# GuoYi0/alphaFive

Hardware: AMD Instinct MI355X
Metric: self-play moves/sec (11x11, 500 sims/move) (higher is better)
Workload: dtype f32 (fp16x2 split operands: 3 fp16 MFMA products per MAC, fp32 accumulate)

## Files before the change

### alphafive_amd/csrc/af_conv_f16s.h

```cpp
#ifndef AF_CONV_F16S_H
#define AF_CONV_F16S_H

#include <hip/hip_runtime.h>

#define AF_NET_BLOCKS(X) X("bone/block1", 32, 64) X("bone/block2", 64, 128) X("value/block3", 128, 32) X("policy/block4", 128, 64) X("policy/block5", 64, 32)
struct NetBlock { const char* name; int cin, cout; };
#define AF_BLOCK_ROW(name, cin, cout) {name, cin, cout},
constexpr NetBlock kBlocks[5] = {AF_NET_BLOCKS(AF_BLOCK_ROW)};
enum { kVarStemK, kVarStemB, kVarHeads, kVarVcK = kVarHeads, kVarVcB, kVarV1K, kVarV1B, kVarV2K, kVarV2B, kVarPcK, kVarPcB, kVarPfK, kVarPfB,
       kVarBlocks, kVars = kVarBlocks + 6 * 5, kC1K = 0, kC1B, kC2K, kC2B, kResK, kResB };
constexpr int var(int block, int which) { return kVarBlocks + 6 * block + which; }
struct NetVar { const char* name; int c0, c1, c2; };
#define AF_BLOCK_VARS(name, cin, cout) {name "_conv1/kernel", 9 * cin * cout}, {name "_conv1/bias", cout}, {name "_conv2/kernel", 9 * cout * cout}, \
                                       {name "_conv2/bias", cout}, {name "_res/kernel", cin * cout}, {name "_res/bias", cout},
constexpr NetVar kNetVars[kVars] = {
    {"bone/conv1/kernel", 75 * 32}, {"bone/conv1/bias", 32}, {"value/conv/kernel", 32 * 4}, {"value/conv/bias", 4},
    {"value/fc1/kernel", 0, 4 * 64}, {"value/fc1/bias", 64}, {"value/fc2/kernel", 64}, {"value/fc2/bias", 1},
    {"policy/conv/kernel", 32 * 16}, {"policy/conv/bias", 16}, {"policy/fc/kernel", 0, 0, 16}, {"policy/fc/bias", 0, 1},
    AF_NET_BLOCKS(AF_BLOCK_VARS)};

struct f16s_net;

int f16s_supported(int board_size);
int f16s_create(f16s_net** out, int board_size, int max_batch, int device);
void f16s_destroy(f16s_net* n);
int f16s_reset_roles(f16s_net* n);
enum F16sBits : int {
    kF16sProfilingBits = 1 | 2 | 4 | 8 | 4096,
    kF16sValuStem = 16,
    kF16sOneWgPerCu = 32,
    kF16sTwoHalves15 = 64,
    kF16sWgPerPosition = 128,
    kF16sTwoLaunchBlocks = 256,
    kF16sBranchLaunchesSmall = 512,
    kF16sBranchLaunchesBig = 1024,
    kF16sLaunchSequence = 2048,
};
enum F16sForm {
    kF16sRoles,
    kF16sPaired,
    kF16sBranches,
};
struct F16sPlan {
    int batch, bits;
    bool heads;
    F16sForm form;
    bool valu_stem, two_wg_per_cu, half_classes, tile_split, fused_blocks;
};
F16sPlan f16s_plan(const f16s_net* n, int batch, int bits, bool heads);
int f16s_forward(f16s_net* n, const F16sPlan& p, hipStream_t st, const float* planes_dev, float* value, float* policy);
int f16s_trunk(f16s_net* n, const F16sPlan& p, hipStream_t st, const float* planes_dev);
int f16s_value_branch(f16s_net* n, const F16sPlan& p, hipStream_t st, float* o3_dev, int WP, int PP, float* value);
int f16s_policy_branch(f16s_net* n, const F16sPlan& p, hipStream_t st, float* o5_dev, int WP, int PP, float* policy);
int f16s_small_forward_error(f16s_net* n);
int f16s_read_activation(f16s_net* n, int which, int batch, float* host);

constexpr int kF16sScaleGroups = 20;
int f16s_update_absmax(f16s_net* n, hipStream_t st, const float* const* src, float* max_dev);
int f16s_update_pack(f16s_net* n, hipStream_t st, const float* const* src, const float* max_host);
int f16s_weight_buffer(const f16s_net* n, int index, const void** ptr, size_t* bytes);
int f16s_scales(const f16s_net* n, float* out, int cap);
struct UpdCopy { float* dst; const float* a; const float* b; int n_dst, n_src, sum; };
int upd_launch_copies(hipStream_t st, const UpdCopy* d, int count);

#endif
```

### alphafive_amd/csrc/af_conv_f16s.hip

```cpp
#include <hip/hip_runtime.h>
#include <stdint.h>
#include <stdio.h>
#include <stdlib.h>
#include <string.h>

#include <algorithm>
#include <atomic>
#include <cmath>
#include <vector>

#include "af_conv_f16s.h"

typedef _Float16 h8 __attribute__((ext_vector_type(8)));
typedef float f32x16 __attribute__((ext_vector_type(16)));
typedef float f32x4 __attribute__((ext_vector_type(4)));

#define FS_HIP_OK(x) do { hipError_t e_ = (x); if (e_ != hipSuccess) { fprintf(stderr, "[af_conv_f16s] %s failed: %s\n", #x, hipGetErrorString(e_)); return -2; } } while (0)

namespace {

template <int S_> struct Geo;
template <> struct Geo<11> {
    static constexpr int S = 11, NPIX = 121, HALVES = 1, POFF = 11;
    static constexpr uint32_t ROWU = 144, WINU = 144;
    static constexpr int PR = 2, NPC = 4;
    static constexpr uint32_t PADL = 8, PADR = 8;
    __host__ __device__ static constexpr uint32_t seg_unit(int seg) { return 8u + 64u * (uint32_t)seg; }
    __host__ __device__ static constexpr uint32_t wbase(int) { return 0u; }
};
template <> struct Geo<15> {
    static constexpr int S = 15, NPIX = 225, HALVES = 2, POFF = 16;
    static constexpr uint32_t ROWU = 256, WINU = 160;
    static constexpr int PR = 3, NPC = 6;
    static constexpr uint32_t PADL = 0, PADR = 0;
    __host__ __device__ static constexpr uint32_t seg_unit(int seg) { return seg == 0 ? 0u : (seg == 1 ? 64u : 96u); }
    __host__ __device__ static constexpr uint32_t wbase(int h) { return h ? 96u : 0u; }
};
template <class G> struct Lay {
    static constexpr uint32_t kRowH = G::ROWU * 16u, kHalfH = 4u * kRowH, kSlabH = 2u * kHalfH;
    static constexpr uint32_t kRowL = G::WINU * 16u, kHalfL = 4u * kRowL, kSlotL = 2u * kHalfL;
};
constexpr uint32_t kLds0 = 256u;
#ifndef AF_F16S_DIST
#define AF_F16S_DIST 3
#endif
constexpr int kDist = AF_F16S_DIST;
template <class G, int DIST = kDist> struct Lds {
    static constexpr uint32_t kZoff = kLds0 + (DIST + 2) * Lay<G>::kSlotL;
    static constexpr uint32_t kBiasOff = kZoff + Lay<G>::kSlotL;
    static constexpr uint32_t kScrOff = kBiasOff + 512u;
};
template <class G> struct Hx {
    static constexpr int HXP = 128 * G::HALVES;
    static constexpr uint32_t kValPos = HXP * 16u, kValLo = HXP * 8u;
    static constexpr uint32_t kPolPos = HXP * 64u, kPolLo = HXP * 32u;
    static constexpr int VSTEPS = (G::NPIX + 3) / 4;
    static constexpr int NLT = (G::NPIX + 31) / 32;
};

constexpr int kS = 11, kPIX = 144, kNPIX = kS * kS;
constexpr uint32_t kRowB = kPIX * 16u, kHalfB = 4u * kRowB, kSlabB = 2u * kHalfB;

#ifndef AF_F16S_APIN
#define AF_F16S_APIN 1
#endif
#ifndef AF_F16S_VW
#define AF_F16S_VW 128
#endif
#ifndef AF_F16S_ZPAD
#define AF_F16S_ZPAD 1
#endif

__device__ __forceinline__ void st16(void* gdst, const h8& v) { *reinterpret_cast<h8*>(gdst) = v; }

template <class V16>
__device__ __forceinline__ void st16_sc1(void* gdst, const V16& v) {
    static_assert(sizeof(V16) == 16, "16-byte store");
    asm volatile("global_store_dwordx4 %0, %1, off sc1\n\ts_nop 1" : : "v"(gdst), "v"(v) : "memory");
}
template <class V8>
__device__ __forceinline__ void st8_sc1(void* gdst, const V8& v) {
    static_assert(sizeof(V8) == 8, "8-byte store");
    asm volatile("global_store_dwordx2 %0, %1, off sc1" : : "v"(gdst), "v"(v) : "memory");
}

__device__ __forceinline__ void wait_vmcnt(int n) {
#define AF_VM(k) case k: asm volatile("s_waitcnt vmcnt(" #k ")" ::: "memory"); break;
    switch (n) {
        AF_VM(0) AF_VM(1) AF_VM(2) AF_VM(3) AF_VM(4) AF_VM(5) AF_VM(6) AF_VM(7) AF_VM(8) AF_VM(9) AF_VM(10) AF_VM(11) AF_VM(12) AF_VM(13)
        AF_VM(14) AF_VM(15) AF_VM(16) AF_VM(17) AF_VM(18) AF_VM(19) AF_VM(20) AF_VM(21) AF_VM(22) AF_VM(23) AF_VM(24) AF_VM(25) AF_VM(26)
        AF_VM(27) AF_VM(28) AF_VM(29) AF_VM(30) AF_VM(31) AF_VM(32) AF_VM(33) AF_VM(34) AF_VM(35) AF_VM(36) AF_VM(37) AF_VM(38) AF_VM(39)
        AF_VM(40) AF_VM(41) AF_VM(42) AF_VM(43) AF_VM(44) AF_VM(45) AF_VM(46) AF_VM(47) AF_VM(48) AF_VM(49) AF_VM(50) AF_VM(51) AF_VM(52)
        AF_VM(53) AF_VM(54) AF_VM(55) AF_VM(56) AF_VM(57) AF_VM(58) AF_VM(59) AF_VM(60) AF_VM(61) AF_VM(62) AF_VM(63)
        default: asm volatile("s_waitcnt vmcnt(0)" ::: "memory"); break;
    }
#undef AF_VM
}

__device__ __forceinline__ void glds16(const void* gsrc, uint32_t lds_dst) {
    unsigned keep;
    asm volatile("s_mov_b32 %0, m0\n\ts_mov_b32 m0, %2\n\ts_nop 0\n\tglobal_load_lds_dwordx4 %1, off nt\n\ts_mov_b32 m0, %0"
                 : "=&s"(keep) : "v"(gsrc), "s"(lds_dst) : "memory");
}

__device__ __forceinline__ void glds16_sc1(const void* gsrc, uint32_t lds_dst) {
    unsigned keep;
    asm volatile("s_mov_b32 %0, m0\n\ts_mov_b32 m0, %2\n\ts_nop 0\n\tglobal_load_lds_dwordx4 %1, off sc1\n\ts_mov_b32 m0, %0"
                 : "=&s"(keep) : "v"(gsrc), "s"(lds_dst) : "memory");
}

typedef float f32x2 __attribute__((ext_vector_type(2)));
__device__ __forceinline__ float elu1(float x) {
    const float e = __builtin_amdgcn_exp2f(x * 1.44269504088896341f);
    return fmaxf(x, fminf(fmaxf(e, 0.0f), 1.0f) - 1.0f);
}
__device__ __forceinline__ f32x2 elu2(f32x2 x) {
    const f32x2 t = x * 1.44269504088896341f;
    f32x2 e;
    e.x = fminf(fmaxf(__builtin_amdgcn_exp2f(t.x), 0.0f), 1.0f);
    e.y = fminf(fmaxf(__builtin_amdgcn_exp2f(t.y), 0.0f), 1.0f);
    const f32x2 em1 = e - 1.0f;
    return f32x2{fmaxf(x.x, em1.x), fmaxf(x.y, em1.y)};
}

#ifndef AF_F16S_XCD_SWIZZLE
#define AF_F16S_XCD_SWIZZLE 1
#endif
#ifdef AF_F16S_TIMING
__device__ unsigned long long g_f16s_cycles[10][512][4][9];
__device__ unsigned long long g_f16s_wall[10][512][2];
#define AF_T(var) const unsigned long long var = __builtin_readcyclecounter()
#define AF_TACC(slot, a, b) tacc[slot] += (b) - (a)
#else
#define AF_T(var)
#define AF_TACC(slot, a, b)
#endif

#ifdef AF_DF_TIMING
__device__ unsigned long long g_df_wall[256][5];
#define DF_T(i) if (threadIdx.x == 0 && blockIdx.x < 256) g_df_wall[blockIdx.x][i] = wall_clock64()
#else
#define DF_T(i)
#endif
__device__ __forceinline__ void df_signal(int* ctr) {
    DF_T(2);
    asm volatile("s_waitcnt vmcnt(0)" ::: "memory");
    __syncthreads();
    if (threadIdx.x == 0) __hip_atomic_fetch_add(ctr, 1, __ATOMIC_RELAXED, __HIP_MEMORY_SCOPE_AGENT);
    DF_T(3);
}
__device__ __forceinline__ void df_poll(const int* ctr, int need, int* err) {
    int it = 0;
    while (__hip_atomic_load(ctr, __ATOMIC_RELAXED, __HIP_MEMORY_SCOPE_AGENT) < need) {
        __builtin_amdgcn_s_sleep(2);
        if (++it > (1 << 22)) { __hip_atomic_store(err, 1, __ATOMIC_RELAXED, __HIP_MEMORY_SCOPE_AGENT); break; }
    }
}
__device__ __forceinline__ void df_wait_one(const int* ctr, int need, int* err) {
    if (threadIdx.x == 0) df_poll(ctr, need, err);
    DF_T(1);
    __syncthreads();
}
__device__ __forceinline__ void df_wait_inv(const int* ctr, int need, int* err) {
    if (threadIdx.x == 0) {
        df_poll(ctr, need, err);
        __builtin_amdgcn_fence(__ATOMIC_ACQUIRE, "agent");
    }
    DF_T(1);
    __syncthreads();
}

struct F16sArgs {
    const char* in;
    const char* in2;
    const uint4* w;
    const float* bias;
    char* out;
    float* out32;
    float inv_scale;
    const uint4* pw;
    float* pbuf;
    float inv_scale_p;
    const uint4* hw;
    const float* hbias;
    char* hx;
    float inv_scale_h;
    int batch, WP, PP;
    const uint4* w2;
    const float* bias2;
    float inv_scale2;
    int gx0;
    char* stash;
    const int* df_wait;
    int df_need;
    int* df_done;
    int* df_err;
    int abl;
};

template <class G, int NSM, int NSP, int CT, int KS, int PS, bool OUT32, bool XACC, int PJ, int HD, int DIST, int WPE, int NTW, int HSEL, int FU = 0, int DF = 0>
__device__ __forceinline__ void f16s_body(const F16sArgs& A, char* smem, const int bx, const int gxw, const int tb = 0,
                                          const int by = (int)blockIdx.y, const int gy = (int)gridDim.y) {
    using L = Lay<G>;
    constexpr uint32_t kRowH = L::kRowH, kHalfH = L::kHalfH, kSlabH = L::kSlabH, kRowL = L::kRowL, kHalfL = L::kHalfL, kSlotL = L::kSlotL;
    constexpr uint32_t kZoff = Lds<G, DIST>::kZoff, kBiasOff = Lds<G, DIST>::kBiasOff, kScrOff = Lds<G, DIST>::kScrOff;
    constexpr int kDist = DIST, kRing = DIST + 2;
    constexpr int NPC = G::NPC, HV = G::HALVES;
    static_assert(FU == 0 || (G::HALVES == 1 && PJ == 1 && HD == 0 && !OUT32 && NSP == 0 && CT == 1 && HSEL < 0 &&
                              ((KS == 1 && NTW == 1) || (KS == 2 && NTW == 2))), "fused block: see above");
    constexpr uint32_t kScrBytes = KS == 2 ? (uint32_t)(CT * PS * NTW) * 4096u * (PJ == 1 ? 2u : 1u) : 0u;
    constexpr uint32_t kGOff = Lds<G, DIST>::kScrOff;
    constexpr uint32_t kW2Off = kGOff + (kScrBytes > Lay<G>::kSlotL ? kScrBytes : Lay<G>::kSlotL);
    constexpr int NT = NTW;
    static_assert(HSEL < 0 || (HV == 2 && PJ == 0 && HD == 0 && !OUT32), "half classes: plain 15x15 layers only");
    static_assert(NT % KS == 0 || PJ == 0, "an odd tile count under a k-split has no projection exchange");
    constexpr int C16 = 2 / KS;
    constexpr int ITP = C16, ITM = 9 * C16;
    constexpr int NIT = NSP * ITP + NSM * ITM;
    constexpr int SPP = NSP + NSM;
    constexpr int NFIN = NT / KS;
    static_assert(CT * KS * PS == 4 && NT >= KS, "4 waves");
    static_assert(PJ == 0 || NSP == 0, "a producer / consumer of the separate projection has no projection slabs");
    constexpr int NPW = PJ == 1 ? NSM * C16 : 0;
    static_assert(NPC * (DIST > 1 ? DIST - 1 : 1) < 64, "vmcnt is a 6-bit field");
    static_assert(DIST >= 2 || (NSP == 0 && ITM - 1 >= NPC), "distance 1: a slab's pieces must all be issued before its predecessor's last item");
    const int lane = threadIdx.x & 63, kg = lane >> 5, nn = lane & 31;
    const int wv = __builtin_amdgcn_readfirstlane((int)(threadIdx.x >> 6));
    const int ct = wv % CT, ks = (wv / CT) % KS, ps = wv / (CT * KS);
    const int rot = KS == 2 ? ks * ((NT + 1) / 2) : 0;
#define AF_OWN(jj) (KS == 1 || (jj) < NT / 2 || ((jj) < (NT + 1) / 2 && ks == 0))
    const int ctg = by * CT + ct, nso = gy * CT;
    const uint32_t lds = (uint32_t)(uintptr_t)smem;

    const int nq = HSEL >= 0 ? A.batch : A.batch * HV;
    int qpos = bx;
    if (AF_F16S_XCD_SWIZZLE && (gxw & (8 * (HSEL >= 0 ? 1 : HV) - 1)) == 0) qpos = (bx >> 3) + (gxw >> 3) * (bx & 7);
    if (qpos >= nq) return;
    const int hv = HSEL >= 0 ? HSEL : (HV == 1 ? 0 : qpos % HV);
    const uint32_t wsrc = G::wbase(hv) * 16u;
    AF_T(t_entry);
#ifdef AF_F16S_TIMING
    const unsigned long long wall_entry = wall_clock64();
#endif

    auto slab_src = [&](int qq, int j) -> const char* {
        const int p_ = (HV == 1 || HSEL >= 0) ? qq : qq / HV;
        const int p = (A.abl & 0x1000) ? (p_ & 127) : p_;
        return (j < NSM ? A.in + ((size_t)p * NSM + j) * kSlabH : A.in2 + ((size_t)p * NSP + (j - NSM)) * kSlabH) + wsrc;
    };
    auto dma_piece = [&](const char* src, uint32_t slot_off, int k) {
        const int piece = wv + 4 * k, row = piece / G::PR;
        const uint32_t su = G::seg_unit(piece % G::PR) * 16u;
        const uint32_t offh = (uint32_t)(row >> 2) * kHalfH + (uint32_t)(row & 3) * kRowH + su;
        const uint32_t offl = (uint32_t)(row >> 2) * kHalfL + (uint32_t)(row & 3) * kRowL + su;
        if (DF != 0) glds16_sc1(src + offh + lane * 16, (uint32_t)__builtin_amdgcn_readfirstlane((int)(lds + kLds0 + slot_off + offl)));
        else glds16(src + offh + lane * 16, (uint32_t)__builtin_amdgcn_readfirstlane((int)(lds + kLds0 + slot_off + offl)));
    };
    const int q0 = qpos;
    auto stream_src = [&](uint32_t idx) -> const char* {
        const int p = q0 + (int)(idx / SPP) * gxw, j = (int)(idx % SPP);
        return slab_src(p, j);
    };
    const uint32_t nslabs = (uint32_t)((nq - q0 + gxw - 1) / gxw) * SPP;

    if (DF == 0) {
#pragma unroll
        for (int d = 0; d < kDist; ++d) {
            if ((uint32_t)d < nslabs) {
#pragma unroll
                for (int k = 0; k < NPC; ++k) dma_piece(stream_src(d), (uint32_t)d * kSlotL, k);
            }
        }
    }

    h8 W[2 * NIT];
    {
        const uint4* wp = A.w + ((size_t)(ctg * KS + ks) * (2 * NIT)) * 64 + lane;
#pragma unroll
        for (int f = 0; f < 2 * NIT; ++f) {
            const uint4 v = wp[f * 64];
            __builtin_memcpy(&W[f], &v, 16);
        }
    }
    h8 PW[PJ == 1 ? 2 * NPW : 1];
    if (PJ == 1) {
        const uint4* wp = A.pw + ((size_t)(ctg * KS + ks) * (2 * NPW)) * 64 + lane;
#pragma unroll
        for (int f = 0; f < 2 * NPW; ++f) {
            const uint4 v = wp[f * 64];
            __builtin_memcpy(&PW[f], &v, 16);
        }
    }
    constexpr int HDS = HD > 0 ? HD : FU;
    h8 HA[HDS > 0 ? 4 : 1];
    float hb[HDS > 0 ? 8 : 1];
    if (FU > 0) {
        const uint4* w2 = A.w2;
#pragma unroll
        for (int i = 0; i < 9; ++i) *reinterpret_cast<uint4*>(smem + kW2Off + (uint32_t)(i * 256 + (int)threadIdx.x) * 16u) = w2[i * 256 + threadIdx.x];
        if (threadIdx.x < 32) reinterpret_cast<float*>(smem + kBiasOff + 256u)[threadIdx.x] = A.bias2[threadIdx.x];
        if (KS == 1) {
            for (uint32_t u = threadIdx.x; u < kSlotL / 16; u += 256) *reinterpret_cast<uint4*>(smem + kGOff + u * 16) = uint4{0, 0, 0, 0};
        }
    }
    if (HDS > 0) {
#pragma unroll
        for (int f = 0; f < 4; ++f) {
            const uint4 v = A.hw[f * 64 + lane];
            __builtin_memcpy(&HA[f], &v, 16);
        }
#pragma unroll
        for (int r = 0; r < 8; ++r) hb[r] = A.hbias[8 * kg + r];
    }
    if (threadIdx.x < kLds0 / 16) *reinterpret_cast<uint4*>(smem + threadIdx.x * 16) = uint4{0, 0, 0, 0};
    if (G::PADL + G::PADR > 0) {
        static_assert(G::PADL + G::PADR == 0 || (G::PADL == 8 && G::PADR == 8), "pad zeroing is written for 8 + 8 units");
        for (uint32_t u = threadIdx.x; u < (uint32_t)kRing * 128u; u += 256) {
            const uint32_t off = kLds0 + (u >> 7) * kSlotL + ((u >> 4) & 7u) * kRowL + (((u >> 3) & 1u) ? (G::WINU - 8u) * 16u : 0u) + (u & 7u) * 16u;
            *reinterpret_cast<uint4*>(smem + off) = uint4{0, 0, 0, 0};
        }
    }
    for (uint32_t u = threadIdx.x; u < kSlotL / 16; u += 256) *reinterpret_cast<uint4*>(smem + kZoff + u * 16) = uint4{0, 0, 0, 0};
    if (threadIdx.x < CT * 32) reinterpret_cast<float*>(smem + kBiasOff)[threadIdx.x] = A.bias[by * CT * 32 + threadIdx.x];
    uint32_t lb[NT], zb[NT];
    int pix[NT];
    bool ok[NT], edgeL[NT], edgeR[NT];
#pragma unroll
    for (int jj = 0; jj < NT; ++jj) {
        const int n = 128 * hv + 32 * (tb + ps * NT + ((jj + rot) % NT)) + nn;
        ok[jj] = n < G::NPIX;
        const int nc = ok[jj] ? n : 128 * hv;
        pix[jj] = nc;
        const int x = nc % G::S;
        edgeL[jj] = x == 0; edgeR[jj] = x == G::S - 1;
        lb[jj] = kLds0 + (uint32_t)((KS == 2 ? 2 * ks : 0) + kg) * kRowL + (uint32_t)((nc + G::POFF - G::S - 1 - (int)G::wbase(hv)) * 16);
        zb[jj] = kZoff + (lb[jj] & 255u);
    }
    constexpr int kAccRegs = 16 * NT * (1 + (XACC ? 1 : 0) + (PJ == 1 ? 1 : 0));
    constexpr int kWRegs = 4 * (2 * NIT + (PJ == 1 ? 2 * NPW : 0) + (HDS > 0 ? 4 : 0));
    constexpr int kNAmax = (256 - kAccRegs - 16) / 4, kNAwant = (kWRegs - AF_F16S_VW + 3) / 4;
    constexpr int NA = (AF_F16S_APIN && WPE == 1 && kNAwant > 0) ? (kNAwant < kNAmax ? kNAwant : kNAmax) : 0;
#pragma unroll
    for (int f = 0; f < 2 * NIT; ++f) {
        if (f < 2 * NIT - NA) asm volatile("" : "+v"(W[f]));
        else asm volatile("" : "+a"(W[f]));
    }
    if (PJ == 1) {
#pragma unroll
        for (int f = 0; f < 2 * NPW; ++f) asm volatile("" : "+v"(PW[f]));
    }
    if (HDS > 0) {
#pragma unroll
        for (int f = 0; f < 4; ++f) asm volatile("" : "+v"(HA[f]));
    }
    if (DF != 0) {
        df_wait_one(A.df_wait + qpos, A.df_need, A.df_err);
#pragma unroll
        for (int d = 0; d < kDist; ++d) {
            if ((uint32_t)d < nslabs) {
#pragma unroll
                for (int k = 0; k < NPC; ++k) dma_piece(stream_src(d), (uint32_t)d * kSlotL, k);
            }
        }
    }
    asm volatile("s_waitcnt vmcnt(0) lgkmcnt(0)" ::: "memory");
    __builtin_amdgcn_s_barrier();
    AF_T(t_ready);

    auto rd = [](const char* sm, bool proj, int it, int p, uint32_t c_, uint32_t l_, uint32_t r_) -> h8 {
        const int c = proj ? it : it / 9, tap = proj ? 4 : it % 9, ky = tap / 3, kx = tap % 3;
        const uint32_t base = kx == 0 ? l_ : (kx == 2 ? r_ : c_);
        const uint32_t imm = (uint32_t)p * kHalfL + (KS == 1 ? 2u * c * kRowL : 0u) + (uint32_t)(ky * G::S + kx) * 16u;
        return *reinterpret_cast<const h8*>(sm + base + imm);
    };

    auto head_tile = [&](const float (&v)[16], const int jj, const int pos) {
      if constexpr (HDS > 0) {
        h8 bh[2], bl[2];
#pragma unroll
        for (int st_ = 0; st_ < 2; ++st_)
#pragma unroll
            for (int e = 0; e < 8; ++e) {
                const float f = v[8 * st_ + e];
                const _Float16 h = (_Float16)f;
                bh[st_][e] = h;
                bl[st_][e] = (_Float16)(f - (float)h);
            }
        f32x16 a2;
#pragma unroll
        for (int r = 0; r < 16; ++r) a2[r] = 0.0f;
#pragma unroll
        for (int st_ = 0; st_ < 2; ++st_) {
            a2 = __builtin_amdgcn_mfma_f32_32x32x16_f16(HA[2 * st_], bh[st_], a2, 0, 0, 0);
            a2 = __builtin_amdgcn_mfma_f32_32x32x16_f16(HA[2 * st_], bl[st_], a2, 0, 0, 0);
            a2 = __builtin_amdgcn_mfma_f32_32x32x16_f16(HA[2 * st_ + 1], bh[st_], a2, 0, 0, 0);
        }
        constexpr int NR = HDS == 1 ? 4 : 8;
        _Float16 uh[8], ul[8];
#pragma unroll
        for (int r = 0; r < NR; ++r) {
            const float f = elu1(a2[r] * A.inv_scale_h + hb[r]);
            const _Float16 h = (_Float16)f;
            uh[r] = h;
            ul[r] = (_Float16)(f - (float)h);
        }
        if (ok[jj] && !(A.abl & 2)) {
            if (HDS == 1) {
                if (kg == 0) {
                    typedef _Float16 h4 __attribute__((ext_vector_type(4)));
                    char* o = A.hx + (size_t)pos * Hx<G>::kValPos + (uint32_t)pix[jj] * 8u;
                    if (DF != 0) {
                        st8_sc1(o, h4{uh[0], uh[1], uh[2], uh[3]});
                        st8_sc1(o + Hx<G>::kValLo, h4{ul[0], ul[1], ul[2], ul[3]});
                    } else {
                        *reinterpret_cast<h4*>(o) = h4{uh[0], uh[1], uh[2], uh[3]};
                        *reinterpret_cast<h4*>(o + Hx<G>::kValLo) = h4{ul[0], ul[1], ul[2], ul[3]};
                    }
                }
            } else {
                char* o = A.hx + (size_t)pos * Hx<G>::kPolPos + (uint32_t)pix[jj] * 32u + (uint32_t)kg * 16u;
                if (DF != 0) {
                    st16_sc1(o, h8{uh[0], uh[1], uh[2], uh[3], uh[4], uh[5], uh[6], uh[7]});
                    st16_sc1(o + Hx<G>::kPolLo, h8{ul[0], ul[1], ul[2], ul[3], ul[4], ul[5], ul[6], ul[7]});
                } else {
                    *reinterpret_cast<h8*>(o) = h8{uh[0], uh[1], uh[2], uh[3], uh[4], uh[5], uh[6], uh[7]};
                    *reinterpret_cast<h8*>(o + Hx<G>::kPolLo) = h8{ul[0], ul[1], ul[2], ul[3], ul[4], ul[5], ul[6], ul[7]};
                }
            }
        }
      }
    };
    uint32_t t = 0;
    uint32_t cur = 0u, nxd = (uint32_t)kDist * kSlotL;
    constexpr bool XPOS = !(NT >= 3 && NIT >= 36) && FU == 0;
    h8 fr[2][NT][2];
#define AF_FIRST_ITEM(slot)                                                                                      \
    _Pragma("unroll") for (int jj = 0; jj < NT; ++jj) {                                                          \
        const uint32_t c_ = (AF_F16S_ZPAD && !ok[jj]) ? zb[jj] : lb[jj] + (slot), l_ = edgeL[jj] ? zb[jj] : c_, r_ = edgeR[jj] ? zb[jj] : c_; \
        fr[0][jj][0] = rd(smem, false, 0, 0, c_, l_, r_);                                                        \
        fr[0][jj][1] = rd(smem, false, 0, 1, c_, l_, r_);                                                        \
    }
    if (XPOS) { AF_FIRST_ITEM(0u) }
#ifdef AF_F16S_TIMING
    unsigned long long tacc[8] = {0, 0, 0, 0, 0, 0, 0, 0};
#endif
    for (; qpos < nq; qpos += gxw) {
        const int pos = (HV == 1 || HSEL >= 0) ? qpos : qpos / HV;
        AF_T(tp0);
        if (!XPOS) { AF_FIRST_ITEM(cur) }
#undef AF_FIRST_ITEM
        f32x16 acc[NT], acx[XACC ? NT : 1], pac[PJ == 1 ? NT : 1];
#pragma unroll
        for (int jj = 0; jj < NT; ++jj)
#pragma unroll
            for (int r = 0; r < 16; ++r) { acc[jj][r] = 0.0f; if (XACC) acx[jj][r] = 0.0f; if (PJ == 1) pac[jj][r] = 0.0f; }
        f32x4 padd[PJ == 2 ? NFIN : 1][4];
        if (PJ == 2) {
#pragma unroll
            for (int jf = 0; jf < NFIN; ++jf) {
                const int tile = tb + ps * NT + (KS == 2 ? ks * NFIN : 0) + jf;
                const f32x4* src = reinterpret_cast<const f32x4*>(A.pbuf) + ((((size_t)qpos * nso + ctg) * 4 + tile) * 4) * 64 + lane;
#pragma unroll
                for (int q = 0; q < 4; ++q) padd[jf][q] = src[q * 64];
            }
        }

#pragma clang loop unroll(full)
        for (int j = 0; j < SPP; ++j) {
            const bool proj = j >= NSM;
            const bool nproj = (j + 1) % SPP >= NSM;
            const int ms = j, pslab = j - NSM;
            const int NI = proj ? ITP : ITM;
            const int ibase = proj ? pslab * ITP : NSP * ITP + ms * ITM;
            const int seq = proj ? NSM * ITM + pslab * ITP : ms * ITM;
            const int npos = qpos + ((j + kDist) / SPP) * gxw;
            const bool more = npos < nq && !(A.abl & 1);
            const char* nsrc = slab_src((A.abl & 4) ? q0 : (more ? npos : qpos), (j + kDist) % SPP);
            const uint32_t nx1 = cur + kSlotL == kRing * kSlotL ? 0u : cur + kSlotL;
            uint32_t bC[NT], bL[NT], bR[NT];
#pragma unroll
            for (int jj = 0; jj < NT; ++jj) {
                bC[jj] = (AF_F16S_ZPAD && !ok[jj]) ? zb[jj] : lb[jj] + cur;
                bL[jj] = edgeL[jj] ? zb[jj] : bC[jj];
                bR[jj] = edgeR[jj] ? zb[jj] : bC[jj];
            }
            if (HSEL == 1 && wv == (j & 3) && by == 0 && lane < 32) {
                const uint32_t u = (uint32_t)(lane & 3), un = (u < 2 ? 128u + u : 141u + u);
                const uint4 q = *reinterpret_cast<const uint4*>(smem + kLds0 + cur + (uint32_t)(lane >> 4) * kHalfL + (uint32_t)((lane >> 2) & 3) * kRowL + un * 16u);
                *reinterpret_cast<uint4*>(A.stash + (((size_t)pos * SPP + j) * 32 + lane) * 16) = q;
            }
#pragma clang loop unroll(full)
            for (int it = 0; it < NI; ++it) {
                const int b = (seq + it) & 1;
                if (it + 1 < NI) {
#pragma unroll
                    for (int jj = 0; jj < NT; ++jj) {
                        fr[b ^ 1][jj][0] = rd(smem, proj, it + 1, 0, bC[jj], bL[jj], bR[jj]);
                        fr[b ^ 1][jj][1] = rd(smem, proj, it + 1, 1, bC[jj], bL[jj], bR[jj]);
                    }
                } else {
                    const int issued = NI - 1 < NPC ? NI - 1 : NPC;
                    AF_T(tw0);
                    if (more) {
                        wait_vmcnt(NPC * (kDist - 2) + issued);
                    } else {
                        asm volatile("s_waitcnt vmcnt(0)" ::: "memory");
                    }
                    AF_T(tw1);
                    __builtin_amdgcn_s_barrier();
                    AF_T(tw2);
                    AF_TACC(1, tw0, tw1);
                    AF_TACC(2, tw1, tw2);
                    if ((XPOS || j + 1 < SPP) && t + 1 < nslabs) {
#pragma unroll
                        for (int jj = 0; jj < NT; ++jj) {
                            const uint32_t c_ = (AF_F16S_ZPAD && !ok[jj]) ? zb[jj] : lb[jj] + nx1, l_ = edgeL[jj] ? zb[jj] : c_, r_ = edgeR[jj] ? zb[jj] : c_;
                            fr[b ^ 1][jj][0] = rd(smem, nproj, 0, 0, c_, l_, r_);
                            fr[b ^ 1][jj][1] = rd(smem, nproj, 0, 1, c_, l_, r_);
                        }
                    }
                }
                const h8 wh = W[2 * (ibase + it)], wl = W[2 * (ibase + it) + 1];
#pragma unroll
                for (int jj = 0; jj < NT; ++jj) acc[jj] = __builtin_amdgcn_mfma_f32_32x32x16_f16(wh, fr[b][jj][0], acc[jj], 0, 0, 0);
                if (XACC) {
#pragma unroll
                    for (int jj = 0; jj < NT; ++jj) acx[jj] = __builtin_amdgcn_mfma_f32_32x32x16_f16(wh, fr[b][jj][1], acx[jj], 0, 0, 0);
#pragma unroll
                    for (int jj = 0; jj < NT; ++jj) acx[jj] = __builtin_amdgcn_mfma_f32_32x32x16_f16(wl, fr[b][jj][0], acx[jj], 0, 0, 0);
                } else {
#pragma unroll
                    for (int jj = 0; jj < NT; ++jj) acc[jj] = __builtin_amdgcn_mfma_f32_32x32x16_f16(wh, fr[b][jj][1], acc[jj], 0, 0, 0);
#pragma unroll
                    for (int jj = 0; jj < NT; ++jj) acc[jj] = __builtin_amdgcn_mfma_f32_32x32x16_f16(wl, fr[b][jj][0], acc[jj], 0, 0, 0);
                }
                if (PJ == 1 && !proj && it % 9 == 4) {
                    const int pi = ms * C16 + it / 9;
                    const h8 ph = PW[2 * pi], pl = PW[2 * pi + 1];
#pragma unroll
                    for (int jj = 0; jj < NT; ++jj) pac[jj] = __builtin_amdgcn_mfma_f32_32x32x16_f16(ph, fr[b][jj][0], pac[jj], 0, 0, 0);
#pragma unroll
                    for (int jj = 0; jj < NT; ++jj) pac[jj] = __builtin_amdgcn_mfma_f32_32x32x16_f16(ph, fr[b][jj][1], pac[jj], 0, 0, 0);
#pragma unroll
                    for (int jj = 0; jj < NT; ++jj) pac[jj] = __builtin_amdgcn_mfma_f32_32x32x16_f16(pl, fr[b][jj][0], pac[jj], 0, 0, 0);
                }
#pragma unroll
                for (int q = 0; q < 2 * NT; ++q) {
                    __builtin_amdgcn_sched_group_barrier(0x008, 1, 0);
                    __builtin_amdgcn_sched_group_barrier(0x100, 1, 0);
                }
                __builtin_amdgcn_sched_group_barrier(0x008, NT, 0);
                if (more) {
                    if (it < NI - 1 && it < NPC) dma_piece(nsrc, nxd, it);
                    if (it == NI - 1) {
#pragma unroll
                        for (int k = (NI - 1 < NPC ? NI - 1 : NPC); k < NPC; ++k) dma_piece(nsrc, nxd, k);
                    }
                }
            }
            ++t;
            cur = nx1;
            nxd = nxd + kSlotL == kRing * kSlotL ? 0u : nxd + kSlotL;
        }
        if (XPOS && (NIT & 1)) {
#pragma unroll
            for (int jj = 0; jj < NT; ++jj) { fr[0][jj][0] = fr[1][jj][0]; fr[0][jj][1] = fr[1][jj][1]; }
        }

        AF_T(tp1);
        if (XACC) {
#pragma unroll
            for (int jj = 0; jj < NT; ++jj)
#pragma unroll
                for (int r = 0; r < 16; ++r) acc[jj][r] += acx[jj][r];
        }
#define AF_EXCHANGE(ACC, SCR)                                                                                              \
    {                                                                                                                      \
        _Pragma("unroll") for (int jj = 0; jj < NT; ++jj) {                                                                \
            if (!AF_OWN(jj)) {                                                                                             \
                _Pragma("unroll") for (int q = 0; q < 4; ++q) {                                                            \
                    f32x4 v = {ACC[jj][4 * q], ACC[jj][4 * q + 1], ACC[jj][4 * q + 2], ACC[jj][4 * q + 3]};                \
                    *reinterpret_cast<f32x4*>((SCR) + (uint32_t)(((jj + rot) % NT) * 4 + q) * 1024u + lane * 16u) = v;     \
                }                                                                                                          \
            }                                                                                                              \
        }                                                                                                                  \
    }
#define AF_COMBINE(ACC, SCR)                                                                                               \
    {                                                                                                                      \
        _Pragma("unroll") for (int jj = 0; jj < NT; ++jj) {                                                                \
            if (AF_OWN(jj)) {                                                                                              \
                _Pragma("unroll") for (int q = 0; q < 4; ++q) {                                                            \
                    const f32x4 v = *reinterpret_cast<const f32x4*>((SCR) + (uint32_t)(((jj + rot) % NT) * 4 + q) * 1024u + lane * 16u); \
                    ACC[jj][4 * q] += v[0]; ACC[jj][4 * q + 1] += v[1]; ACC[jj][4 * q + 2] += v[2]; ACC[jj][4 * q + 3] += v[3]; \
                }                                                                                                          \
            }                                                                                                              \
        }                                                                                                                  \
    }
        if (KS == 2) {
            char* scr = smem + kScrOff + (uint32_t)(ct + CT * ps) * (NT * 4096u);
            char* scp = scr + (uint32_t)(CT * PS) * (NT * 4096u);
            AF_EXCHANGE(acc, scr)
            if (PJ == 1) AF_EXCHANGE(pac, scp)
            asm volatile("s_waitcnt lgkmcnt(0)" ::: "memory");
            AF_T(tx0);
            __builtin_amdgcn_s_barrier();
            AF_T(tx1);
            AF_TACC(7, tx0, tx1);
            AF_COMBINE(acc, scr)
            if (PJ == 1) AF_COMBINE(pac, scp)
        }
#undef AF_EXCHANGE
#undef AF_COMBINE
        if (PJ == 1 && FU == 0) {
#pragma unroll
            for (int jj = 0; jj < NT; ++jj) {
                if (!AF_OWN(jj)) continue;
                f32x4* dst = reinterpret_cast<f32x4*>(A.pbuf) + ((((size_t)qpos * nso + ctg) * 4 + tb + ps * NT + ((jj + rot) % NT)) * 4) * 64 + lane;
                if (!(A.abl & 2)) {
#pragma unroll
                    for (int q = 0; q < 4; ++q) {
                        f32x4 v = {pac[jj][4 * q] * A.inv_scale_p, pac[jj][4 * q + 1] * A.inv_scale_p, pac[jj][4 * q + 2] * A.inv_scale_p, pac[jj][4 * q + 3] * A.inv_scale_p};
                        dst[q * 64] = v;
                    }
                }
            }
        }

        if (FU > 0 && KS == 2) {
// ... 186 lines not shown
    const int tile = (int)blockIdx.y * 4 + (int)(threadIdx.x >> 6);
    if (tile >= A.NCT) return;
    const int p = 32 * (int)blockIdx.x + nn;
    const bool valid = p < A.batch;
    const size_t pc = (size_t)(valid ? p : A.batch - 1);
    f32x16 acc[KS], acx[XACC ? KS : 1];
#pragma unroll
    for (int h = 0; h < KS; ++h)
#pragma unroll
        for (int r = 0; r < 16; ++r) { acc[h][r] = 0.0f; if (XACC) acx[h][r] = 0.0f; }
    const uint4* const wbase = A.w + (size_t)tile * KS * NIT * 2 * 64 + lane;
    constexpr int SPP = NSM + NSP;
    const char* const st0 = A.stash + (pc * SPP * 32 + (uint32_t)kg * 4u) * 16;
    struct Ops { uint4 a0, a1, b0, b1; };
    auto half_of = [](int t) constexpr -> int {
        const int k16 = t < NSM * 8 ? (t >> 2) & 1 : (t - NSM * 8) & 1;
        return KS == 2 ? k16 : 0;
    };
    auto fetch = [&](int t) -> Ops {
        int k16, item;
        const char* bsrc;
        if (t < NSM * 8) {
            const int s_ = t >> 3, tq = t & 3, ky = tq >> 1, kx = tq & 1;
            k16 = (t >> 2) & 1;
            item = NSP * C16 + s_ * 9 * C16 + (KS == 2 ? 0 : k16) * 9 + 3 * ky + kx;
            bsrc = st0 + (uint32_t)((s_ * 32 + 2 * k16 * 4 + tq) * 16);
        } else {
            const int u = t - NSM * 8, s_ = u >> 1;
            k16 = u & 1;
            item = s_ * C16 + (KS == 2 ? 0 : k16);
            bsrc = st0 + (uint32_t)(((NSM + s_) * 32 + 2 * k16 * 4 + 3) * 16);
        }
        const uint4* wp = wbase + ((size_t)((KS == 2 ? k16 : 0) * NIT + item) * 2) * 64;
        Ops o;
        o.a0 = wp[0]; o.a1 = wp[64];
        o.b0 = *reinterpret_cast<const uint4*>(bsrc); o.b1 = *reinterpret_cast<const uint4*>(bsrc + 256);
        return o;
    };
    Ops ring[D];
#pragma unroll
    for (int t = 0; t < D; ++t) ring[t] = fetch(t);
    __builtin_amdgcn_sched_barrier(0);
#pragma unroll
    for (int t = 0; t < NST; ++t) {
        const Ops o = ring[t % D];
        if (t + D < NST) ring[t % D] = fetch(t + D);
        const int h = half_of(t);
        h8 wh, wl, bh, bl;
        __builtin_memcpy(&wh, &o.a0, 16); __builtin_memcpy(&wl, &o.a1, 16); __builtin_memcpy(&bh, &o.b0, 16); __builtin_memcpy(&bl, &o.b1, 16);
        acc[h] = __builtin_amdgcn_mfma_f32_32x32x16_f16(wh, bh, acc[h], 0, 0, 0);
        if (XACC) {
            acx[h] = __builtin_amdgcn_mfma_f32_32x32x16_f16(wh, bl, acx[h], 0, 0, 0);
            acx[h] = __builtin_amdgcn_mfma_f32_32x32x16_f16(wl, bh, acx[h], 0, 0, 0);
        } else {
            acc[h] = __builtin_amdgcn_mfma_f32_32x32x16_f16(wh, bl, acc[h], 0, 0, 0);
            acc[h] = __builtin_amdgcn_mfma_f32_32x32x16_f16(wl, bh, acc[h], 0, 0, 0);
        }
        __builtin_amdgcn_sched_group_barrier(0x008, 3, 0);
        __builtin_amdgcn_sched_group_barrier(0x020, 4, 0);
    }
    if (XACC) {
#pragma unroll
        for (int h = 0; h < KS; ++h)
#pragma unroll
            for (int r = 0; r < 16; ++r) acc[h][r] += acx[h][r];
    }
    if (KS == 2) {
#pragma unroll
        for (int r = 0; r < 16; ++r) acc[0][r] = acc[KS - 1][r] + acc[0][r];
    }
    if (!valid) return;
    float v[16];
#pragma unroll
    for (int r = 0; r < 16; r += 2) {
        const f32x2 pre = f32x2{acc[0][r], acc[0][r + 1]} * A.inv_scale + f32x2{A.bias[32 * tile + 16 * kg + r], A.bias[32 * tile + 16 * kg + r + 1]};
        const f32x2 y = elu2(pre);
        v[r] = y.x; v[r + 1] = y.y;
    }
    char* o = A.out + ((size_t)p * A.NCT + tile) * L::kSlabH + (uint32_t)(2 * kg) * L::kRowH + (uint32_t)(CPIX + G::POFF) * 16u;
#pragma unroll
    for (int hf = 0; hf < 2; ++hf) {
        h8 hi, lo;
#pragma unroll
        for (int e = 0; e < 8; ++e) {
            const float f = v[8 * hf + e];
            const _Float16 h = (_Float16)f;
            hi[e] = h;
            lo[e] = (_Float16)(f - (float)h);
        }
        st16(o + hf * L::kRowH, hi);
        st16(o + hf * L::kRowH + L::kHalfH, lo);
    }
}

template <class G>
__global__ __launch_bounds__(256) void af_stem_f16s(const float* __restrict__ planes, const float* __restrict__ w,
                                                    const float* __restrict__ bias, char* __restrict__ out, int batch) {
    constexpr int S = G::S, NPIX = G::NPIX, SP = S + 4;
    constexpr uint32_t kRowH = Lay<G>::kRowH, kHalfH = Lay<G>::kHalfH, kSlabH = Lay<G>::kSlabH;
    __shared__ float sx[3 * SP * SP];
    __shared__ float sw[75 * 32];
    __shared__ float sb[32];
    const int t = threadIdx.x;
    for (int i = t; i < 75 * 32; i += 256) sw[i] = w[i];
    if (t < 32) sb[t] = bias[t];
    for (int i = t; i < 3 * SP * SP; i += 256) sx[i] = 0.0f;
    for (int b = blockIdx.x; b < batch; b += gridDim.x) {
        __syncthreads();
        for (int i = t; i < 3 * NPIX; i += 256) {
            const int c = i / NPIX, p = i - c * NPIX, y = p / S, x = p - y * S;
            sx[c * SP * SP + (y + 2) * SP + x + 2] = planes[(size_t)b * 3 * NPIX + i];
        }
        __syncthreads();
        if (t < NPIX) {
            const int y = t / S, x = t - y * S;
            float acc[32];
#pragma unroll
            for (int co = 0; co < 32; ++co) acc[co] = sb[co];
            for (int ky = 0; ky < 5; ++ky)
                for (int kx = 0; kx < 5; ++kx)
#pragma unroll
                    for (int c = 0; c < 3; ++c) {
                        const float xv = sx[c * SP * SP + (y + ky) * SP + x + kx];
                        const float* wr = sw + ((ky * 5 + kx) * 3 + c) * 32;
#pragma unroll
                        for (int co = 0; co < 32; ++co) acc[co] = fmaf(xv, wr[co], acc[co]);
                    }
            char* o = out + (size_t)b * kSlabH + (uint32_t)(t + G::POFF) * 16u;
#pragma unroll
            for (int u = 0; u < 4; ++u) {
                h8 hi, lo;
#pragma unroll
                for (int e = 0; e < 8; ++e) {
                    const float f = elu1(acc[8 * u + e]);
                    const _Float16 h = (_Float16)f;
                    hi[e] = h;
                    lo[e] = (_Float16)(f - (float)h);
                }
                *reinterpret_cast<h8*>(o + u * kRowH) = hi;
                *reinterpret_cast<h8*>(o + u * kRowH + kHalfH) = lo;
            }
        }
    }
}

template <class G> struct StemLds {
    static constexpr int SR = G::S + 4, IW = G::S + 5;
    static constexpr int kEnt = 3 * SR * G::S + 1, kImg = 3 * SR * IW;
    static constexpr uint32_t kImgOff = (uint32_t)((kEnt * 16 + 255) / 256 * 256), kBytes = kImgOff + (uint32_t)kImg * 2u;
};
template <class G, bool SC1 = false>
__device__ __forceinline__ void f16s_stem_body(const float* __restrict__ planes, const uint4* __restrict__ w ,
                                               const float* __restrict__ bias, float inv_scale, char* __restrict__ out, int batch,
                                               const int bx, const int gx, uint4* ent, _Float16* img) {
    constexpr int S = G::S, NPIX = G::NPIX, SR = S + 4, IW = S + 5;
    constexpr int NPL = 3 * NPIX, NLD = (NPL + 255) / 256;
    constexpr int NTL = (NPIX + 31) / 32, NRND = (NTL + 3) / 4;
    constexpr uint32_t kRowH = Lay<G>::kRowH, kHalfH = Lay<G>::kHalfH, kSlabH = Lay<G>::kSlabH;
    const int lane = threadIdx.x & 63, kg = lane >> 5, nn = lane & 31;
    const int wv = __builtin_amdgcn_readfirstlane((int)(threadIdx.x >> 6));
    h8 W[16];
#pragma unroll
    for (int f = 0; f < 16; ++f) {
        const uint4 v = w[f * 64 + lane];
        __builtin_memcpy(&W[f], &v, 16);
    }
    float bs[16];
#pragma unroll
    for (int r = 0; r < 16; ++r) bs[r] = bias[16 * kg + r];
    for (int i = threadIdx.x; i < 3 * SR * IW; i += 256) img[i] = (_Float16)0.0f;
    auto img_at = [](int i) -> int { const int c = i / NPIX, p = i - c * NPIX, y = p / S, x = p - y * S; return (c * SR + y + 2) * IW + x + 2; };
    int at[NLD];
    float nx[NLD];
#pragma unroll
    for (int q = 0; q < NLD; ++q) {
        const int i = (int)threadIdx.x + 256 * q;
        at[q] = img_at(i < NPL ? i : 0);
        nx[q] = 0.0f;
        if (i < NPL && bx < batch) nx[q] = planes[(size_t)bx * NPL + i];
    }
    for (int pos = bx; pos < batch; pos += gx) {
        __syncthreads();
#pragma unroll
        for (int q = 0; q < NLD; ++q)
            if ((int)threadIdx.x + 256 * q < NPL) img[at[q]] = (_Float16)nx[q];
        if (pos + gx < batch) {
            const float* pl = planes + (size_t)(pos + gx) * NPL;
#pragma unroll
            for (int q = 0; q < NLD; ++q)
                if ((int)threadIdx.x + 256 * q < NPL) nx[q] = pl[threadIdx.x + 256 * q];
        }
        __syncthreads();
        for (int en = threadIdx.x; en < 3 * SR * S; en += 256) {
            const int cin = en / (SR * S), rem = en - cin * SR * S, yy = rem / S, x = rem - yy * S;
            const _Float16* src = img + (cin * SR + yy) * IW + x;
            const h8 v = {src[0], src[1], src[2], src[3], src[4], 0, 0, 0};
            __builtin_memcpy(&ent[en], &v, 16);
        }
        __syncthreads();
#pragma unroll
        for (int rd_ = 0; rd_ < NRND; ++rd_) {
            const int n = 32 * (wv + 4 * rd_) + nn;
            const bool ok = n < NPIX;
            const int nc = ok ? n : 0;
            if (32 * (wv + 4 * rd_) >= NPIX) continue;
            f32x16 acc;
#pragma unroll
            for (int r = 0; r < 16; ++r) acc[r] = 0.0f;
#pragma unroll
            for (int s_ = 0; s_ < 8; ++s_) {
                const int ga = 2 * s_, gb = 2 * s_ + 1 < 15 ? 2 * s_ + 1 : 0;
                const uint32_t offa = (uint32_t)((ga / 5) * SR + ga % 5) * S, offb = (uint32_t)((gb / 5) * SR + gb % 5) * S;
                h8 b;
                __builtin_memcpy(&b, &ent[(uint32_t)nc + (kg ? offb : offa)], 16);
                acc = __builtin_amdgcn_mfma_f32_32x32x16_f16(W[2 * s_], b, acc, 0, 0, 0);
                acc = __builtin_amdgcn_mfma_f32_32x32x16_f16(W[2 * s_ + 1], b, acc, 0, 0, 0);
            }
            char* o = out + (size_t)pos * kSlabH + (uint32_t)(2 * kg) * kRowH + (uint32_t)(nc + G::POFF) * 16u;
#pragma unroll
            for (int hf = 0; hf < 2; ++hf) {
                h8 hi, lo;
#pragma unroll
                for (int e = 0; e < 8; ++e) {
                    const float f = elu1(acc[8 * hf + e] * inv_scale + bs[8 * hf + e]);
                    const _Float16 h = (_Float16)f;
                    hi[e] = h;
                    lo[e] = (_Float16)(f - (float)h);
                }
                if (ok) {
                    if (SC1) { st16_sc1(o + hf * kRowH, hi); st16_sc1(o + hf * kRowH + kHalfH, lo); }
                    else {
                        *reinterpret_cast<h8*>(o + hf * kRowH) = hi;
                        *reinterpret_cast<h8*>(o + hf * kRowH + kHalfH) = lo;
                    }
                }
            }
        }
    }
}

template <class G>
__global__ __launch_bounds__(256) void af_stem_mfma_f16s(const float* __restrict__ planes, const uint4* __restrict__ w, const float* __restrict__ bias,
                                                         float inv_scale, char* __restrict__ out, int batch) {
    __shared__ __attribute__((aligned(16))) uint4 ent[StemLds<G>::kEnt];
    __shared__ _Float16 img[StemLds<G>::kImg];
    f16s_stem_body<G>(planes, w, bias, inv_scale, out, batch, (int)blockIdx.x, (int)gridDim.x, ent, img);
}

template <class G>
__device__ __forceinline__ void f16s_vfc_body(const char* __restrict__ xv, const uint4* __restrict__ a, const float* __restrict__ b1,
                                              const float* __restrict__ w2, const float* __restrict__ b2, float inv_scale,
                                              float* __restrict__ value, int batch, const int bx) {
    __shared__ float red[2][32];
    constexpr int NS = Hx<G>::VSTEPS;
    const bool act = threadIdx.x < 128;
    const int lane = threadIdx.x & 63, mt = (threadIdx.x >> 6) & 1, n = lane & 31, kg = lane >> 5;
    const int pos = bx * 32 + n, posc = pos < batch ? pos : batch - 1;
    const char* xb = xv + (size_t)posc * Hx<G>::kValPos + (uint32_t)kg * 16u;
    const uint4* ap = a + (size_t)mt * 128 + lane;
    f32x16 acc;
#pragma unroll
    for (int r = 0; r < 16; ++r) acc[r] = 0.0f;
#pragma unroll
    for (int half = 0; half < (NS + 15) / 16; ++half) {
        uint4 bh[16], bl[16], ah[16], al[16];
#pragma unroll
        for (int q = 0; q < 16; ++q) {
            const int s_ = 16 * half + q;
            if (s_ < NS) {
                bh[q] = *reinterpret_cast<const uint4*>(xb + s_ * 32);
                bl[q] = *reinterpret_cast<const uint4*>(xb + Hx<G>::kValLo + s_ * 32);
                ah[q] = ap[(size_t)s_ * 256];
                al[q] = ap[(size_t)s_ * 256 + 64];
            }
        }
        typedef uint32_t u32x4 __attribute__((ext_vector_type(4)));
#pragma unroll
        for (int q = 0; q < 16; ++q) {
            if (16 * half + q < NS) {
                u32x4 t0, t1, t2, t3;
                __builtin_memcpy(&t0, &bh[q], 16); __builtin_memcpy(&t1, &bl[q], 16); __builtin_memcpy(&t2, &ah[q], 16); __builtin_memcpy(&t3, &al[q], 16);
                asm volatile("" : "+v"(t0), "+v"(t1), "+v"(t2), "+v"(t3));
                __builtin_memcpy(&bh[q], &t0, 16); __builtin_memcpy(&bl[q], &t1, 16); __builtin_memcpy(&ah[q], &t2, 16); __builtin_memcpy(&al[q], &t3, 16);
            }
        }
#pragma unroll
        for (int q = 0; q < 16; ++q) {
            if (16 * half + q < NS) {
                h8 xh, xl, wh, wl;
                __builtin_memcpy(&xh, &bh[q], 16); __builtin_memcpy(&xl, &bl[q], 16);
                __builtin_memcpy(&wh, &ah[q], 16); __builtin_memcpy(&wl, &al[q], 16);
                acc = __builtin_amdgcn_mfma_f32_32x32x16_f16(wh, xh, acc, 0, 0, 0);
                acc = __builtin_amdgcn_mfma_f32_32x32x16_f16(wh, xl, acc, 0, 0, 0);
                acc = __builtin_amdgcn_mfma_f32_32x32x16_f16(wl, xh, acc, 0, 0, 0);
            }
        }
    }
    float part = 0.0f;
#pragma unroll
    for (int r = 0; r < 16; ++r) {
        const int j = 32 * mt + 16 * kg + r;
        part += elu1(acc[r] * inv_scale + b1[j]) * w2[j];
    }
    part += __shfl_xor(part, 32);
    if (act && kg == 0) red[mt][n] = part;
    __syncthreads();
    if (act && mt == 0 && kg == 0 && pos < batch) value[pos] = tanhf((red[0][n] + red[1][n] + b2[0]) * 0.5f);
}
template <class G>
__global__ __launch_bounds__(128) __attribute__((amdgpu_waves_per_eu(1, 2))) void af_value_fc_f16s(
    const char* __restrict__ xv, const uint4* __restrict__ a , const float* __restrict__ b1, const float* __restrict__ w2,
    const float* __restrict__ b2, float inv_scale, float* __restrict__ value, int batch) {
    f16s_vfc_body<G>(xv, a, b1, w2, b2, inv_scale, value, batch, (int)blockIdx.x);
}
struct VfcArgs { const char* xv; const uint4* a; const float *b1, *w2, *b2; float inv_scale; float* value; };
template <class G>
__global__ __launch_bounds__(256, 1) __attribute__((amdgpu_waves_per_eu(1, 1))) void af_small_l7v_f16s(F16sArgs P, VfcArgs V) {
    extern __shared__ __attribute__((aligned(16))) char smem[];
    const int nb = P.batch, id = (int)blockIdx.x;
    if (id < 2 * nb) f16s_body<G, 2, 4, 2, 2, 1, false, true, 0, 0, kDist, 1, 2, -1>(P, smem, id % nb, nb, (id / nb) * 2);
    else f16s_vfc_body<G>(V.xv, V.a, V.b1, V.w2, V.b2, V.inv_scale, V.value, nb, id - 2 * nb);
}
template <class G>
__global__ __launch_bounds__(256, 1) __attribute__((amdgpu_waves_per_eu(1, 1))) void af_big_l7v_f16s(F16sArgs P, VfcArgs V) {
    extern __shared__ __attribute__((aligned(16))) char smem[];
    const int gp = P.gx0, id = (int)blockIdx.x;
    if (id < gp) f16s_body<G, 2, 4, 2, 2, 1, false, true, 0, 0, kDist, 1, 4, -1>(P, smem, id, gp);
    else f16s_vfc_body<G>(V.xv, V.a, V.b1, V.w2, V.b2, V.inv_scale, V.value, P.batch, id - gp);
}

constexpr int kDfStem = 0, kDfL0 = 8, kDfL1 = 16, kDfL2 = 24, kDfL3 = 32, kDfP = 40, kDfV = 48, kDfQ = 56, kDfB5 = 64, kDfPF = 72, kDfFin = 73, kDfErr = 74, kDfWords = 75;
struct SmallFwdArgs {
    const float* planes; const uint4* stem_w; const float* stem_b; float stem_inv; char* f0;
    F16sArgs L0, L1, L2, L3, P, V, Q, B5;
    VfcArgs F;
    const char* xp; const uint4* pfa; const float* pfb; float pf_inv; float* policy; float* pfx;
    int* df;
    int batch;
};

template <class G>
__device__ __forceinline__ void f16s_pfc_role(const SmallFwdArgs& S, const int kh, char* smem) {
    constexpr int NPIX = G::NPIX, HXP = Hx<G>::HXP, NLT = Hx<G>::NLT, LW = 32 * NLT, LWP = LW + 1, NS = HXP / 2, RD = 32;
    static_assert(NLT == 4 && NS == 64, "the role form of the policy head is written for 11x11 (one logit tile per wave)");
    const int nb = S.batch, lane = threadIdx.x & 63, n = lane & 31, kg = lane >> 5;
    const int mt = __builtin_amdgcn_readfirstlane((int)(threadIdx.x >> 6));
    int* const df = S.df;
    const int step0 = NS * kh, nstep = NPIX - step0 < NS ? NPIX - step0 : NS;
    const uint4* ap = S.pfa + ((size_t)step0 * NLT + mt) * 128 + lane;
    uint4 ring[RD][2];
#pragma unroll
    for (int q = 0; q < RD; ++q) {
        const int st_ = q < nstep ? q : nstep - 1;
        ring[q][0] = ap[(size_t)st_ * NLT * 128];
        ring[q][1] = ap[(size_t)st_ * NLT * 128 + 64];
    }
    float bj[16];
#pragma unroll
    for (int r = 0; r < 16; ++r) { const int j = 32 * mt + 16 * kg + r; bj[r] = S.pfb[j < NPIX ? j : 0]; }
    {
        unsigned sink = 0;
#pragma unroll
        for (int q = RD; q < NS; ++q) {
            const int st_ = q < nstep ? q : nstep - 1;
            sink ^= reinterpret_cast<const unsigned*>(ap + (size_t)st_ * NLT * 128)[0] ^ reinterpret_cast<const unsigned*>(ap + (size_t)st_ * NLT * 128 + 64)[0];
        }
        asm volatile("" : : "v"(sink));
    }
    if (threadIdx.x == 0) {
        for (int p = 0; p < nb; ++p) df_poll(df + kDfB5 + p, 1, df + kDfErr);
    }
    DF_T(1);
    __syncthreads();
    constexpr uint32_t kXS = 2u * NS * 32u + 16u;
    for (int c = mt; c < nb * 4; c += 4) {
        const int pp = c >> 2, hl = (c >> 1) & 1, part = c & 1;
        glds16_sc1(S.xp + (size_t)pp * Hx<G>::kPolPos + (uint32_t)hl * Hx<G>::kPolLo + (uint32_t)step0 * 32u + (uint32_t)part * 1024u + (uint32_t)lane * 16u,
                   (uint32_t)__builtin_amdgcn_readfirstlane((int)((uint32_t)(uintptr_t)smem + (uint32_t)pp * kXS + (uint32_t)hl * (NS * 32u) + (uint32_t)part * 1024u)));
    }
    asm volatile("s_waitcnt vmcnt(0)" ::: "memory");
    __syncthreads();
    const int pq = n < nb ? n : nb - 1;
    const char* xb = smem + (uint32_t)pq * kXS + (uint32_t)kg * 16u;
    f32x16 acc;
#pragma unroll
    for (int r = 0; r < 16; ++r) acc[r] = 0.0f;
    h8 bh = *reinterpret_cast<const h8*>(xb), bl = *reinterpret_cast<const h8*>(xb + NS * 32);
#pragma unroll
    for (int st_ = 0; st_ < NS; ++st_) {
        h8 ah, al, nbh = bh, nbl = bl;
        __builtin_memcpy(&ah, &ring[st_ % RD][0], 16); __builtin_memcpy(&al, &ring[st_ % RD][1], 16);
        if (st_ + 1 < NS) {
            nbh = *reinterpret_cast<const h8*>(xb + (st_ + 1) * 32);
            nbl = *reinterpret_cast<const h8*>(xb + NS * 32 + (st_ + 1) * 32);
        }
        if (st_ + RD < NS) {
            const int pf = st_ + RD < nstep ? st_ + RD : nstep - 1;
            ring[st_ % RD][0] = ap[(size_t)pf * NLT * 128];
            ring[st_ % RD][1] = ap[(size_t)pf * NLT * 128 + 64];
// ... 490 lines not shown
            const int c16 = D.KS == 2 ? ks : c;
            const int co = 32 * tile + row_perm(m), ci = 32 * s + 16 * c16 + 8 * kh + e;
            return (proj ? D.w1[(size_t)ci * D.cout + co] : D.w3[((size_t)tap * D.cin + ci) * D.cout + co]) * D.scale;
        }
        case FK_STEM: {
            const int g = 2 * f + kh;
            if (e >= 5 || g >= 15) return 0.0f;
            const int cin = g / 5, ky = g - 5 * cin;
            return D.w3[(size_t)((ky * 5 + e) * 3 + cin) * 32 + row_perm(m)] * D.scale;
        }
        case FK_HCONV: {
            const int co = m < 16 ? 8 * ((m >> 2) & 1) + 4 * (m >> 3) + (m & 3) : 99, ci = 16 * kh + 8 * f + e;
            return co < D.nc ? D.w3[(size_t)ci * D.nc + co] * D.scale : 0.0f;
        }
        case FK_VFC: {
            const int s_ = f >> 1, mt = f & 1, px = 4 * s_ + 2 * kh + (e >> 2), ch = e & 3, j = 32 * mt + row_perm(m);
            return px < D.npix ? D.w3[(size_t)(ch * D.npix + px) * 64 + j] * D.scale : 0.0f;
        }
        default: {
            const int nlt = (D.npix + 31) / 32, px = f / nlt, mt = f - px * nlt, c16 = 8 * kh + e, j = 32 * mt + row_perm(m);
            return j < D.npix ? D.w3[(size_t)(c16 * D.npix + px) * D.npix + j] * D.scale : 0.0f;
        }
    }
}

constexpr int kFragBlocks = 64;
__global__ __launch_bounds__(256) void af_update_frags(FragTable T) {
#pragma clang fp contract(off)
    const FragDesc& D = T.d[blockIdx.y];
    for (int row = blockIdx.x * 256 + threadIdx.x; row < D.frags * 64; row += kFragBlocks * 256) {
        const int f = row >> 6, lane = row & 63;
        h8 hi, lo;
#pragma unroll
        for (int e = 0; e < 8; ++e) {
            const float v = frag_value(D, f, lane, e);
            const _Float16 h = (_Float16)v;
            hi[e] = h;
            lo[e] = (_Float16)(v - (float)h);
        }
        h8* dst = reinterpret_cast<h8*>(D.dst);
        dst[(size_t)(2 * f) * 64 + lane] = hi;
        dst[(size_t)(2 * f + 1) * 64 + lane] = lo;
    }
}

constexpr int kMaxCopies = 48, kCopyBlocks = 32;
struct CopyTable { UpdCopy d[kMaxCopies]; };
__global__ __launch_bounds__(256) void af_update_copy(CopyTable T) {
    const UpdCopy& D = T.d[blockIdx.y];
    for (int i = blockIdx.x * 256 + threadIdx.x; i < D.n_dst; i += kCopyBlocks * 256) {
        float v = 0.0f;
        if (i < D.n_src) v = D.sum ? D.a[i] + (D.b ? D.b[i] : 0.0f) : D.a[i];
        D.dst[i] = v;
    }
}

}

int upd_launch_copies(hipStream_t st, const UpdCopy* d, int count) {
    if (count < 1 || count > kMaxCopies) return -1;
    CopyTable T = {};
    for (int i = 0; i < count; ++i) T.d[i] = d[i];
    hipLaunchKernelGGL(af_update_copy, dim3(kCopyBlocks, count), dim3(256), 0, st, T);
    FS_HIP_OK(hipGetLastError());
    return 0;
}

int f16s_update_absmax(f16s_net* n, hipStream_t st, const float* const* src, float* max_dev) {
    const int npix = n->S * n->S;
    MaxTable T = {};
    T.g[0] = {src[kVarStemK], nullptr, 75 * 32, 0};
    for (int b = 0; b < 5; ++b) {
        const LayerCfg &L1 = kLayers[2 * b], &L2 = kLayers[2 * b + 1];
        const float* kr = src[var(b, kResK)];
        const int nr = L1.cin * L2.cout;
        T.g[1 + 3 * b] = {src[var(b, kC1K)], nullptr, 9 * L1.cin * L1.cout, 0};
        T.g[2 + 3 * b] = {src[var(b, kC2K)], kr, 9 * L2.cin * L2.cout, L1.pj == 1 ? 0 : nr};
        T.g[3 + 3 * b] = {kr, nullptr, nr, 0};
    }
    T.g[16] = {src[kVarVcK], nullptr, 32 * 4, 0};
    T.g[17] = {src[kVarPcK], nullptr, 32 * 16, 0};
    T.g[18] = {src[kVarV1K], nullptr, 4 * npix * 64, 0};
    T.g[19] = {src[kVarPfK], nullptr, 16 * npix * npix, 0};
    FS_HIP_OK(hipMemsetAsync(max_dev, 0, kF16sScaleGroups * sizeof(float), st));
    hipLaunchKernelGGL(af_update_absmax, dim3(kMaxBlocks, kF16sScaleGroups), dim3(256), 0, st, T, max_dev);
    FS_HIP_OK(hipGetLastError());
    return 0;
}

int f16s_update_pack(f16s_net* n, hipStream_t st, const float* const* src, const float* max_host) {
    const int npix = n->S * n->S;
    float sc[kF16sScaleGroups];
    for (int g = 0; g < kF16sScaleGroups; ++g) sc[g] = pick_scale(max_host[g]);
    FragTable T = {};
    int nb = 0;
    auto frag = [&](uint4* dst, const float* w3, const float* w1, float scale, int kind, int frags, int cin, int cout, int pcin, int KS, int nc) {
        T.d[nb++] = FragDesc{dst, w3, w1, scale, kind, frags, cin, cout, pcin, KS, nc, npix};
    };
    UpdCopy C[kMaxCopies];
    int ncp = 0;
    auto copy = [&](float* dst, const float* a, const float* b, int n_dst, int n_src, int sum) { C[ncp++] = UpdCopy{dst, a, b, n_dst, n_src, sum}; };
    frag(n->stem_wm, src[kVarStemK], nullptr, sc[0], FK_STEM, kStemFrags, 0, 0, 0, 1, 0);
    copy(n->stem_w, src[kVarStemK], nullptr, 75 * 32, 75 * 32, 0);
    copy(n->stem_b, src[kVarStemB], nullptr, 32, 32, 0);
    for (int b = 0; b < 5; ++b) {
        const LayerCfg &L1 = kLayers[2 * b], &L2 = kLayers[2 * b + 1];
        const float *k1 = src[var(b, kC1K)], *k2 = src[var(b, kC2K)], *kr = src[var(b, kResK)];
        frag(n->w[2 * b], k1, nullptr, sc[1 + 3 * b], FK_LAYER, layer_frags(L1), L1.cin, L1.cout, L1.pcin, L1.KS, 0);
        frag(n->w[2 * b + 1], k2, kr, sc[2 + 3 * b], FK_LAYER, layer_frags(L2), L2.cin, L2.cout, L2.pcin, L2.KS, 0);
        if (L1.pj == 1) frag(n->pw[2 * b], nullptr, kr, sc[3 + 3 * b], FK_LAYER, proj_frags(L1, L2.cout), 0, L2.cout, L1.cin, L1.KS, 0);
        copy(n->bias[2 * b], src[var(b, kC1B)], nullptr, L1.cout, L1.cout, 0);
        copy(n->bias[2 * b + 1], src[var(b, kC2B)], src[var(b, kResB)], L2.cout, L2.cout, 1);
    }
    frag(n->hcw[0], src[kVarVcK], nullptr, sc[16], FK_HCONV, kHconvFrags, 0, 0, 0, 1, 4);
    frag(n->hcw[1], src[kVarPcK], nullptr, sc[17], FK_HCONV, kHconvFrags, 0, 0, 0, 1, 16);
    frag(n->hfw[0], src[kVarV1K], nullptr, sc[18], FK_VFC, vfc_frags(npix), 0, 0, 0, 1, 0);
    frag(n->hfw[1], src[kVarPfK], nullptr, sc[19], FK_PFC, pfc_frags(npix), 0, 0, 0, 1, 0);
    copy(n->hcb[0], src[kVarVcB], nullptr, 16, 4, 0);
    copy(n->hcb[1], src[kVarPcB], nullptr, 16, 16, 0);
    copy(n->hfb[0], src[kVarV1B], nullptr, 64, 64, 0);
    copy(n->hfb[1], src[kVarPfB], nullptr, npix, npix, 0);
    copy(n->v2w, src[kVarV2K], nullptr, 64, 64, 0);
    copy(n->v2b, src[kVarV2B], nullptr, 1, 1, 0);
    hipLaunchKernelGGL(af_update_frags, dim3(kFragBlocks, nb), dim3(256), 0, st, T);
    FS_HIP_OK(hipGetLastError());
    if (upd_launch_copies(st, C, ncp)) return -2;
    n->stem_inv_scale = 1.0f / sc[0];
    for (int b = 0; b < 5; ++b) {
        n->inv_scale[2 * b] = 1.0f / sc[1 + 3 * b]; n->inv_scale[2 * b + 1] = 1.0f / sc[2 + 3 * b];
        if (kLayers[2 * b].pj == 1) n->inv_scale_p[2 * b] = 1.0f / sc[3 + 3 * b];
    }
    n->hc_inv[0] = 1.0f / sc[16]; n->hc_inv[1] = 1.0f / sc[17];
    n->hf_inv[0] = 1.0f / sc[18]; n->hf_inv[1] = 1.0f / sc[19];
    return 0;
}

int f16s_weight_buffer(const f16s_net* n, int index, const void** ptr, size_t* bytes) {
    if (!n || index < 0 || index >= (int)n->wreg.size()) return -1;
    *ptr = n->wreg[index].first; *bytes = n->wreg[index].second;
    return 0;
}

int f16s_scales(const f16s_net* n, float* out, int cap) {
    float v[25];
    v[0] = n->stem_inv_scale;
    for (int i = 0; i < 10; ++i) { v[1 + i] = n->inv_scale[i]; v[11 + i] = n->inv_scale_p[i]; }
    v[21] = n->hc_inv[0]; v[22] = n->hc_inv[1]; v[23] = n->hf_inv[0]; v[24] = n->hf_inv[1];
    for (int i = 0; i < 25 && i < cap; ++i) out[i] = v[i];
    return 25;
}

constexpr int kSmallBatch = 8;

F16sPlan f16s_plan(const f16s_net* n, int batch, int bits, bool heads) {
    const bool s11 = n->S == 11, small = batch <= kSmallBatch;
    F16sPlan p = {};
    p.batch = batch; p.bits = bits; p.heads = heads;
    p.valu_stem = bits & kF16sValuStem;
    p.two_wg_per_cu = s11 && !(bits & kF16sOneWgPerCu);
    p.half_classes = !s11 && batch >= 128 && !(bits & kF16sTwoHalves15);
    p.tile_split = small && !(bits & kF16sWgPerPosition);
    p.fused_blocks = s11 && heads && !(bits & kF16sTwoLaunchBlocks);
    if (p.fused_blocks && p.tile_split && p.two_wg_per_cu && !p.valu_stem && !(bits & (kF16sBranchLaunchesSmall | kF16sLaunchSequence)))
        p.form = kF16sRoles;
    else if (p.fused_blocks && (small ? p.tile_split && !(bits & kF16sBranchLaunchesSmall) : !(bits & kF16sBranchLaunchesBig)))
        p.form = kF16sPaired;
    else
        p.form = kF16sBranches;
    return p;
}

static F16sArgs layer_args(const f16s_net* n, const F16sPlan& p, int li, const char* in, const char* in2, char* out) {
    F16sArgs a = {};
    a.in = in; a.in2 = in2; a.out = out;
    a.w = n->w[li]; a.bias = n->bias[li]; a.inv_scale = n->inv_scale[li];
    a.pw = n->pw[li]; a.pbuf = n->pbuf[li / 2]; a.inv_scale_p = n->inv_scale_p[li];
    a.inv_scale2 = a.inv_scale_h = 1.0f;
    a.batch = p.batch; a.stash = n->stash;
    a.abl = (p.bits & 0xf0ff) | (li << 8);
    static const int mask = [] { const char* e = getenv("AF_F16S_ABL_LAYERS"); return e ? (int)strtol(e, nullptr, 0) : 0x3ff; }();
    if (!((mask >> li) & 1)) a.abl &= ~kF16sProfilingBits;
    return a;
}
static void add_conv2(F16sArgs& a, const f16s_net* n, int li) { a.w2 = n->w[li]; a.bias2 = n->bias[li]; a.inv_scale2 = n->inv_scale[li]; }
static void add_head(F16sArgs& a, const f16s_net* n, int h) { a.hw = n->hcw[h]; a.hbias = n->hcb[h]; a.hx = n->hx[h]; a.inv_scale_h = n->hc_inv[h]; }
template <int LI>
static F16sArgs block_args(const f16s_net* n, const F16sPlan& p, const char* in) {
    F16sArgs a = layer_args(n, p, LI, in, nullptr, nullptr);
    add_conv2(a, n, LI + 1);
    add_head(a, n, kHeadOf<LI> - 1);
    return a;
}

template <class F>
static int with_geo(const f16s_net* n, F&& f) { return n->S == 11 ? f(Geo<11>{}) : f(Geo<15>{}); }

template <class G, int LI>
static int launch_one(const f16s_net* n, const F16sPlan& p, hipStream_t st, const F16sArgs& a) {
    constexpr LayerCfg L = kLayers[LI];
    constexpr int NSM = L.cin / 32, NSP = L.pcin / 32, CT = L.CT, KS = L.KS, PS = L.PS, PJ = L.pj, HD = kHeadOf<LI>;
    constexpr bool OUT32 = PJ == 2, XACC = L.xacc;
    const bool head = OUT32 && p.heads;
    if constexpr (G::S == 11 && (LI == 0 || LI == 5 || LI == 9)) {
        if (p.two_wg_per_cu && (head || !OUT32))
            return launch_cfg<G, NSM, NSP, CT, KS, PS, OUT32, XACC && LI != 0, PJ, HD, 1, 2>(st, a, L.gy, n->ncu, p.tile_split);
    }
    if constexpr (G::S == 15 && (LI == 2 || LI == 3 || LI == 6 || LI == 7)) {
        if (p.half_classes) return launch_h15<G, NSM, NSP, CT, KS, XACC>(st, a, L.gy, n->ncu);
    }
    if constexpr (OUT32) {
        if (head) return launch_cfg<G, NSM, NSP, CT, KS, PS, OUT32, XACC, PJ, HD>(st, a, L.gy, n->ncu, p.tile_split);
    }
    return launch_cfg<G, NSM, NSP, CT, KS, PS, OUT32, XACC, PJ>(st, a, L.gy, n->ncu, p.tile_split);
}
template <int LI>
static int launch_layer(const f16s_net* n, const F16sPlan& p, hipStream_t st, const char* in, const char* in2, char* out,
                        float* out32 = nullptr, int WP = 0, int PP = 0) {
    F16sArgs a = layer_args(n, p, LI, in, in2, out);
    a.out32 = out32; a.WP = WP; a.PP = PP;
    if constexpr (kLayers[LI].pj == 2) {
        if (p.heads) add_head(a, n, kHeadOf<LI> - 1);
    }
    return with_geo(n, [&](auto g) { return launch_one<decltype(g), LI>(n, p, st, a); });
}
static int launch_policy_fc(const f16s_net* n, hipStream_t st, int batch, float* policy) {
    return with_geo(n, [&](auto g) {
        hipLaunchKernelGGL(af_policy_fc_f16s<decltype(g)>, dim3((batch + kPfPos - 1) / kPfPos), dim3(512), kPfLds, st, n->hx[1], n->hfw[1], n->hfb[1],
                           n->hf_inv[1], policy, batch);
        FS_HIP_OK(hipGetLastError());
        return 0;
    });
}

int f16s_trunk(f16s_net* n, const F16sPlan& p, hipStream_t st, const float* planes) {
    const int batch = p.batch;
    if (!n || batch < 1 || batch > n->max_batch) return -1;
    int rc = with_geo(n, [&](auto g) {
        using G = decltype(g);
        if (p.valu_stem) hipLaunchKernelGGL(af_stem_f16s<G>, dim3(std::min(batch, 2048)), dim3(256), 0, st, planes, n->stem_w, n->stem_b, n->f0, batch);
        else hipLaunchKernelGGL(af_stem_mfma_f16s<G>, dim3(std::min(batch, 1024)), dim3(256), 0, st, planes, n->stem_wm, n->stem_b, n->stem_inv_scale, n->f0, batch);
        FS_HIP_OK(hipGetLastError());
        return 0;
    });
    if (!rc) rc = launch_layer<0>(n, p, st, n->f0, nullptr, n->g[0]);
    if (!rc) rc = launch_layer<1>(n, p, st, n->g[0], n->f0, n->o[0]);
    if (!rc) rc = launch_layer<2>(n, p, st, n->o[0], nullptr, n->g[1]);
    if (!rc) rc = launch_layer<3>(n, p, st, n->g[1], n->o[0], n->o[1]);
    return rc;
}

int f16s_value_branch(f16s_net* n, const F16sPlan& p, hipStream_t st, float* o3, int WP, int PP, float* value) {
    int rc;
    if (p.fused_blocks) {
        rc = launch_block<Geo<11>, 4>(st, block_args<4>(n, p, n->o[1]), n->ncu);
    } else {
        rc = launch_layer<4>(n, p, st, n->o[1], nullptr, n->g[2]);
        if (!rc) rc = launch_layer<5>(n, p, st, n->g[2], n->o[1], nullptr, o3, WP, PP);
    }
    if (!rc && p.heads)
        rc = with_geo(n, [&](auto g) {
            hipLaunchKernelGGL(af_value_fc_f16s<decltype(g)>, dim3((p.batch + 31) / 32), dim3(128), 0, st, n->hx[0], n->hfw[0], n->hfb[0], n->v2w, n->v2b,
                               n->hf_inv[0], value, p.batch);
            FS_HIP_OK(hipGetLastError());
            return 0;
        });
    return rc;
}

int f16s_policy_branch(f16s_net* n, const F16sPlan& p, hipStream_t st, float* o5, int WP, int PP, float* policy) {
    int rc = launch_layer<6>(n, p, st, n->o[1], nullptr, n->g[3]);
    if (!rc) rc = launch_layer<7>(n, p, st, n->g[3], n->o[1], n->o[3]);
    if (!rc && p.fused_blocks) {
        rc = launch_block<Geo<11>, 8>(st, block_args<8>(n, p, n->o[3]), n->ncu);
    } else {
        if (!rc) rc = launch_layer<8>(n, p, st, n->o[3], nullptr, n->g[4]);
        if (!rc) rc = launch_layer<9>(n, p, st, n->g[4], n->o[3], nullptr, o5, WP, PP);
    }
    if (!rc && p.heads) rc = launch_policy_fc(n, st, p.batch, policy);
    return rc;
}

static int paired_branches(f16s_net* n, const F16sPlan& p, hipStream_t st, float* value, float* policy) {
    using G = Geo<11>;
    const int batch = p.batch;
    F16sArgs P = layer_args(n, p, 6, n->o[1], nullptr, n->g[3]);
    const F16sArgs V = block_args<4>(n, p, n->o[1]);
    constexpr size_t ldsP = Lds<G, kDist>::kScrOff + (size_t)2 * 1 * 4 * 4096;
    constexpr size_t ldsV = Lds<G, 2>::kScrOff + (size_t)2 * 2 * 4096 * 2 + 36864;
    constexpr size_t lds = ldsP > ldsV ? ldsP : ldsV;
    static_assert(lds <= 160 * 1024, "LDS budget");
    uint64_t bit;
    if (device_bit(&bit)) return -2;
    const int gp = std::max(1, std::min(batch, n->ncu));
    if (p.tile_split) {
        if (dyn_lds<af_small_pair_f16s<G>>(bit, 160 * 1024)) return -2;
        hipLaunchKernelGGL(af_small_pair_f16s<G>, dim3(3 * batch), dim3(256), lds, st, P, V);
    } else {
        if (dyn_lds<af_big_pair_f16s<G>>(bit, 160 * 1024)) return -2;
        P.gx0 = gp;
        hipLaunchKernelGGL(af_big_pair_f16s<G>, dim3(2 * gp), dim3(256), lds, st, P, V);
    }
    FS_HIP_OK(hipGetLastError());
    F16sArgs Q = layer_args(n, p, 7, n->g[3], n->o[1], n->o[3]);
    const VfcArgs F = {n->hx[0], n->hfw[0], n->hfb[0], n->v2w, n->v2b, n->hf_inv[0], value};
    constexpr size_t lds7 = Lds<G, kDist>::kScrOff + (size_t)2 * 1 * 4 * 4096;
    if (p.tile_split) {
        if (dyn_lds<af_small_l7v_f16s<G>>(bit, (int)lds7)) return -2;
        hipLaunchKernelGGL(af_small_l7v_f16s<G>, dim3(2 * batch + 1), dim3(256), lds7, st, Q, F);
    } else {
        if (dyn_lds<af_big_l7v_f16s<G>>(bit, (int)lds7)) return -2;
        Q.gx0 = gp;
        hipLaunchKernelGGL(af_big_l7v_f16s<G>, dim3(gp + (batch + 31) / 32), dim3(256), lds7, st, Q, F);
    }
    FS_HIP_OK(hipGetLastError());
    const int rc = launch_block<G, 8>(st, block_args<8>(n, p, n->o[3]), n->ncu);
    return rc ? rc : launch_policy_fc(n, st, batch, policy);
}

static int roles_forward(f16s_net* n, const F16sPlan& p, hipStream_t st, const float* planes, float* value, float* policy) {
    using G = Geo<11>;
    const int batch = p.batch;
    SmallFwdArgs S = {};
    S.planes = planes; S.stem_w = n->stem_wm; S.stem_b = n->stem_b; S.stem_inv = n->stem_inv_scale; S.f0 = n->f0;
    S.df = n->df; S.batch = batch;
    auto role = [&](F16sArgs a, int wait, int need, int done) { a.df_wait = n->df + wait; a.df_need = need; a.df_done = n->df + done; a.df_err = n->df + kDfErr; return a; };
    S.L0 = role(layer_args(n, p, 0, n->f0, nullptr, n->g[0]), kDfStem, 1, kDfL0);
    S.L1 = role(layer_args(n, p, 1, n->g[0], n->f0, n->o[0]), kDfL0, 2, kDfL1);
    S.L2 = role(layer_args(n, p, 2, n->o[0], nullptr, n->g[1]), kDfL1, 2, kDfL2);
    S.L3 = role(layer_args(n, p, 3, n->g[1], n->o[0], n->o[1]), kDfL2, 4, kDfL3);
    S.P = role(layer_args(n, p, 6, n->o[1], nullptr, n->g[3]), kDfL3, 4, kDfP);
    S.V = role(block_args<4>(n, p, n->o[1]), kDfL3, 4, kDfV);
    S.Q = role(layer_args(n, p, 7, n->g[3], n->o[1], n->o[3]), kDfP, 2, kDfQ);
    S.B5 = role(block_args<8>(n, p, n->o[3]), kDfQ, 2, kDfB5);
    S.F = VfcArgs{n->hx[0], n->hfw[0], n->hfb[0], n->v2w, n->v2b, n->hf_inv[0], value};
    constexpr size_t ldsC = Lds<G, kDist>::kScrOff + (size_t)2 * 1 * 4 * 4096;
    constexpr size_t ldsV = Lds<G, 2>::kScrOff + (size_t)2 * 2 * 4096 * 2 + 36864;
    constexpr size_t ldsB = Lds<G, 2>::kScrOff + Lay<G>::kSlotL + 36864;
    constexpr size_t lds = std::max(std::max(ldsC, ldsV), std::max(ldsB, (size_t)StemLds<G>::kBytes));
    static_assert(lds + 256 <= 160 * 1024, "LDS budget (dynamic + the value head's static reduction buffer)");
    uint64_t bit;
    if (device_bit(&bit) || dyn_lds<af_small_forward_f16s<G>>(bit, (int)lds)) return -2;
    S.xp = n->hx[1]; S.pfa = n->hfw[1]; S.pfb = n->hfb[1]; S.pf_inv = n->hf_inv[1]; S.policy = policy; S.pfx = n->pfx;
    hipLaunchKernelGGL(af_small_forward_f16s<G>, dim3(19 * batch + 3), dim3(256), lds, st, S);
    FS_HIP_OK(hipGetLastError());
    return 0;
}

int f16s_forward(f16s_net* n, const F16sPlan& p, hipStream_t st, const float* planes, float* value, float* policy) {
    if (!n || p.form == kF16sBranches || p.batch < 1 || p.batch > n->max_batch || !planes || !value || !policy) return -1;
    if (p.form == kF16sRoles) return roles_forward(n, p, st, planes, value, policy);
    const int rc = f16s_trunk(n, p, st, planes);
    return rc ? rc : paired_branches(n, p, st, value, policy);
}
int f16s_small_forward_error(f16s_net* n) {
    if (!n || !n->df) return -1;
    int e = 0;
    FS_HIP_OK(hipDeviceSynchronize());
    FS_HIP_OK(hipMemcpy(&e, n->df + kDfErr, sizeof(int), hipMemcpyDeviceToHost));
    return e;
}

int f16s_read_activation(f16s_net* n, int which, int batch, float* host) {
    if (!n || batch < 1 || batch > n->max_batch) return -1;
    if (which == 9 || which == 10) {
        const int C = which == 9 ? 4 : 16, hxp = 128 * (n->S == 11 ? 1 : 2), npix = n->S * n->S;
        const size_t pos_h = (size_t)2 * hxp * C, lo_h = (size_t)hxp * C;
        std::vector<_Float16> h((size_t)batch * pos_h);
        FS_HIP_OK(hipDeviceSynchronize());
        FS_HIP_OK(hipMemcpy(h.data(), n->hx[which - 9], h.size() * 2, hipMemcpyDeviceToHost));
        for (int b = 0; b < batch; ++b)
            for (int c = 0; c < C; ++c)
                for (int p = 0; p < npix; ++p) {
                    const size_t idx = (size_t)b * pos_h + (size_t)p * C + c;
                    host[((size_t)b * C + c) * npix + p] = (float)h[idx] + (float)h[idx + lo_h];
                }
        return C;
    }
    const char* bufs[9] = {n->f0, n->g[0], n->o[0], n->g[1], n->o[1], n->g[2], n->g[3], n->o[3], n->g[4]};
    const int chans[9] = {32, 64, 64, 128, 128, 32, 64, 64, 32};
    if (which < 0 || which > 8) return -1;
    const int C = chans[which];
    const bool s11 = n->S == 11;
    const size_t slab_h = (s11 ? Lay<Geo<11>>::kSlabH : Lay<Geo<15>>::kSlabH) / 2, half_h = slab_h / 2;
    const int rowu = s11 ? (int)Geo<11>::ROWU : (int)Geo<15>::ROWU, poff = s11 ? Geo<11>::POFF : Geo<15>::POFF, npix = n->S * n->S;
    std::vector<_Float16> h((size_t)batch * (C / 32) * slab_h);
    FS_HIP_OK(hipDeviceSynchronize());
    FS_HIP_OK(hipMemcpy(h.data(), bufs[which], h.size() * 2, hipMemcpyDeviceToHost));
    for (int b = 0; b < batch; ++b)
        for (int c = 0; c < C; ++c)
            for (int p = 0; p < npix; ++p) {
                const size_t slab = ((size_t)b * (C / 32) + c / 32) * slab_h;
                const size_t idx = slab + ((size_t)((c % 32) / 8) * rowu + p + poff) * 8 + c % 8;
                host[((size_t)b * C + c) * npix + p] = (float)h[idx] + (float)h[idx + half_h];
            }
    return C;
}

#ifdef AF_DF_TIMING
extern "C" int af_df_debug_wall(unsigned long long* host) {
    FS_HIP_OK(hipDeviceSynchronize());
    FS_HIP_OK(hipMemcpyFromSymbol(host, HIP_SYMBOL(g_df_wall), sizeof(unsigned long long) * 256 * 5));
    return 0;
}
#endif
#ifdef AF_F16S_TIMING
extern "C" int af_f16s_debug_cycles(unsigned long long* host) {
    FS_HIP_OK(hipDeviceSynchronize());
    FS_HIP_OK(hipMemcpyFromSymbol(host, HIP_SYMBOL(g_f16s_cycles), sizeof(unsigned long long) * 10 * 512 * 4 * 9));
    return 0;
}
extern "C" int af_f16s_debug_wall(unsigned long long* host) {
    FS_HIP_OK(hipDeviceSynchronize());
    FS_HIP_OK(hipMemcpyFromSymbol(host, HIP_SYMBOL(g_f16s_wall), sizeof(unsigned long long) * 10 * 512 * 2));
    return 0;
}
#endif
```

### alphafive_amd/csrc/af_engine.hip

```cpp

#include <hip/hip_runtime.h>
#include <stdint.h>
#include <stdio.h>
#include <stdlib.h>
#include <string.h>

#include <type_traits>
#include <vector>

#include "af_engine.h"
#include "af_noise.h"

typedef unsigned long long u64;

enum { PH_IDLE = 0, PH_MOVE_START = 1, PH_SEARCH = 2, PH_MOVE_DONE = 3, PH_ERROR = 4, PH_DESCENT = 5  };
enum { CT_SIMS = 0, CT_SELECTS, CT_EXPANDS, CT_TERMINALS, CT_PLIES, CT_EPISODES, CT_LSUM, CT_LEXP,
       CT_GC, CT_GC_SCANNED, CT_YIELDS, CT_STALLS, CT_N };
enum { HIST_WORK = 0, HIST_TIME = 64, HIST_MAXTIME = 96, HIST_N = 97 };

struct EngineParams {
    int G, S, C, goal, sims, upper, training, mode, node_cap, max_ply, budget, budget_hard;
    uint32_t hash_mask;
    double init_temp, tau_decay, tau_decay_r, alpha, c_puct;
    float c_puct32;
// ... 1388 lines not shown
        for (int c = 0; c < C; ++c) dst[i * W + c] = (D)src[i * C + c];
    return dst;
}

extern "C" {

int af_abi_version(void) { return AF_ABI_VERSION; }

const char* af_strerror(int code) {
    switch (code) {
        case AF_OK: return "ok";
        case AF_ERR_ARG: return "bad argument";
        case AF_ERR_HIP: return "HIP runtime error";
        case AF_ERR_NODE_CAP: return "transposition store full (raise node_cap)";
        case AF_ERR_NO_ROOT: return "get_action on a finished position";
        case AF_ERR_EP_OVERRUN: return "finished episodes not popped in time";
        case AF_ERR_STATE: return "engine state error";
        default: return "unknown error";
    }
}

int af_engine_create(const af_config* cfg, int32_t num_games, int32_t device, int32_t mode, int32_t training,
                     uint64_t seed, uint32_t first_game_id, int32_t node_cap, af_engine** out) {
    if (!cfg || !out || num_games < 1) return AF_ERR_ARG;
    const int S = cfg->board_size, C = S * S;
    if (S < 2 || C > 256 || cfg->goal < 2 || cfg->goal > S || cfg->simulation_per_step < 1) return AF_ERR_ARG;
    const int value_f64 = (mode & AF_MODE_VALUE_F64) ? 1 : 0;
    mode &= ~AF_MODE_VALUE_F64;
    if (mode != AF_MODE_SELFPLAY && mode != AF_MODE_EXTERNAL) return AF_ERR_ARG;
    if (!(cfg->dirichlet_alpha > 0.0 && cfg->dirichlet_alpha < 1.0)) return AF_ERR_ARG;
    if (cfg->upper_simulation_per_step < 1 || !(cfg->c_puct >= 0.0)) return AF_ERR_ARG;
    HIP_OK(hipSetDevice(device));
    af_engine* e = new af_engine();
    e->device = device;
    e->KW = C <= 128 ? 2 : 4;
    const int KW = e->KW, CP = 64 * KW;
    EngineParams& P = e->P;
    memset(&P, 0, sizeof(P));
    P.G = num_games; P.S = S; P.C = C; P.goal = cfg->goal;
    P.sims = cfg->simulation_per_step; P.upper = cfg->upper_simulation_per_step;
    P.training = training ? 1 : 0; P.mode = mode; P.max_ply = C; P.w64 = value_f64;
    P.budget = AF_DEFAULT_TICK_BUDGET; P.budget_hard = AF_DEFAULT_TICK_BUDGET_HARD;
    if (const char* b = getenv("AF_TICK_BUDGET")) { const int v = atoi(b); if (v > 0) P.budget = v; }
    if (const char* b = getenv("AF_TICK_BUDGET_HARD")) { const int v = atoi(b); if (v > 0) P.budget_hard = v; }
    if (P.budget_hard < P.budget) P.budget_hard = P.budget;
    if (node_cap <= 0) node_cap = mode == AF_MODE_SELFPLAY ? 4 * P.sims + 64 : 32768;
    if (node_cap < P.sims + 8) node_cap = P.sims + 8;
    P.node_cap = node_cap;
    uint32_t hcap = 64;
    while (hcap < 2u * (uint32_t)node_cap) hcap <<= 1;
    P.hash_mask = hcap - 1;
    P.init_temp = cfg->init_temp; P.tau_decay = cfg->tau_decay_rate; P.tau_decay_r = cfg->tau_decay_rate_r;
    P.alpha = cfg->dirichlet_alpha; P.c_puct = cfg->c_puct; P.c_puct32 = (float)cfg->c_puct;
    P.k0 = af_key0(seed); P.seed_hi = (uint32_t)(seed >> 32); P.first_game_id = first_game_id;
    for (int c = 0; c < C; ++c) {
        P.boardmask[c >> 6] |= 1ull << (c & 63);
        if (c % S <= S - cfg->goal) P.colmask[c >> 6] |= 1ull << (c & 63);
    }
    const size_t G = num_games;
    int rc = AF_OK;
#define A(p, n) if (rc == AF_OK) rc = dalloc(e, &P.p, (n))
    A(phase, G); A(pending, G); A(sims_left, G); A(ply, G); A(root_last, G); A(nodes, G); A(nfree, G); A(depth, G);
    A(leaf_last, G); A(leaf_slot, G); A(status, G); A(random_a, G); A(action, G); A(has_policy, G);
    A(visits, G * CP); A(policy, G * CP); A(root, G * 2 * KW); A(leaf, G * 2 * KW); A(tau, G);
    A(episode, G); A(sel, G); A(plyctr, G); A(path_node, G * CP); A(path_cell, G * CP);
    A(hash, G * hcap); A(node_key, G * node_cap * 2 * KW); A(node_sum, G * node_cap); A(free_idx, G * node_cap);
    A(edge_n, G * node_cap * CP); A(edge_p, G * node_cap * CP); A(edge_c, G * node_cap * CP);
    if (value_f64) { A(edge_w64, G * node_cap * CP); A(edge_w, 64); } else { A(edge_w, G * node_cap * CP); A(edge_w64, 8); }
    A(ep_seq, G); A(ep_popped, G); A(counters, G * CT_N); A(progress, 2); A(hist, HIST_N);
    if (mode == AF_MODE_SELFPLAY) {
        const size_t R = G * 2 * P.max_ply;
        A(ep_len, G * 2); A(ep_final, G * 2); A(rec_key, R * 2 * KW); A(rec_policy, R * C); A(rec_visits, R * C);
        A(rec_last, R); A(rec_action, R);
    }
#undef A
    if (rc == AF_OK) rc = dalloc(e, &e->stamps, (size_t)AF_STAMP_SLOTS);
    if (rc != AF_OK) { af_engine_destroy(e); return rc; }
    std::vector<int32_t> ph(G, mode == AF_MODE_SELFPLAY ? PH_MOVE_START : PH_IDLE), rl(G, -1);
    std::vector<double> tau(G, cfg->init_temp);
    HIP_OK(hipMemcpy(P.phase, ph.data(), G * 4, hipMemcpyHostToDevice));
    HIP_OK(hipMemcpy(P.root_last, rl.data(), G * 4, hipMemcpyHostToDevice));
    HIP_OK(hipMemcpy(P.tau, tau.data(), G * 8, hipMemcpyHostToDevice));
    e->h_i32.resize(G); e->h_i32b.resize(G); e->h_ct.resize(G * CT_N);
    *out = e;
    return AF_OK;
}

void af_engine_destroy(af_engine* e) {
    if (!e) return;
    (void)hipSetDevice(e->device);
    for (void* p : e->allocs) (void)hipFree(p);
    if (e->stage_dev) (void)hipFree(e->stage_dev);
    delete e;
}

int32_t af_engine_num_games(const af_engine* e) { return e->P.G; }
int32_t af_engine_cells(const af_engine* e) { return e->P.C; }
int32_t af_engine_key_words(const af_engine* e) { return 2 * e->KW; }
int32_t af_engine_max_plies(const af_engine* e) { return e->P.max_ply; }

int af_engine_tick(af_engine* e, void* stream, const float* policy_dev, const float* value_dev, float* planes_dev) {
    if (!e || !planes_dev) return AF_ERR_ARG;
    hipStream_t st = (hipStream_t)stream;
    WITH_FLAG(e->memo, MEMO_, WITH_KW(e->KW, WITH_FLAG(e->P.w64, W64_,
        hipLaunchKernelGGL((af_tick_kernel<KW_, W64_, MEMO_>), dim3(e->P.G), dim3(64), 0, st, e->P, policy_dev, value_dev, planes_dev))));
    HIP_OK(hipGetLastError());
    return AF_OK;
}

int af_engine_memo_enable(af_engine* e, int32_t log2_buckets, int32_t max_stones) {
    if (!e || e->memo || log2_buckets < 4 || log2_buckets > 28 || max_stones < 0) return AF_ERR_ARG;
    HIP_OK(hipSetDevice(e->device));
    EngineParams& P = e->P;
    const size_t NE = (size_t)4 << log2_buckets, CP = 64 * (size_t)e->KW, MK = 4 * (size_t)e->KW;
    int rc = AF_OK;
    if (rc == AF_OK) rc = dalloc(e, &P.memo_key, NE * MK);
    if (rc == AF_OK) rc = dalloc(e, &P.memo_pv, NE * CP);
    if (rc == AF_OK) rc = dalloc(e, &P.memo_val, NE);
    if (rc == AF_OK) rc = dalloc(e, &P.memo_lock, NE);
    if (rc == AF_OK) rc = dalloc(e, &P.memo_stats, (size_t)MEMO_N);
    if (rc != AF_OK) return rc;
    P.memo_bucket_mask = (uint32_t)((1ull << log2_buckets) - 1ull);
    P.memo_max_stones = max_stones;
    P.memo_epoch = 1;
    P.memo_budget = P.budget < 6 ? P.budget : 6;
    if (const char* b = getenv("AF_MEMO_BUDGET")) { const int v = atoi(b); if (v > 0) { P.memo_budget = v; e->memo_budget_fixed = true; } }
    e->memo_entries = NE;
    e->memo = true;
    return AF_OK;
}

int af_engine_memo_insert(af_engine* e, void* stream, const float* policy_dev, const float* value_dev) {
    if (!e || !e->memo || !policy_dev || !value_dev) return AF_ERR_ARG;
    hipStream_t st = (hipStream_t)stream;
    WITH_KW(e->KW, hipLaunchKernelGGL((af_memo_insert_kernel<KW_>), dim3(e->P.G), dim3(64), 0, st, e->P, policy_dev, value_dev));
    HIP_OK(hipGetLastError());
    return AF_OK;
}

int af_engine_memo_clear(af_engine* e, void* stream) {
    if (!e || !e->memo) return AF_ERR_ARG;
    hipStream_t st = (hipStream_t)stream;
    if (e->P.memo_epoch == 0xffffffffu) {
        HIP_OK(hipMemsetAsync(e->P.memo_key, 0, e->memo_entries * 4 * (size_t)e->KW * 8, st));
        e->P.memo_epoch = 1;
    } else {
        ++e->P.memo_epoch;
    }
    return AF_OK;
}

int64_t af_engine_memo_epoch(af_engine* e) { return (e && e->memo) ? (int64_t)e->P.memo_epoch : 0; }

int af_engine_memo_stats(af_engine* e, void* stream, uint64_t* out) {
    if (!e || !e->memo || !out) return AF_ERR_ARG;
    hipStream_t st = (hipStream_t)stream;
    HIP_OK(hipMemcpyAsync(out, e->P.memo_stats, (size_t)MEMO_N * 8, hipMemcpyDeviceToHost, st));
    HIP_OK(hipStreamSynchronize(st));
    out[MEMO_N] = (uint64_t)e->memo_entries;
    return AF_OK;
}

int af_engine_status(af_engine* e, void* stream, int32_t* status_host) {
    if (!e || !status_host) return AF_ERR_ARG;
    hipStream_t st = (hipStream_t)stream;
    HIP_OK(hipMemcpyAsync(status_host, e->P.status, (size_t)e->P.G * 4, hipMemcpyDeviceToHost, st));
    HIP_OK(hipStreamSynchronize(st));
    for (int g = 0; g < e->P.G; ++g) if (status_host[g] < 0) return status_host[g];
    return AF_OK;
}

int af_engine_set_training(af_engine* e, int32_t training) {
    if (!e) return AF_ERR_ARG;
    e->P.training = training ? 1 : 0;
    return AF_OK;
}

int af_engine_set_simulations(af_engine* e, int32_t sims, int32_t upper) {
    if (!e || sims < 1 || upper < 1 || sims + 8 > e->P.node_cap) return AF_ERR_ARG;
    e->P.sims = sims;
    e->P.upper = upper;
    return AF_OK;
}

int af_engine_set_root(af_engine* e, int32_t game, const uint64_t* key, int32_t last_cell, int32_t random_a,
                       int32_t reset_tree) {
    if (!e || !key || game < 0 || game >= e->P.G || e->P.mode != AF_MODE_EXTERNAL) return AF_ERR_ARG;
    if (last_cell < -1 || last_cell >= e->P.C) return AF_ERR_ARG;
    HIP_OK(hipDeviceSynchronize());
    return af_engine_set_roots(e, nullptr, 1, &game, key, &last_cell, &random_a, &reset_tree);
}

int af_engine_set_roots(af_engine* e, void* stream, int32_t n, const int32_t* games, const uint64_t* keys, const int32_t* last_cells,
                        const int32_t* random_a, const int32_t* reset_tree) {
    if (!e || e->P.mode != AF_MODE_EXTERNAL || n < 0 || (n > 0 && (!games || !keys || !last_cells))) return AF_ERR_ARG;
    if (n == 0) return AF_OK;
    EngineParams& P = e->P;
    const int KW = e->KW, KW2 = 2 * KW;
    std::vector<int32_t> req((size_t)4 * n);
    for (int i = 0; i < n; ++i) {
        if (games[i] < 0 || games[i] >= P.G || last_cells[i] < -1 || last_cells[i] >= P.C) return AF_ERR_ARG;
        if (!valid_position(P, KW, keys + (size_t)i * KW2)) return AF_ERR_ARG;
        req[4 * i] = games[i]; req[4 * i + 1] = last_cells[i]; req[4 * i + 2] = random_a ? random_a[i] : 0; req[4 * i + 3] = reset_tree ? reset_tree[i] : 0;
    }
    hipStream_t st = (hipStream_t)stream;
    const size_t rb = (size_t)4 * n * 4, kb = (size_t)n * KW2 * 8;
    if (int rc = stage_reserve(e, rb + kb)) return rc;
    HIP_OK(hipMemcpyAsync(e->stage_dev, req.data(), rb, hipMemcpyHostToDevice, st));
    HIP_OK(hipMemcpyAsync(e->stage_dev + rb, keys, kb, hipMemcpyHostToDevice, st));
    hipLaunchKernelGGL(af_set_roots_kernel, dim3(n), dim3(64), 0, st, P, n, (const int32_t*)e->stage_dev, (const u64*)(e->stage_dev + rb), KW2);
    HIP_OK(hipGetLastError());
    HIP_OK(hipStreamSynchronize(st));
    return AF_OK;
}

int af_engine_move_results(af_engine* e, void* stream, int32_t n, const int32_t* games, int32_t* action_cells, int32_t* has_policy,
                           float* policies, int32_t* visits, double* taus) {
    if (!e || n < 0 || (n > 0 && (!games || !action_cells))) return AF_ERR_ARG;
    if (n == 0) return AF_OK;
    EngineParams& P = e->P;
    for (int i = 0; i < n; ++i) if (games[i] < 0 || games[i] >= P.G) return AF_ERR_ARG;
    hipStream_t st = (hipStream_t)stream;
    const int C = P.C, R = 8 + 2 * C, CP = 64 * e->KW;
    const size_t gb = (size_t)n * 4, ob = (size_t)n * R * 4;
    if (int rc = stage_reserve(e, gb + ob)) return rc;
    HIP_OK(hipMemcpyAsync(e->stage_dev, games, gb, hipMemcpyHostToDevice, st));
    hipLaunchKernelGGL(af_move_results_kernel, dim3(n), dim3(64), 0, st, P, n, (const int32_t*)e->stage_dev, (int32_t*)(e->stage_dev + gb), CP);
    HIP_OK(hipGetLastError());
    std::vector<int32_t> out((size_t)n * R);
    HIP_OK(hipMemcpyAsync(out.data(), e->stage_dev + gb, ob, hipMemcpyDeviceToHost, st));
    HIP_OK(hipStreamSynchronize(st));
    for (int i = 0; i < n; ++i) {
        const int32_t* o = out.data() + (size_t)i * R;
        if (o[2] != 0) return o[2];
        action_cells[i] = o[0];
        if (has_policy) has_policy[i] = o[1];
        if (policies) memcpy(policies + (size_t)i * C, o + 8, (size_t)C * 4);
        if (visits) memcpy(visits + (size_t)i * C, o + 8 + C, (size_t)C * 4);
        if (taus) { const uint64_t tb = (uint64_t)(uint32_t)o[3] | ((uint64_t)(uint32_t)o[4] << 32); memcpy(taus + i, &tb, 8); }
    }
    return AF_OK;
}

int af_engine_move_result(af_engine* e, int32_t game, int32_t* action_cell, int32_t* has_policy, float* policy,
                          int32_t* visits, double* tau) {
    if (!e || game < 0 || game >= e->P.G) return AF_ERR_ARG;
    HIP_OK(hipDeviceSynchronize());
    int32_t cell;
    const int rc = af_engine_move_results(e, nullptr, 1, &game, &cell, has_policy, policy, visits, tau);
    if (rc == AF_OK && action_cell) *action_cell = cell;
    return rc;
}

int64_t af_engine_pack_ints(const af_engine* e, int32_t max_episodes, int32_t max_plies) {
    if (!e || max_episodes < 0 || max_plies < 0) return AF_ERR_ARG;
    const int64_t R = 4 * e->KW + 2 * e->P.C + 2;
    return 4 + (int64_t)max_episodes * 5 + (int64_t)max_plies * R;
}

int af_engine_pack_episodes(af_engine* e, void* stream, int32_t max_episodes, int32_t max_plies, int32_t* out_dev) {
    if (!e || e->P.mode != AF_MODE_SELFPLAY || max_episodes < 1 || max_plies < 1 || !out_dev) return AF_ERR_ARG;
    hipStream_t st = (hipStream_t)stream;
    hipLaunchKernelGGL(af_pack_scan, dim3(1), dim3(1024), 0, st, e->P, max_episodes, max_plies, out_dev);
    hipLaunchKernelGGL(af_pack_copy, dim3(max_episodes), dim3(256), 0, st, e->P, max_episodes, out_dev);
    HIP_OK(hipGetLastError());
    return AF_OK;
}

int af_engine_pop_episodes(af_engine* e, void* stream, int32_t cap, int32_t* meta, float* final_value,
                           uint64_t* keys, float* policies, int32_t* visits, int32_t* lasts, int32_t* actions) {
    if (!e || e->P.mode != AF_MODE_SELFPLAY || cap < 0) return AF_ERR_ARG;
    if (cap == 0) return 0;
    EngineParams& P = e->P;
    hipStream_t st = (hipStream_t)stream;
    const int C = P.C, KW2 = 2 * e->KW, MP = P.max_ply, R = 2 * KW2 + 2 * C + 2;
    const int max_plies = cap * MP > (1 << 18) ? (1 << 18) : cap * MP;
    int rc = stage_reserve(e, (size_t)af_engine_pack_ints(e, cap, max_plies) * 4);
    if (rc) return rc;
    int32_t* pack_dev = (int32_t*)e->stage_dev;
    rc = af_engine_pack_episodes(e, stream, cap, max_plies, pack_dev);
    if (rc) return rc;
    const size_t head = 4 + (size_t)cap * 5;
    e->pack_host.resize(head);
    HIP_OK(hipMemcpyAsync(e->pack_host.data(), pack_dev, head * 4, hipMemcpyDeviceToHost, st));
    HIP_OK(hipStreamSynchronize(st));
    const int n = e->pack_host[0], np = e->pack_host[1];
    if (n <= 0) return 0;
    e->pack_host.resize(head + (size_t)np * R);
    HIP_OK(hipMemcpyAsync(e->pack_host.data() + head, pack_dev + head, (size_t)np * R * 4, hipMemcpyDeviceToHost, st));
    HIP_OK(hipStreamSynchronize(st));
    const int32_t* H = e->pack_host.data();
    for (int i = 0; i < n; ++i) {
        const int32_t* m = H + 4 + (size_t)i * 4;
        const int T = m[2], poff = m[3];
        meta[4 * i] = m[0]; meta[4 * i + 1] = m[1]; meta[4 * i + 2] = T; meta[4 * i + 3] = 0;
        memcpy(final_value + i, H + 4 + (size_t)cap * 4 + i, 4);
        for (int t = 0; t < T; ++t) {
            const int32_t* r = H + head + (size_t)(poff + t) * R;
            memcpy(keys + ((size_t)i * MP + t) * KW2, r, (size_t)KW2 * 8);
            memcpy(policies + ((size_t)i * MP + t) * C, r + 2 * KW2, (size_t)C * 4);
            memcpy(visits + ((size_t)i * MP + t) * C, r + 2 * KW2 + C, (size_t)C * 4);
            lasts[(size_t)i * MP + t] = r[2 * KW2 + 2 * C];
            actions[(size_t)i * MP + t] = r[2 * KW2 + 2 * C + 1];
        }
    }
    return n;
// ... 307 lines not shown
```

### alphafive_amd/csrc/af_net.hip

```cpp

#include <hip/hip_runtime.h>
#include <stdint.h>
#include <stdio.h>
#include <string.h>

#include <vector>

#include "af_net.h"
#include "af_conv_f16s.h"

typedef float f32x16 __attribute__((ext_vector_type(16)));
typedef float f4u __attribute__((ext_vector_type(4), aligned(4)));
typedef float f2u __attribute__((ext_vector_type(2), aligned(4)));
typedef float f2a __attribute__((ext_vector_type(2)));

__device__ __forceinline__ float elu1(float x) { return x > 0.0f ? x : __expf(x) - 1.0f; }

struct WinoArgs {
    const float* in;
    const float* u;
    const float* in2;
    const float* u2;
    const float* bias;
    float* out;
// ... 653 lines not shown
    for (float* a : n->act) (void)hipFree(a);
    if (n->upd_max_host) (void)hipHostFree(n->upd_max_host);
    if (n->branch_stream) (void)hipStreamDestroy(n->branch_stream);
    if (n->ev_trunk) (void)hipEventDestroy(n->ev_trunk);
    if (n->ev_value) (void)hipEventDestroy(n->ev_value);
    delete n;
}

int af_net_set_variable(af_net* n, const char* name, const float* data, int64_t count) {
    if (!n || !name || !data) return AF_NET_ERR_ARG;
    const int v = var_index(name);
    if (v < 0 || (int64_t)var_count(v, n->HW) != count) return AF_NET_ERR_NAME;
    memcpy(n->image.data() + var_offset(v, n->HW), data, (size_t)count * sizeof(float));
    n->set[v] = true;
    n->ready = false;
    return AF_NET_OK;
}

int af_net_finalize(af_net* n) {
    if (!n) return AF_NET_ERR_ARG;
    for (bool s : n->set) if (!s) return AF_NET_ERR_STATE;
    NET_HIP_OK(hipSetDevice(n->device));
    NET_HIP_OK(hipDeviceSynchronize());
    if (n->f16s && f16s_reset_roles(n->f16s)) return AF_NET_ERR_HIP;
    NET_HIP_OK(hipMemcpy(n->stage, n->image.data(), n->image.size() * sizeof(float), hipMemcpyHostToDevice));
    const float* src[kVars];
    for (int i = 0; i < kVars; ++i) src[i] = n->stage + var_offset(i, n->HW);
    const int rc = pack_from_device(n, nullptr, src);
    if (rc) return rc;
    NET_HIP_OK(hipStreamSynchronize(nullptr));
    return AF_NET_OK;
}

int af_net_update_device(af_net* n, void* stream, const char* const* tf_names, const float* const* dev_ptrs, const int64_t* counts,
                         int32_t nvars) {
    if (!n || !tf_names || !dev_ptrs || !counts) return AF_NET_ERR_ARG;
    if (!n->packed) return AF_NET_ERR_STATE;
    if (nvars != kVars) return AF_NET_ERR_ARG;
    const float* src[kVars] = {};
    for (int i = 0; i < nvars; ++i) {
        if (!tf_names[i] || !dev_ptrs[i]) return AF_NET_ERR_ARG;
        const int v = var_index(tf_names[i]);
        if (v < 0 || (int64_t)var_count(v, n->HW) != counts[i]) return AF_NET_ERR_NAME;
        if (src[v]) return AF_NET_ERR_ARG;
        src[v] = dev_ptrs[i];
    }
    hipStream_t st = (hipStream_t)stream;
    hipStreamCaptureStatus cap = hipStreamCaptureStatusNone;
    NET_HIP_OK(hipStreamIsCapturing(st, &cap));
    if (cap != hipStreamCaptureStatusNone) return AF_NET_ERR_STATE;
    NET_HIP_OK(hipSetDevice(n->device));
    const int rc = pack_from_device(n, st, src);
    if (rc) return rc;
    for (bool& s : n->set) s = false;
    return AF_NET_OK;
}

int64_t af_net_debug_weights(af_net* n, int32_t index, void* host_out, int64_t cap_bytes) {
    if (!n || index < 0 || !n->packed) return AF_NET_ERR_ARG;
    const void* p = nullptr;
    size_t bytes = 0;
    if (index < kWeightBufs) { p = n->w[index]; bytes = weight_count(index, n->HW) * sizeof(float); }
    else if (!n->f16s || f16s_weight_buffer(n->f16s, index - kWeightBufs, &p, &bytes)) return AF_NET_ERR_ARG;
    if (!host_out) return (int64_t)bytes;
    if (cap_bytes < (int64_t)bytes) return AF_NET_ERR_ARG;
    NET_HIP_OK(hipSetDevice(n->device));
    NET_HIP_OK(hipDeviceSynchronize());
    NET_HIP_OK(hipMemcpy(host_out, p, bytes, hipMemcpyDeviceToHost));
    return (int64_t)bytes;
}

int32_t af_net_debug_scales(af_net* n, float* host_out, int32_t cap) {
    if (!n || !host_out || cap < 0) return AF_NET_ERR_ARG;
    return n->f16s ? f16s_scales(n->f16s, host_out, cap) : 0;
}

}

static struct {
    int conv = 5;
    int branch = 1;
    int phead = 1;
    int f16s_bits = 0;
    int fhead = 1;
} g_tune;

extern "C" int af_net_tune(int32_t key, int32_t value) {
    if (key == 0) { if (value != 1 && value != 5) return AF_NET_ERR_ARG; g_tune.conv = value; return AF_NET_OK; }
    if (key == 4) { g_tune.branch = value; return AF_NET_OK; }
    if (key == 5) { g_tune.phead = value; return AF_NET_OK; }
    if (key == 7) { g_tune.f16s_bits = value; return AF_NET_OK; }
    if (key == 9) { g_tune.fhead = value ? 1 : 0; return AF_NET_OK; }
    return AF_NET_ERR_ARG;
}

static void launch_wino(hipStream_t st, const af_net* n, int batch, const float* in, const float* u, int cin,
                        const float* in2, const float* u2, int cin2, const float* bias, float* out, int cout) {
    WinoArgs a;
    a.in = in; a.u = u; a.in2 = in2; a.u2 = u2; a.bias = bias; a.out = out;
    a.cin = cin; a.cin2 = cin2; a.cout = cout; a.T = n->T; a.S = n->S; a.WP = n->WP; a.PP = n->PP;
    a.ntiles = batch * n->T * n->T;
    const int ntb = (a.ntiles + 31) / 32;
    const int ngrp8 = (((ntb + 3) / 4) + 7) / 8 * 8;
    hipLaunchKernelGGL(af_conv_wino, dim3(ngrp8 * (cout / 32)), dim3(256), 0, st, a);
}
static void launch_wino_block(hipStream_t st, const af_net* n, int batch, int i, const float* in) {
    const NetBlock& b = kBlocks[i];
    float *g = n->act[kG + 2 * i], *o = n->act[kO + 2 * i];
    launch_wino(st, n, batch, in, n->w[kWino1 + i], b.cin, nullptr, nullptr, 0, n->w[kConv1B + i], g, b.cout);
    launch_wino(st, n, batch, g, n->w[kWino2 + i], b.cout, in, n->w[kWinoR + i], b.cin, n->w[kSumB + i], o, b.cout);
}

static void launch_value_head(hipStream_t st, const af_net* n, int batch, const float* o3, float* value) {
    hipLaunchKernelGGL(af_value_head, dim3((batch + VPB - 1) / VPB), dim3(256), 0, st, o3, n->w[kVcW], n->w[kVcB], n->w[kV1W], n->w[kV1B],
                       n->w[kV2W], n->w[kV2B], value, batch, n->S, n->WP, n->PP);
}
static void launch_policy_head(hipStream_t st, const af_net* n, int batch, const float* o5, float* policy) {
    const int HW = n->HW, K = 16 * HW, KS = K + ((2 - K % 32) + 32) % 32;
    const bool mfma = HW <= 128 && g_tune.phead;
    const int ppb = mfma ? 16 : HW <= 128 ? 8 : 4;
    const size_t lds = mfma ? (size_t)16 * KS * 4 : ((size_t)16 * HW * ppb + 512 + 4 * ppb) * 4;
    const auto head = mfma ? af_policy_head_mfma : HW <= 128 ? af_policy_head<8> : af_policy_head<4>;
    hipLaunchKernelGGL(head, dim3((batch + ppb - 1) / ppb), dim3(256), lds, st, o5, n->w[kPcW], n->w[kPcB], n->w[kPfW], n->w[kPfB], policy,
                       batch, n->S, n->WP, n->PP);
}

static int fork_value(af_net* n, hipStream_t st, hipStream_t vs) {
    if (vs != st) { NET_HIP_OK(hipEventRecord(n->ev_trunk, st)); NET_HIP_OK(hipStreamWaitEvent(vs, n->ev_trunk, 0)); }
    return AF_NET_OK;
}
static int value_done(af_net* n, hipStream_t st, hipStream_t vs) { if (vs != st) NET_HIP_OK(hipEventRecord(n->ev_value, vs)); return AF_NET_OK; }
static int join_value(af_net* n, hipStream_t st, hipStream_t vs) {
    if (vs != st) NET_HIP_OK(hipStreamWaitEvent(st, n->ev_value, 0));
    NET_HIP_OK(hipGetLastError());
    return AF_NET_OK;
}

static int forward_wino(af_net* n, hipStream_t st, const float* planes, int batch, float* policy, float* value) {
    float *f0 = n->act[kF0], *o1 = n->act[kO], *o2 = n->act[kO + 2], *o3 = n->act[kO + 4], *o4 = n->act[kO + 6], *o5 = n->act[kO + 8];
    hipLaunchKernelGGL(af_stem_conv, dim3(batch), dim3(256), 0, st, planes, n->w[kStemW], n->w[kStemB], f0, n->S, n->WP, n->PP);
    launch_wino_block(st, n, batch, 0, f0);
    launch_wino_block(st, n, batch, 1, o1);
    const hipStream_t vs = g_tune.branch ? n->branch_stream : st;
    if (const int rc = fork_value(n, st, vs)) return rc;
    launch_wino_block(vs, n, batch, 2, o2);
    launch_value_head(vs, n, batch, o3, value);
    if (const int rc = value_done(n, st, vs)) return rc;
    launch_wino_block(st, n, batch, 3, o2);
    launch_wino_block(st, n, batch, 4, o4);
    launch_policy_head(st, n, batch, o5, policy);
    return join_value(n, st, vs);
}

static int forward_f16s(af_net* n, hipStream_t st, const float* planes, int batch, float* policy, float* value) {
    const bool fhead = g_tune.fhead;
    const F16sPlan plan = f16s_plan(n->f16s, batch, g_tune.f16s_bits, fhead);
    if (plan.form != kF16sBranches) return f16s_forward(n->f16s, plan, st, planes, value, policy) ? AF_NET_ERR_HIP : AF_NET_OK;
    float *o3 = n->act[kO + 4], *o5 = n->act[kO + 8];
    if (f16s_trunk(n->f16s, plan, st, planes)) return AF_NET_ERR_HIP;
    const hipStream_t vs = g_tune.branch == 2 ? n->branch_stream : st;
    if (const int rc = fork_value(n, st, vs)) return rc;
    if (f16s_value_branch(n->f16s, plan, vs, o3, n->WP, n->PP, value)) return AF_NET_ERR_HIP;
    if (!fhead) launch_value_head(vs, n, batch, o3, value);
    if (const int rc = value_done(n, st, vs)) return rc;
    if (f16s_policy_branch(n->f16s, plan, st, o5, n->WP, n->PP, policy)) return AF_NET_ERR_HIP;
    if (!fhead) launch_policy_head(st, n, batch, o5, policy);
    return join_value(n, st, vs);
}

extern "C" {

int af_net_forward(af_net* n, void* stream, const float* planes, int32_t batch, float* policy, float* value) {
    if (!n || !planes || !policy || !value || batch < 1 || batch > n->max_batch) return AF_NET_ERR_ARG;
    if (!n->ready) return AF_NET_ERR_STATE;
    if (g_tune.conv == 5 && n->f16s) return forward_f16s(n, (hipStream_t)stream, planes, batch, policy, value);
    return forward_wino(n, (hipStream_t)stream, planes, batch, policy, value);
}

int af_net_debug_activation(af_net* n, int32_t which, int32_t batch, float* host_out) {
    if (!n || !host_out) return AF_NET_ERR_ARG;
    if (which >= 16) {
        const bool stored = which >= 32;
        const int i = which - (stored ? 32 : 16);
        if (i >= kActs || batch < 1 || batch > n->max_batch) return AF_NET_ERR_ARG;
        const int C = act_channels(i), S = n->S, WP = n->WP, PP = n->PP;
        const size_t count = (size_t)batch * C * PP;
        NET_HIP_OK(hipSetDevice(n->device));
        NET_HIP_OK(hipDeviceSynchronize());
        if (stored) { NET_HIP_OK(hipMemcpy(host_out, n->act[i], count * sizeof(float), hipMemcpyDeviceToHost)); return C; }
        std::vector<float> h(count);
        NET_HIP_OK(hipMemcpy(h.data(), n->act[i], count * sizeof(float), hipMemcpyDeviceToHost));
        for (size_t bc = 0; bc < (size_t)batch * C; ++bc)
            for (int y = 0; y < S; ++y) memcpy(host_out + (bc * S + y) * S, h.data() + bc * PP + (y + 1) * WP + 1, S * sizeof(float));
        return C;
    }
    if (!n->f16s) return AF_NET_ERR_ARG;
    const int c = f16s_read_activation(n->f16s, which, batch, host_out);
    return c < 0 ? AF_NET_ERR_ARG : c;
}

int af_net_small_forward_error(af_net* n) {
    if (!n || !n->f16s) return AF_NET_ERR_ARG;
    return f16s_small_forward_error(n->f16s);
}

int64_t af_net_flops_per_position(const af_net* n) {
    const int64_t HW = n->HW;
    int64_t mac = 75 * 32 * HW;
    for (const NetBlock& b : kBlocks) mac += ((int64_t)9 * b.cin * b.cout + (int64_t)9 * b.cout * b.cout + (int64_t)b.cin * b.cout) * HW;
    mac += 32 * 4 * HW + 4 * HW * 64 + 64 + 32 * 16 * HW + 16 * HW * HW;
    return 2 * mac;
}

}
```

### alphafive_amd/engine.py

```python
import ctypes as C
import os

import numpy as np

_PKG = os.path.dirname(os.path.abspath(__file__))
_LIBPATH = os.environ.get("AF_HIP_LIB") or os.path.join(_PKG, "_lib", "libaf_hip.so")

MODE_SELFPLAY, MODE_EXTERNAL = 0, 1
MODE_VALUE_F64 = 0x100
STATUS_IDLE, STATUS_NEED_EVAL, STATUS_MOVE_DONE, STATUS_YIELD = 0, 1, 2, 3
STAMP_SLOTS = 64
BLACK_WIN, WHITE_WIN, DRAW = 1, -1, 0

CFG_ATTRS = ("board_size", "goal", "simulation_per_step", "upper_simulation_per_step", "init_temp", "gamma",
             "tau_decay_rate", "tau_decay_rate_r", "dirichlet_alpha", "c_puct")


class AfConfig(C.Structure):
    _fields_ = [("board_size", C.c_int32), ("goal", C.c_int32), ("simulation_per_step", C.c_int32),
                ("upper_simulation_per_step", C.c_int32), ("init_temp", C.c_double), ("gamma", C.c_double),
                ("tau_decay_rate", C.c_double), ("tau_decay_rate_r", C.c_double), ("dirichlet_alpha", C.c_double),
                ("c_puct", C.c_double)]

    @classmethod
    def from_cfg(cls, cfg):
        return cls(*[getattr(cfg, a) for a in CFG_ATTRS])


class EngineError(RuntimeError):
    pass


_lib = None


def lib():
    global _lib
    if _lib is None:
        if not os.path.exists(_LIBPATH):
            raise EngineError(f"{_LIBPATH} not found: build the HIP engine first "
                              f"(python -m alphafive_amd.build). There is no CPU fallback.")
        import torch
        L = C.CDLL(_LIBPATH)
        vp = C.c_void_p
        i32p, f32p, u64p, u8p = (C.POINTER(C.c_int32), C.POINTER(C.c_float), C.POINTER(C.c_uint64),
                                 C.POINTER(C.c_uint8))
        L.af_abi_version.restype = C.c_int
        L.af_strerror.restype = C.c_char_p
        L.af_strerror.argtypes = [C.c_int]
        L.af_engine_create.argtypes = [C.POINTER(AfConfig), C.c_int32, C.c_int32, C.c_int32, C.c_int32, C.c_uint64,
                                       C.c_uint32, C.c_int32, C.POINTER(vp)]
        L.af_engine_destroy.argtypes = [vp]
        L.af_engine_destroy.restype = None
        for fn in ("af_engine_num_games", "af_engine_cells", "af_engine_key_words", "af_engine_max_plies"):
            getattr(L, fn).argtypes = [vp]
            getattr(L, fn).restype = C.c_int32
        L.af_engine_tick.argtypes = [vp, vp, vp, vp, vp]
        L.af_engine_status.argtypes = [vp, vp, i32p]
        L.af_engine_set_root.argtypes = [vp, C.c_int32, u64p, C.c_int32, C.c_int32, C.c_int32]
        L.af_engine_move_result.argtypes = [vp, C.c_int32, i32p, i32p, f32p, i32p, C.POINTER(C.c_double)]
        L.af_engine_set_training.argtypes = [vp, C.c_int32]
        L.af_engine_set_simulations.argtypes = [vp, C.c_int32, C.c_int32]
        L.af_engine_set_roots.argtypes = [vp, vp, C.c_int32, i32p, u64p, i32p, i32p, i32p]
        L.af_engine_move_results.argtypes = [vp, vp, C.c_int32, i32p, i32p, i32p, f32p, i32p, C.POINTER(C.c_double)]
        L.af_engine_pop_episodes.argtypes = [vp, vp, C.c_int32, i32p, f32p, u64p, f32p, i32p, i32p, i32p]
        L.af_engine_pack_ints.argtypes = [vp, C.c_int32, C.c_int32]
        L.af_engine_pack_ints.restype = C.c_int64
        L.af_engine_pack_episodes.argtypes = [vp, vp, C.c_int32, C.c_int32, vp]
        L.af_engine_counters.argtypes = [vp, vp, u64p]
        L.af_engine_tree_w64.argtypes = [vp, C.c_int32, C.c_int32, C.POINTER(C.c_double)]
        L.af_engine_set_tree_w64.argtypes = [vp, C.c_int32, C.c_int32, C.POINTER(C.c_double)]
        L.af_engine_progress.argtypes = [vp, vp, u64p]
        L.af_engine_progress_async.argtypes = [vp, vp, vp]
        L.af_engine_stamp.argtypes = [vp, vp, C.c_int32]
        L.af_engine_stamps_async.argtypes = [vp, vp, vp]
        L.af_engine_tick_histogram.argtypes = [vp, vp, u64p, C.c_int32]
        L.af_engine_set_tick_budget.argtypes = [vp, C.c_int32]
        L.af_engine_memo_enable.argtypes = [vp, C.c_int32, C.c_int32]
        L.af_engine_memo_insert.argtypes = [vp, vp, vp, vp]
        L.af_engine_memo_clear.argtypes = [vp, vp]
        L.af_engine_memo_stats.argtypes = [vp, vp, u64p]
        L.af_engine_memo_epoch.argtypes = [vp]
        L.af_engine_memo_epoch.restype = C.c_int64
        L.af_match_create.argtypes = [vp, vp, C.POINTER(vp)]
        L.af_match_destroy.argtypes = [vp]
        L.af_match_destroy.restype = None
        L.af_match_start.argtypes = [vp, vp, C.c_int32, C.c_int32]
        L.af_match_step.argtypes = [vp, vp]
        L.af_match_progress_async.argtypes = [vp, vp, vp]
        L.af_match_results.argtypes = [vp, vp, i32p, i32p, i32p]
        L.af_engine_tree_dump.argtypes = [vp, C.c_int32, C.c_int32, u64p, i32p, i32p, f32p, f32p, u8p]
        L.af_engine_load_tree.argtypes = [vp, C.c_int32, C.c_int32, u64p, i32p, i32p, f32p, f32p, u8p]
        L.af_state_to_key.argtypes = [C.c_char_p, C.c_int32, u64p]
        L.af_key_to_state.argtypes = [u64p, C.c_int32, C.c_char_p, C.c_int32]
        _lib = L
    return _lib


def _check(rc, what):
    if rc < 0:
        raise EngineError(f"{what}: {lib().af_strerror(rc).decode()} (code {rc})")
    return rc


def _p(a, ct):
    return a.ctypes.data_as(C.POINTER(ct))


def key_words(S):
    return 4 if S * S <= 128 else 8


def state_to_key(state, S):
    key = np.zeros(key_words(S), np.uint64)
    _check(lib().af_state_to_key(state.encode(), S, _p(key, C.c_uint64)), "af_state_to_key")
    return key


def key_to_state(key, S):
    key = np.ascontiguousarray(key, np.uint64)
    out = C.create_string_buffer(288)
    _check(lib().af_key_to_state(_p(key, C.c_uint64), S, out, 288), "af_key_to_state")
    return out.value.decode()


COUNTER_NAMES = ("sims", "selects", "expands", "terminals", "plies", "episodes", "legal_sum", "legal_sum_expand",
                 "nodes", "collector_runs", "collector_scanned", "yields", "stalls")


class Engine:

    def __init__(self, cfg, num_games, device=0, mode=MODE_SELFPLAY, training=True, seed=0, first_game_id=0,
                 node_cap=0, value_f64=False):
        self._h = C.c_void_p()
        self.cfg = AfConfig.from_cfg(cfg) if not isinstance(cfg, AfConfig) else cfg
        self.value_f64 = bool(value_f64) or bool(mode & MODE_VALUE_F64)
        mode = (mode & ~MODE_VALUE_F64) | (MODE_VALUE_F64 if self.value_f64 else 0)
        _check(lib().af_engine_create(C.byref(self.cfg), num_games, device, mode, int(training), seed, first_game_id,
                                      node_cap, C.byref(self._h)), "af_engine_create")
        self.G = num_games
        self.S = self.cfg.board_size
        self.C = self.S * self.S
        self.KW2 = lib().af_engine_key_words(self._h)
        self.max_plies = lib().af_engine_max_plies(self._h)
        self.mode = mode & ~MODE_VALUE_F64
        self.device = device
        self._status = np.zeros(num_games, np.int32)
        self._params = {"training": int(bool(training)), "sims": int(self.cfg.simulation_per_step),
                        "upper": int(self.cfg.upper_simulation_per_step), "tick_budget": None}

    def close(self):
        if getattr(self, "_h", None):
            lib().af_engine_destroy(self._h)
            self._h = None

    __del__ = close

    def tick(self, policy_ptr, value_ptr, planes_ptr, stream=None):
        _check(lib().af_engine_tick(self._h, stream, policy_ptr, value_ptr, planes_ptr), "af_engine_tick")

    def status(self, stream=None):
        rc = lib().af_engine_status(self._h, stream, _p(self._status, C.c_int32))
        _check(rc, "engine status")
        return self._status

    def params_key(self):
        p = self._params
        return (p["training"], p["sims"], p["upper"], p["tick_budget"], p.get("memo_epoch"), p.get("memo"))

    def set_training(self, training):
        _check(lib().af_engine_set_training(self._h, int(training)), "af_engine_set_training")
        self._params["training"] = int(bool(training))

    def set_simulations(self, sims, upper):
        _check(lib().af_engine_set_simulations(self._h, int(sims), int(upper)), "af_engine_set_simulations")
        self._params["sims"], self._params["upper"] = int(sims), int(upper)

    def set_root(self, game, key, last_cell=-1, random_a=False, reset_tree=False):
        key = np.ascontiguousarray(key, np.uint64)
        _check(lib().af_engine_set_root(self._h, game, _p(key, C.c_uint64), last_cell, int(random_a), int(reset_tree)),
               "af_engine_set_root")

    def move_result(self, game):
        a, hp, tau = C.c_int32(-1), C.c_int32(0), C.c_double(0)
        pol = np.zeros(self.C, np.float32)
        vis = np.zeros(self.C, np.int32)
        _check(lib().af_engine_move_result(self._h, game, C.byref(a), C.byref(hp), _p(pol, C.c_float),
                                           _p(vis, C.c_int32), C.byref(tau)), "af_engine_move_result")
        return a.value, (pol if hp.value else None), vis, tau.value

    def set_roots(self, games, keys, last_cells, random_a=False, reset_tree=False, stream=None):
        n = len(games)
        g = np.ascontiguousarray(games, np.int32)
        k = np.ascontiguousarray(keys, np.uint64).reshape(n, self.KW2)
        lc = np.ascontiguousarray(last_cells, np.int32)
        ra = np.ascontiguousarray(np.broadcast_to(np.asarray(random_a, np.int32), (n,)))
        rt = np.ascontiguousarray(np.broadcast_to(np.asarray(reset_tree, np.int32), (n,)))
        _check(lib().af_engine_set_roots(self._h, stream, n, _p(g, C.c_int32), _p(k, C.c_uint64), _p(lc, C.c_int32),
                                         _p(ra, C.c_int32), _p(rt, C.c_int32)), "af_engine_set_roots")

    def move_results(self, games, stream=None):
        n = len(games)
        g = np.ascontiguousarray(games, np.int32)
        act, hp = np.zeros(n, np.int32), np.zeros(n, np.int32)
        pol, vis, tau = np.zeros((n, self.C), np.float32), np.zeros((n, self.C), np.int32), np.zeros(n, np.float64)
        _check(lib().af_engine_move_results(self._h, stream, n, _p(g, C.c_int32), _p(act, C.c_int32), _p(hp, C.c_int32),
                                            _p(pol, C.c_float), _p(vis, C.c_int32), _p(tau, C.c_double)), "af_engine_move_results")
        return act, hp, pol, vis, tau

    def counters(self, stream=None):
        out = np.zeros(len(COUNTER_NAMES), np.uint64)
        _check(lib().af_engine_counters(self._h, stream, _p(out, C.c_uint64)), "af_engine_counters")
        return {k: int(v) for k, v in zip(COUNTER_NAMES, out)}

    def tick_histogram(self, stream=None, reset=False):
        out = np.zeros(97, np.uint64)
        _check(lib().af_engine_tick_histogram(self._h, stream, _p(out, C.c_uint64), int(reset)), "tick_histogram")
        return dict(selects=out[:64].astype(np.int64), wave_us=out[64:96].astype(np.int64),
                    max_wave_us=float(out[96]) * 0.01)

    def memo_enable(self, log2_buckets=18, max_stones=5):
        _check(lib().af_engine_memo_enable(self._h, int(log2_buckets), int(max_stones)), "af_engine_memo_enable")
        kw = self.KW2 // 2
        self.memo_bytes = (4 << int(log2_buckets)) * (32 * kw + 256 * kw + 12)
        self._params["memo"] = (int(log2_buckets), int(max_stones))
        self._params["memo_epoch"] = int(lib().af_engine_memo_epoch(self._h))

    @property
    def memo(self):
        return self._params.get("memo")

    def memo_insert(self, policy_ptr, value_ptr, stream=None):
        _check(lib().af_engine_memo_insert(self._h, stream, policy_ptr, value_ptr), "af_engine_memo_insert")

    def memo_clear(self, stream=None):
        _check(lib().af_engine_memo_clear(self._h, stream), "af_engine_memo_clear")
        self._params["memo_epoch"] = int(lib().af_engine_memo_epoch(self._h))

    def memo_stats(self, stream=None):
        out = np.zeros(6, np.uint64)
        _check(lib().af_engine_memo_stats(self._h, stream, _p(out, C.c_uint64)), "af_engine_memo_stats")
        return {k: int(v) for k, v in zip(("launches", "probes", "hits", "inserts", "replaced", "entries"), out)}

    def set_tick_budget(self, selects_per_launch):
        _check(lib().af_engine_set_tick_budget(self._h, int(selects_per_launch)), "af_engine_set_tick_budget")
        self._params["tick_budget"] = int(selects_per_launch)

    def progress(self, stream=None):
        out = np.zeros(2, np.uint64)
        _check(lib().af_engine_progress(self._h, stream, _p(out, C.c_uint64)), "af_engine_progress")
        return int(out[0]), int(out[1])

    def progress_async(self, out_ptr, stream=None):
        _check(lib().af_engine_progress_async(self._h, stream, out_ptr), "af_engine_progress_async")

    def stamp(self, slot, stream=None):
        _check(lib().af_engine_stamp(self._h, stream, int(slot)), "af_engine_stamp")

    def stamps_async(self, out_ptr, stream=None):
        _check(lib().af_engine_stamps_async(self._h, stream, out_ptr), "af_engine_stamps_async")

    def tree_dump(self, game):
        cnt = _check(lib().af_engine_tree_dump(self._h, game, 0, None, None, None, None, None, None), "tree_dump")
        keys = np.zeros((cnt, self.KW2), np.uint64)
        sum_n = np.zeros(cnt, np.int32)
        n = np.zeros((cnt, self.C), np.int32)
        w = np.zeros((cnt, self.C), np.float32)
        p = np.zeros((cnt, self.C), np.float32)
        f = np.zeros((cnt, self.C), np.uint8)
        if cnt:
            _check(lib().af_engine_tree_dump(self._h, game, cnt, _p(keys, C.c_uint64), _p(sum_n, C.c_int32),
                                             _p(n, C.c_int32), _p(w, C.c_float), _p(p, C.c_float), _p(f, C.c_uint8)),
                   "tree_dump")
            if self.value_f64:
                w = np.zeros((cnt, self.C), np.float64)
                _check(lib().af_engine_tree_w64(self._h, game, cnt, _p(w, C.c_double)), "af_engine_tree_w64")
        return dict(keys=keys, sum_n=sum_n, n=n, w=w, p=p, f32=f)

    def load_tree(self, game, dump):
        cnt = len(dump["sum_n"])
        arr = {k: np.ascontiguousarray(dump[k], t) for k, t in (("keys", np.uint64), ("sum_n", np.int32), ("n", np.int32),
                                                                 ("w", np.float32), ("p", np.float32), ("f32", np.uint8))}
        _check(lib().af_engine_load_tree(self._h, game, cnt, _p(arr["keys"], C.c_uint64), _p(arr["sum_n"], C.c_int32),
                                         _p(arr["n"], C.c_int32), _p(arr["w"], C.c_float), _p(arr["p"], C.c_float),
                                         _p(arr["f32"], C.c_uint8)), "af_engine_load_tree")
        if self.value_f64:
            w64 = np.ascontiguousarray(dump["w"], np.float64)
            _check(lib().af_engine_set_tree_w64(self._h, game, cnt, _p(w64, C.c_double)), "af_engine_set_tree_w64")

    def pack_ints(self, max_eps, max_plies):
        return int(_check(lib().af_engine_pack_ints(self._h, max_eps, max_plies), "af_engine_pack_ints"))

    def pack_episodes(self, out_ptr, max_eps, max_plies, stream=None):
        _check(lib().af_engine_pack_episodes(self._h, stream, max_eps, max_plies, out_ptr), "af_engine_pack_episodes")


def unpack_episodes(buf, max_eps):
    buf = np.ascontiguousarray(buf, np.int32)
    n, _, K, Cc = (int(x) for x in buf[:4])
    R = 2 * K + 2 * Cc + 2
    head = 4 + 5 * max_eps
    out = []
    for i in range(n):
        g, seq, T, p0 = (int(x) for x in buf[4 + 4 * i:8 + 4 * i])
        rec = buf[head + p0 * R:head + (p0 + T) * R].reshape(T, R)
        out.append(dict(game=g, seq=seq, T=T, final_value=float(buf[4 + 4 * max_eps + i:5 + 4 * max_eps + i].view(np.float32)[0]),
                        keys=np.ascontiguousarray(rec[:, :2 * K]).view(np.uint64).reshape(T, K).copy(),
                        policies=np.ascontiguousarray(rec[:, 2 * K:2 * K + Cc]).view(np.float32).copy(),
                        visits=rec[:, 2 * K + Cc:2 * K + 2 * Cc].copy(),
                        lasts=rec[:, 2 * K + 2 * Cc].copy(), actions=rec[:, 2 * K + 2 * Cc + 1].copy()))
    return out


def packed_used_ints(hdr, max_eps):
    n_plies, K, Cc = int(hdr[1]), int(hdr[2]), int(hdr[3])
    return 4 + 5 * max_eps + n_plies * (2 * K + 2 * Cc + 2)


def assemble_episode(raw, S, gamma):
    from . import utils
    T = raw["T"]
    value = float(raw["final_value"])
    if T % 2 == 1:
        value = -value
    weights = utils.construct_weights(T, gamma=gamma)
    rec = []
    for t in range(T):
        la = None if raw["lasts"][t] < 0 else (int(raw["lasts"][t]) // S, int(raw["lasts"][t]) % S)
        rec.append((key_to_state(raw["keys"][t], S), raw["policies"][t].reshape(S, S).copy(), la, value, weights[t]))
        value = -value
    last_value = rec[-1][-2]
    if last_value == 0.0:
        result = DRAW
    elif T % 2 == 1:
        result = BLACK_WIN
    else:
        result = WHITE_WIN
    return rec, result


def resolve_weights_version(pv, explicit=None):
    if explicit is not None:
        return (explicit if callable(explicit) else (lambda: explicit)), False
    ver = getattr(pv, "weights_version", None)
    if callable(ver):
        return ver, False
    owner = getattr(pv, "__self__", None)
    if owner is not None and hasattr(owner, "version"):
        return (lambda: owner.version), False
    return None, hasattr(pv, "bind_outputs")


class SelfPlayEngine:

    def __init__(self, cfg, num_games, pv_device, device=0, seed=0, first_game_id=0, training=True, node_cap=0,
                 value_f64=False, weights_version=None, eval_memo=None):
        import torch
        if not torch.cuda.is_available():
            raise EngineError("SelfPlayEngine needs a HIP device (torch.cuda.is_available() is False)")
        self.torch = torch
        self.cfg = cfg
        self.dev = torch.device("cuda", device)
        torch.cuda.set_device(self.dev)
        self.engine = Engine(cfg, num_games, device=device, mode=MODE_SELFPLAY, training=training, seed=seed,
                             first_game_id=first_game_id, node_cap=node_cap, value_f64=value_f64)
        S = cfg.board_size
        self.G, self.S, self.C = num_games, S, S * S
        self.planes = torch.zeros((num_games, 3, S, S), dtype=torch.float32, device=self.dev)
        self.policy = torch.zeros((num_games, S * S), dtype=torch.float32, device=self.dev)
        self.value = torch.zeros((num_games,), dtype=torch.float32, device=self.dev)
        self.pv_device = pv_device
        self._weights_version = self._resolve_weights_version(weights_version)
        if hasattr(pv_device, "bind_outputs"):
            pv_device.bind_outputs(self.policy, self.value)
        self._memo_version = None
        if eval_memo:
            if self._weights_version is None:
                raise EngineError("eval_memo: the evaluator exposes no weights_version (the memo could not tell when to forget); "
                                  "pass SelfPlayEngine(..., weights_version=lambda: net.version)")
            self.engine.memo_enable(**({} if eval_memo is True else dict(eval_memo)))
            self._memo_version = self._weights_version()
        self.ticks = 0
        self._boxes = {}
        self._graph = None
        self._prog_host, self._prog_events, self._prog_turn, self._prog_replays = None, None, 0, 0
        self.replay_events = []
        self._graph_stamped, self._stamp_host, self._stamp_event, self._stamp_pending, self.stamp_samples = None, None, None, False, []

    def tick(self, stamp_base=None):
        torch = self.torch
        stream = torch.cuda.current_stream(self.dev).cuda_stream
        if stamp_base is not None:
            self.engine.stamp(stamp_base, stream)
        memo = self.engine.memo is not None
        if memo:
            ver = self._weights_version()
            if ver != self._memo_version:
                self.engine.memo_clear(stream)
                self._memo_version = ver
        self.engine.tick(self.policy.data_ptr(), self.value.data_ptr(), self.planes.data_ptr(), stream)
        if stamp_base is not None:
            self.engine.stamp(stamp_base + 1, stream)
        p, v = self.pv_device(self.planes)
        if p.data_ptr() != self.policy.data_ptr():
            self.policy.copy_(p.reshape(self.G, self.C))
        if v.data_ptr() != self.value.data_ptr():
            self.value.copy_(v.reshape(self.G))
        if memo:
            self.engine.memo_insert(self.policy.data_ptr(), self.value.data_ptr(), stream)
        if stamp_base is not None:
            self.engine.stamp(stamp_base + 2, stream)
        self.ticks += 1

    def run_ticks(self, n, check_every=0):
        for i in range(n):
            self.tick()
            if check_every and (i + 1) % check_every == 0:
                self.check()

    def _resolve_weights_version(self, explicit):
        ver, missing = resolve_weights_version(self.pv_device, explicit)
        if missing:
            self._weights_version_missing = True
        return ver

    def _graph_key(self, n):
        ver = self._weights_version
        return (int(n), self.engine.params_key(), ver() if ver is not None else None)

    def run_ticks_graph(self, n=16, timed=False, stamped=False):
        torch = self.torch
        if getattr(self, "_weights_version_missing", False):
            raise EngineError("run_ticks_graph: pv_device takes bind_outputs but exposes no weights_version (a replayed graph "
                              "would keep evaluating with stale weights); pass SelfPlayEngine(..., weights_version=lambda: net.version)")
        key = self._graph_key(n)
        if stamped:
            if 3 * n > STAMP_SLOTS:
                raise EngineError("run_ticks_graph(stamped=True): at most %d ticks per replay" % (STAMP_SLOTS // 3))
            if self._graph_stamped is None or self._graph_stamped[0] != key:
                self._graph_stamped = None
                if self._graph is None or self._graph[0] != key:
                    self.run_ticks_graph(n)
                if self._stamp_host is None:
                    self._stamp_host = torch.zeros(STAMP_SLOTS, dtype=torch.int64, pin_memory=True)
                    self._stamp_event = torch.cuda.Event()
                torch.cuda.synchronize(self.dev)
                g = torch.cuda.CUDAGraph()
                with torch.cuda.graph(g, capture_error_mode="thread_local"):
                    for i in range(n):
                        self.tick(stamp_base=3 * i)
                    st = torch.cuda.current_stream(self.dev).cuda_stream
                    self.engine.stamps_async(self._stamp_host.data_ptr(), st)
                    self.engine.progress_async(self._prog_host.data_ptr(), st)
                self.ticks -= n
                self._graph_stamped = (self._graph_key(n), g, n)
            if self._stamp_pending:
                self._collect_stamps()
            self._graph_stamped[1].replay()
            self._stamp_event.record(torch.cuda.current_stream(self.dev))
            self._stamp_pending = True
            self.ticks += n
            self._prog_turn ^= 1
            self._prog_events[self._prog_turn].record(torch.cuda.current_stream(self.dev))
            self._prog_replays += 1
            return
        if self._graph is None or self._graph[0] != key:
            self._graph = None
            if self._prog_host is None:
                self._prog_host = torch.zeros(2, dtype=torch.int64, pin_memory=True)
                self._prog_events = [torch.cuda.Event(), torch.cuda.Event()]
            self.tick()
            torch.cuda.synchronize(self.dev)
            g = torch.cuda.CUDAGraph()
            with torch.cuda.graph(g, capture_error_mode="thread_local"):
                for _ in range(n):
                    self.tick()
                st = torch.cuda.current_stream(self.dev).cuda_stream
                self.engine.progress_async(self._prog_host.data_ptr(), st)
            self.ticks -= n
            self._graph = (self._graph_key(n), g)
        if timed:
            e0, e1 = torch.cuda.Event(enable_timing=True), torch.cuda.Event(enable_timing=True)
            e0.record(torch.cuda.current_stream(self.dev))
        self._graph[1].replay()
        if timed:
            e1.record(torch.cuda.current_stream(self.dev))
            self.replay_events.append((n, e0, e1))
        self.ticks += n
        self._prog_turn ^= 1
        self._prog_events[self._prog_turn].record(torch.cuda.current_stream(self.dev))
        self._prog_replays += 1

    def _collect_stamps(self):
        self._stamp_event.synchronize()
        t = self._stamp_host.numpy().astype(np.int64)[:3 * self._graph_stamped[2]].reshape(-1, 3)
        self.stamp_samples.append(np.stack([(t[:, 1] - t[:, 0]) * 1e-5, (t[:, 2] - t[:, 1]) * 1e-5], axis=1))
        self._stamp_pending = False

    def read_stamps(self):
        if self._stamp_pending:
            self._collect_stamps()
        return np.concatenate(self.stamp_samples) if self.stamp_samples else np.zeros((0, 2))

    def progress_lagged(self):
        if self._prog_replays < 2:
            return 0, 0
        self._prog_events[self._prog_turn ^ 1].synchronize()
        return int(self._prog_host[0]), int(self._prog_host[1])

    def check(self):
        stream = self.torch.cuda.current_stream(self.dev).cuda_stream
        return self.engine.status(stream)

    def counters(self):
        return self.engine.counters(self.torch.cuda.current_stream(self.dev).cuda_stream)

    def progress(self):
        return self.engine.progress(self.torch.cuda.current_stream(self.dev).cuda_stream)

    def _pack_plies(self, cap):
        return max(cap * 40, int(self.engine.max_plies))

    def _outbox(self, cap):
        box = self._boxes.get(cap)
        if box is None:
            torch = self.torch
            max_plies = self._pack_plies(cap)
            ints = self.engine.pack_ints(cap, max_plies)
            box = dict(cap=cap, max_plies=max_plies, buf=torch.zeros(ints, dtype=torch.int32, pin_memory=True),
                       event=torch.cuda.Event(), posted=False)
            self._boxes[cap] = box
        return box

    def post_episodes(self, cap=256):
        box = self._outbox(cap)
        if box["posted"]:
            raise EngineError("post_episodes: the previous post has not been collected")
        stream = self.torch.cuda.current_stream(self.dev)
        self.engine.pack_episodes(box["buf"].data_ptr(), cap, box["max_plies"], stream.cuda_stream)
        box["event"].record(stream)
        box["posted"] = True
        return box

    def collect_episodes(self, cap=256, unpack=True):
        box = self._outbox(cap)
        if not box["posted"]:
            return [] if unpack else None
        box["event"].synchronize()
        box["posted"] = False
        return unpack_episodes(box["buf"].numpy(), cap) if unpack else box["buf"].numpy()

    def pop_raw(self, cap=256):
        self.post_episodes(cap)
        return self.collect_episodes(cap)

    def post_episodes_device(self, cap=256):
        key = ("dev", cap)
        buf = self._boxes.get(key)
        if buf is None:
            buf = self.torch.zeros(self.engine.pack_ints(cap, self._pack_plies(cap)), dtype=self.torch.int32, device=self.dev)
            self._boxes[key] = buf
        self.engine.pack_episodes(buf.data_ptr(), cap, self._pack_plies(cap), self.torch.cuda.current_stream(self.dev).cuda_stream)
        return buf

    def pop_episodes(self, cap=256):
        return [assemble_episode(r, self.S, self.cfg.gamma) for r in self.pop_raw(cap)]

    def close(self):
        self.engine.close()
```

### alphafive_amd/net_hip.py

```python
import ctypes as C
import os

import numpy as np
import torch

_PKG = os.path.dirname(os.path.abspath(__file__))
_LIBPATH = os.environ.get("AF_NET_LIB") or os.path.join(_PKG, "_lib", "libaf_net.so")
_lib = None


class NetError(RuntimeError):
    pass


def lib():
    global _lib
    if _lib is None:
        if not os.path.exists(_LIBPATH):
            raise ImportError(f"{_LIBPATH} not built (python -m alphafive_amd.build)")
        import torch
        L = C.CDLL(_LIBPATH)
        vp = C.c_void_p
        L.af_net_create.argtypes = [C.c_int32, C.c_int32, C.c_int32, C.POINTER(vp)]
        L.af_net_destroy.argtypes = [vp]
        L.af_net_destroy.restype = None
        L.af_net_set_variable.argtypes = [vp, C.c_char_p, C.POINTER(C.c_float), C.c_int64]
        L.af_net_finalize.argtypes = [vp]
        L.af_net_forward.argtypes = [vp, vp, vp, C.c_int32, vp, vp]
        L.af_net_update_device.argtypes = [vp, vp, C.POINTER(C.c_char_p), C.POINTER(vp), C.POINTER(C.c_int64), C.c_int32]
        L.af_net_debug_weights.argtypes = [vp, C.c_int32, vp, C.c_int64]
        L.af_net_debug_weights.restype = C.c_int64
        L.af_net_debug_scales.argtypes = [vp, C.POINTER(C.c_float), C.c_int32]
        L.af_net_debug_scales.restype = C.c_int32
        L.af_net_flops_per_position.argtypes = [vp]
        L.af_net_flops_per_position.restype = C.c_int64
        L.af_net_debug_activation.argtypes = [vp, C.c_int32, C.c_int32, C.POINTER(C.c_float)]
        L.af_net_small_forward_error.argtypes = [vp]
        L.af_net_strerror.argtypes = [C.c_int]
        L.af_net_strerror.restype = C.c_char_p
        _lib = L
    return _lib


def _check(rc, what):
    if rc < 0:
        raise NetError(f"{what}: {lib().af_net_strerror(rc).decode()} (code {rc})")


class HipNet(object):

    def __init__(self, variables, board_size, max_batch, device):
        self.S, self.max_batch, self.device = board_size, max_batch, torch.device(device)
        self._h = C.c_void_p()
        self._version = 0
        idx = self.device.index if self.device.index is not None else torch.cuda.current_device()
        _check(lib().af_net_create(board_size, max_batch, idx, C.byref(self._h)), "af_net_create")
        self.load(variables)
        self.flops_per_position = int(lib().af_net_flops_per_position(self._h))
        self.policy = torch.empty((max_batch, board_size * board_size), dtype=torch.float32, device=self.device)
        self.value = torch.empty((max_batch,), dtype=torch.float32, device=self.device)

    def load(self, variables):
        for name, arr in variables.items():
            a = np.ascontiguousarray(arr, np.float32)
            _check(lib().af_net_set_variable(self._h, name.encode(), a.ctypes.data_as(C.POINTER(C.c_float)), a.size),
                   f"af_net_set_variable({name})")
        _check(lib().af_net_finalize(self._h), "af_net_finalize")
        self._version += 1

    def load_device(self, tensors):
        names, ptrs, counts = [], [], []
        for name, t in tensors.items():
            if not (torch.is_tensor(t) and t.is_cuda and t.dtype == torch.float32 and t.is_contiguous()):
                raise NetError(f"load_device({name}): a contiguous float32 tensor on {self.device} is required")
            if t.device.index != (self.device.index if self.device.index is not None else torch.cuda.current_device()):
                raise NetError(f"load_device({name}): tensor on {t.device}, handle on {self.device}")
            names.append(name.encode())
            ptrs.append(t.data_ptr())
            counts.append(t.numel())
        n = len(names)
        stream = torch.cuda.current_stream(self.device).cuda_stream
        _check(lib().af_net_update_device(self._h, stream, (C.c_char_p * n)(*names), (C.c_void_p * n)(*ptrs), (C.c_int64 * n)(*counts), n),
               "af_net_update_device")
        self._version += 1

    def debug_weights(self):
        out = []
        while True:
            size = lib().af_net_debug_weights(self._h, len(out), None, 0)
            if size < 0:
                return out
            buf = np.empty(size, np.uint8)
            _check(lib().af_net_debug_weights(self._h, len(out), buf.ctypes.data_as(C.c_void_p), size), "af_net_debug_weights")
            out.append(buf)

    def debug_scales(self):
        buf = np.zeros(64, np.float32)
        n = lib().af_net_debug_scales(self._h, buf.ctypes.data_as(C.POINTER(C.c_float)), buf.size)
        _check(n, "af_net_debug_scales")
        return buf[:n].copy()

    ACTIVATIONS = {"f0": (0, 32), "g1": (1, 64), "o1": (2, 64), "g2": (3, 128), "o2": (4, 128), "g3": (5, 32), "g4": (6, 64),
                   "o4": (7, 64), "g5": (8, 32), "vconv": (9, 4), "pconv": (10, 16)}

    def debug_activation(self, which, batch):
        idx, chans = self.ACTIVATIONS[which] if isinstance(which, str) else next(v for v in self.ACTIVATIONS.values() if v[0] == which)
        out = np.empty((batch, chans, self.S * self.S), np.float32)
        c = lib().af_net_debug_activation(self._h, idx, batch, out.ctypes.data_as(C.POINTER(C.c_float)))
        _check(c, "af_net_debug_activation")
        if c != chans:
            raise NetError(f"af_net_debug_activation({idx}) returned {c} channels, expected {chans}")
        return out

    ACTIVATIONS_FP32 = {"f0": (0, 32), "g1": (1, 64), "o1": (2, 64), "g2": (3, 128), "o2": (4, 128), "g3": (5, 32), "o3": (6, 32),
                        "g4": (7, 64), "o4": (8, 64), "g5": (9, 32), "o5": (10, 32)}

    def debug_activation_fp32(self, name, batch, padded=False):
        idx, chans = self.ACTIVATIONS_FP32[name]
        WP = 2 * ((self.S + 1) // 2) + 2
        out = np.empty((batch, chans, (WP * WP + 15) // 16 * 16 if padded else self.S * self.S), np.float32)
        c = lib().af_net_debug_activation(self._h, (32 if padded else 16) + idx, batch, out.ctypes.data_as(C.POINTER(C.c_float)))
        _check(c, "af_net_debug_activation")
        if c != chans:
            raise NetError(f"af_net_debug_activation({(32 if padded else 16) + idx}) returned {c} channels, expected {chans}")
        return out

    def weights_version(self):
        return self._version

    def bind_outputs(self, policy, value):
        assert policy.is_contiguous() and value.is_contiguous() and policy.dtype == torch.float32
        assert policy.shape[0] >= self.max_batch or policy.shape[0] == value.shape[0]
        self.policy, self.value = policy, value

    def __call__(self, planes):
        B = planes.shape[0]
        assert B <= self.max_batch and planes.is_contiguous() and planes.dtype == torch.float32
        stream = torch.cuda.current_stream(self.device).cuda_stream
        _check(lib().af_net_forward(self._h, stream, planes.data_ptr(), B, self.policy.data_ptr(), self.value.data_ptr()),
               "af_net_forward")
        return self.policy[:B], self.value[:B]

    def small_forward_error(self):
        return int(lib().af_net_small_forward_error(self._h))

    def close(self):
        if getattr(self, "_h", None):
            try:
                lib().af_net_destroy(self._h)
            except Exception:
                pass
            self._h = None

    __del__ = close


def make_eval(resnet):
    if resnet.device.type != "cuda" or not (3 <= resnet.board_size <= 15):
        return None
    lib()
    state = {"net": None, "out": None, "version": None}

    def pv(planes):
        B = planes.shape[0]
        if state["net"] is None or state["net"].max_batch < B:
            if state["net"] is not None:
                state["net"].close()
            state["net"] = HipNet(resnet.variables, resnet.board_size, B, resnet.device)
            state["version"] = getattr(resnet, "version", None)
            if state["out"] is not None and state["out"][0].shape[0] >= B:
                state["net"].bind_outputs(*state["out"])
        elif state["version"] != getattr(resnet, "version", None):
            version = getattr(resnet, "version", None)
            snap = resnet.device_snapshot() if hasattr(resnet, "device_snapshot") else None
            if snap is not None:
                tensors, event = snap
                stream = torch.cuda.current_stream(resnet.device)
                stream.wait_event(event)
                state["net"].load_device(tensors)
                for t in tensors.values():
                    t.record_stream(stream)
            else:
                state["net"].load(resnet.variables)
            state["version"] = version
        return state["net"](planes)

    def bind_outputs(policy, value):
        state["out"] = (policy, value)
        if state["net"] is not None and policy.shape[0] >= state["net"].max_batch:
            state["net"].bind_outputs(policy, value)

    def close():
        if state["net"] is not None:
            state["net"].close()
            state["net"] = None

    pv.bind_outputs = bind_outputs
    pv.close = close
    pv.weights_version = lambda: getattr(resnet, "version", None)
    return pv


_SPLIT_MAC_PER_PIXEL = sum(9 * ci * co + 9 * co * co + ci * co for ci, co in ((32, 64), (64, 128), (128, 32), (128, 64), (64, 32)))
_SPLIT_BYTES_PER_POSITION = (28 * 16384 + 17 * 15488 + 2 * (4 + 16) * 121 * 2 * 2 + 3 * 121 * 4 + 122 * 4)


_conv_mode = 5


def roofline_info(board_size=11):
    if board_size == 15 and _conv_mode == 5:
        return {"backend": "hip (af_conv_f16s.hip on 15x15: two half-board pseudo-positions per board, fp16 split operands, fp32 "
                           "accumulation; MFMA stem and fused heads as on 11x11)",
                "kernel": "af_net_forward = af_stem_mfma_f16s<Geo<15>> + 10x af_conv_f16s<Geo<15>> (the last conv of each branch also "
                          "applies the head's 1x1 convolution) + af_value_fc_f16s<Geo<15>> + af_policy_fc_f16s<Geo<15>> (whole "
                          "forward timed)",
                "peak_tflops": 2500.0, "issued_flop_per_position": 2 * 3 * _SPLIT_MAC_PER_PIXEL * 256,
                "algorithmic_bytes_per_position": (30 * 2 * 20480 + 19 * 30720 + 2 * 2 * 2 * 16384 + 2 * (4 + 16) * 225 * 2 * 2 + 3 * 225 * 4 + 226 * 4)}
    if board_size == 11 and _conv_mode == 5:
        return {"backend": "hip (af_conv_f16s.hip: stem, convs and heads on v_mfma_f32_32x32x16_f16 with fp16 split operands and "
                           "fp32 accumulation; convs weight-stationary with an LDS-DMA slab ring)",
                "kernel": "af_net_forward = af_stem_mfma_f16s + 6x af_conv_f16s + 2x af_block_f16s (blocks 3 and 5: both convolutions "
                          "and the head's 1x1 convolution in one kernel, the intermediate in LDS) + af_value_fc_f16s + af_policy_fc_f16s "
                          "(whole forward timed; the convolution kernels carry 99 % of the algorithmic FLOPs, each MAC issued as 3 fp16 MFMA MACs)",
                "peak_tflops": 2500.0, "issued_flop_per_position": 2 * 3 * _SPLIT_MAC_PER_PIXEL * 121,
                "algorithmic_bytes_per_position": _SPLIT_BYTES_PER_POSITION}
    return {"backend": "hip (af_net.hip: fp32 MFMA Winograd F(2x2,3x3) convs, fused transforms/bias/ELU/residual)",
            "kernel": "af_net_forward = af_stem_conv + 10x af_conv_wino + af_value_head + af_policy_head "
                      "(whole forward timed; af_conv_wino carries 97 % of the algorithmic FLOPs; achieved = "
                      "direct-convolution FLOPs / time, the MFMAs issued are 2.25x fewer on the 3x3 layers)",
            "peak_tflops": 157.3}


def tune(key, value):
    global _conv_mode
    lib().af_net_tune.argtypes = [C.c_int32, C.c_int32]
    _check(lib().af_net_tune(key, value), "af_net_tune")
    if key == 0:
        _conv_mode = int(value)
```

### include/af_engine.h

```cpp
#ifndef AF_ENGINE_H
#define AF_ENGINE_H

#include <stdint.h>

#ifdef __cplusplus
extern "C" {
#endif

#define AF_ABI_VERSION 6

#define AF_MODE_SELFPLAY 0
#define AF_MODE_EXTERNAL 1
#define AF_MODE_VALUE_F64 0x100

#define AF_STATUS_IDLE      0
#define AF_STATUS_NEED_EVAL 1
#define AF_STATUS_MOVE_DONE 2
#define AF_STATUS_YIELD     3

#define AF_DEFAULT_TICK_BUDGET 8
#define AF_DEFAULT_TICK_BUDGET_HARD 12

#define AF_OK 0
#define AF_ERR_ARG        (-1)
#define AF_ERR_HIP        (-2)
#define AF_ERR_NODE_CAP   (-3)
#define AF_ERR_NO_ROOT    (-4)
#define AF_ERR_EP_OVERRUN (-5)
#define AF_ERR_STATE      (-6)

typedef struct {
    int32_t board_size;
    int32_t goal;
    int32_t simulation_per_step;
    int32_t upper_simulation_per_step;
    double init_temp;
    double gamma;
    double tau_decay_rate;
    double tau_decay_rate_r;
    double dirichlet_alpha;
    double c_puct;
} af_config;

typedef struct af_engine af_engine;

int af_engine_create(const af_config* cfg, int32_t num_games, int32_t device, int32_t mode, int32_t training,
                     uint64_t seed, uint32_t first_game_id, int32_t node_cap, af_engine** out);
void af_engine_destroy(af_engine* e);

int32_t af_engine_num_games(const af_engine* e);
int32_t af_engine_cells(const af_engine* e);
int32_t af_engine_key_words(const af_engine* e);
int32_t af_engine_max_plies(const af_engine* e);

int af_engine_tick(af_engine* e, void* stream, const float* policy_dev, const float* value_dev, float* planes_dev);

int af_engine_status(af_engine* e, void* stream, int32_t* status_host);

int af_engine_set_root(af_engine* e, int32_t game, const uint64_t* key, int32_t last_cell, int32_t random_a,
                       int32_t reset_tree);
int af_engine_move_result(af_engine* e, int32_t game, int32_t* action_cell, int32_t* has_policy, float* policy,
                          int32_t* visits, double* tau);
int af_engine_set_training(af_engine* e, int32_t training);
int af_engine_set_simulations(af_engine* e, int32_t simulation_per_step, int32_t upper_simulation_per_step);

int af_engine_set_roots(af_engine* e, void* stream, int32_t n, const int32_t* games, const uint64_t* keys, const int32_t* last_cells,
                        const int32_t* random_a, const int32_t* reset_tree);
int af_engine_move_results(af_engine* e, void* stream, int32_t n, const int32_t* games, int32_t* action_cells, int32_t* has_policy,
                           float* policies, int32_t* visits, double* taus);

int64_t af_engine_pack_ints(const af_engine* e, int32_t max_episodes, int32_t max_plies);
int af_engine_pack_episodes(af_engine* e, void* stream, int32_t max_episodes, int32_t max_plies, int32_t* out);

int af_engine_pop_episodes(af_engine* e, void* stream, int32_t cap, int32_t* meta, float* final_value,
                           uint64_t* keys, float* policies, int32_t* visits, int32_t* lasts, int32_t* actions);

#define AF_NUM_COUNTERS 13
int af_engine_counters(af_engine* e, void* stream, uint64_t* out);

#define AF_MEMO_STATS 6
int af_engine_memo_enable(af_engine* e, int32_t log2_buckets, int32_t max_stones);
int af_engine_memo_insert(af_engine* e, void* stream, const float* policy_dev, const float* value_dev);
int af_engine_memo_clear(af_engine* e, void* stream);
int af_engine_memo_stats(af_engine* e, void* stream, uint64_t* out);
int64_t af_engine_memo_epoch(af_engine* e);

#define AF_HIST_WORDS 97
int af_engine_tick_histogram(af_engine* e, void* stream, uint64_t* out, int32_t reset);

int af_engine_set_tick_budget(af_engine* e, int32_t selects_per_launch);

int af_engine_progress(af_engine* e, void* stream, uint64_t* out);
int af_engine_progress_async(af_engine* e, void* stream, uint64_t* out_pinned);

#define AF_STAMP_SLOTS 64
int af_engine_stamp(af_engine* e, void* stream, int32_t slot);
int af_engine_stamps_async(af_engine* e, void* stream, uint64_t* out_pinned);

#define AF_MATCH_UNFINISHED (-1)
#define AF_MATCH_WIN0 0
#define AF_MATCH_WIN1 1
#define AF_MATCH_DRAW 2
typedef struct af_match af_match;
int af_match_create(af_engine* e0, af_engine* e1, af_match** out);
void af_match_destroy(af_match* m);
int af_match_start(af_match* m, void* stream, int32_t n_games, int32_t max_plies);
int af_match_step(af_match* m, void* stream);
int af_match_progress_async(af_match* m, void* stream, uint64_t* out_pinned);
int af_match_results(af_match* m, void* stream, int32_t* result, int32_t* lengths, int32_t* moves);

int af_engine_tree_dump(af_engine* e, int32_t game, int32_t cap, uint64_t* keys, int32_t* sum_n, int32_t* n,
                        float* w, float* p, uint8_t* f32);

int af_engine_load_tree(af_engine* e, int32_t game, int32_t count, const uint64_t* keys, const int32_t* sum_n,
                        const int32_t* n, const float* w, const float* p, const uint8_t* f32);

int af_engine_tree_w64(af_engine* e, int32_t game, int32_t cap, double* w);
int af_engine_set_tree_w64(af_engine* e, int32_t game, int32_t count, const double* w);

int af_state_to_key(const char* state, int32_t board_size, uint64_t* key);
int af_key_to_state(const uint64_t* key, int32_t board_size, char* out, int32_t cap);

const char* af_strerror(int code);
int af_abi_version(void);

#ifdef __cplusplus
}
#endif
#endif
```

### include/af_net.h

```cpp
#ifndef AF_NET_H
#define AF_NET_H

#include <stdint.h>

#ifdef __cplusplus
extern "C" {
#endif

typedef struct af_net af_net;

#define AF_NET_OK 0
#define AF_NET_ERR_ARG   (-1)
#define AF_NET_ERR_HIP   (-2)
#define AF_NET_ERR_NAME  (-3)
#define AF_NET_ERR_STATE (-4)

int af_net_create(int32_t board_size, int32_t max_batch, int32_t device, af_net** out);
void af_net_destroy(af_net* n);

int af_net_set_variable(af_net* n, const char* tf_name, const float* host_data, int64_t count);
int af_net_finalize(af_net* n);

int af_net_update_device(af_net* n, void* stream, const char* const* tf_names, const float* const* dev_ptrs, const int64_t* counts,
                         int32_t nvars);

int af_net_forward(af_net* n, void* stream, const float* planes_dev, int32_t batch, float* policy_dev, float* value_dev);

int af_net_tune(int32_t key, int32_t value);

int af_net_debug_activation(af_net* n, int32_t which, int32_t batch, float* host_out);

int64_t af_net_debug_weights(af_net* n, int32_t index, void* host_out, int64_t cap_bytes);
int32_t af_net_debug_scales(af_net* n, float* host_out, int32_t cap);

int af_net_small_forward_error(af_net* n);

int64_t af_net_flops_per_position(const af_net* n);
const char* af_net_strerror(int code);

#ifdef __cplusplus
}
#endif
#endif
```

Baseline: 6101.

## Skip network evaluation of non-pending rows via live-row mask in f16s kernels

Passes the engine's per-game pending flags into the f16s conv kernels, so each workgroup builds a wave ballot over the positions it owns and walks only the live ones through the stem and the layer pipelines. Rows with no pending leaf are no longer run through the net, which cuts conv work when many games are idle in a tick. In exchange it adds a mask load and ballot per workgroup, rebuilds the prefetch position queue, and needs graph-capture bookkeeping so stale graphs or weights fall back to evaluating all rows.

```diff
diff --git a/alphafive_amd/csrc/af_conv_f16s.h b/alphafive_amd/csrc/af_conv_f16s.h
--- a/alphafive_amd/csrc/af_conv_f16s.h
+++ b/alphafive_amd/csrc/af_conv_f16s.h
@@ -46,14 +46,16 @@
     bool heads;
     F16sForm form;
     bool valu_stem, two_wg_per_cu, half_classes, tile_split, fused_blocks;
+    const int32_t* live;
 };
-F16sPlan f16s_plan(const f16s_net* n, int batch, int bits, bool heads);
+F16sPlan f16s_plan(const f16s_net* n, int batch, int bits, bool heads, const int32_t* live = nullptr);
 int f16s_forward(f16s_net* n, const F16sPlan& p, hipStream_t st, const float* planes_dev, float* value, float* policy);
 int f16s_trunk(f16s_net* n, const F16sPlan& p, hipStream_t st, const float* planes_dev);
 int f16s_value_branch(f16s_net* n, const F16sPlan& p, hipStream_t st, float* o3_dev, int WP, int PP, float* value);
 int f16s_policy_branch(f16s_net* n, const F16sPlan& p, hipStream_t st, float* o5_dev, int WP, int PP, float* policy);
 int f16s_small_forward_error(f16s_net* n);
 int f16s_read_activation(f16s_net* n, int which, int batch, float* host);
+int f16s_live_walk(int bx, int gxw, int nq, int swizzle, const int32_t* live_host, int32_t* out, int cap);
 
 constexpr int kF16sScaleGroups = 20;
 int f16s_update_absmax(f16s_net* n, hipStream_t st, const float* const* src, float* max_dev);
diff --git a/alphafive_amd/csrc/af_conv_f16s.hip b/alphafive_amd/csrc/af_conv_f16s.hip
--- a/alphafive_amd/csrc/af_conv_f16s.hip
+++ b/alphafive_amd/csrc/af_conv_f16s.hip
@@ -170,6 +170,37 @@
     __syncthreads();
 }
 
+constexpr int kLiveMaxOwned = 64;
+__host__ __device__ inline int f16s_first_pos(int bx, int gxw, int halves, bool swizzle) {
+    if (swizzle && (gxw & (8 * halves - 1)) == 0) return (bx >> 3) + (gxw >> 3) * (bx & 7);
+    return bx;
+}
+__host__ __device__ inline bool f16s_live_walkable(int q0, int gxw, int nq) { return q0 < nq && (nq - q0 + gxw - 1) / gxw <= kLiveMaxOwned; }
+struct LiveWalk {
+    uint64_t rem;
+    int q0, gxw, nq;
+    bool masked;
+    __host__ __device__ inline int next(int q) {
+        if (!masked) return q < nq ? q + gxw : q;
+        if (rem == 0) return nq;
+        const int i = __builtin_ctzll(rem);
+        rem &= rem - 1;
+        return q0 + i * gxw;
+    }
+    __host__ __device__ inline int begin(int* count) {
+        if (!masked) { *count = q0 < nq ? (nq - q0 + gxw - 1) / gxw : 0; return q0; }
+        *count = __builtin_popcountll(rem);
+        return next(q0);
+    }
+};
+__device__ __forceinline__ uint64_t f16s_live_mask(const int32_t* __restrict__ live, int q0, int gxw, int nq) {
+    const int lane = threadIdx.x & 63;
+    const long long q = (long long)q0 + (long long)lane * gxw;
+    int f = 0;
+    if (q < nq) f = live[q];
+    return __ballot(f != 0);
+}
+
 struct F16sArgs {
     const char* in;
     const char* in2;
@@ -195,6 +226,7 @@
     int df_need;
     int* df_done;
     int* df_err;
+    const int32_t* live;
     int abl;
 };
 
@@ -233,9 +265,15 @@
     const uint32_t lds = (uint32_t)(uintptr_t)smem;
 
     const int nq = HSEL >= 0 ? A.batch : A.batch * HV;
-    int qpos = bx;
-    if (AF_F16S_XCD_SWIZZLE && (gxw & (8 * (HSEL >= 0 ? 1 : HV) - 1)) == 0) qpos = (bx >> 3) + (gxw >> 3) * (bx & 7);
-    if (qpos >= nq) return;
+    const int q0 = f16s_first_pos(bx, gxw, HSEL >= 0 ? 1 : HV, AF_F16S_XCD_SWIZZLE != 0);
+    if (q0 >= nq) return;
+    LiveWalk walk;
+    walk.rem = 0; walk.q0 = q0; walk.gxw = gxw; walk.nq = nq;
+    walk.masked = HV == 1 && HSEL < 0 && DF == 0 && A.live != nullptr && f16s_live_walkable(q0, gxw, nq);
+    if (walk.masked) walk.rem = f16s_live_mask(A.live, q0, gxw, nq);
+    int npos_;
+    int qpos = walk.begin(&npos_);
+    if (npos_ == 0) return;
     const int hv = HSEL >= 0 ? HSEL : (HV == 1 ? 0 : qpos % HV);
     const uint32_t wsrc = G::wbase(hv) * 16u;
     AF_T(t_entry);
@@ -256,12 +294,13 @@
         if (DF != 0) glds16_sc1(src + offh + lane * 16, (uint32_t)__builtin_amdgcn_readfirstlane((int)(lds + kLds0 + slot_off + offl)));
         else glds16(src + offh + lane * 16, (uint32_t)__builtin_amdgcn_readfirstlane((int)(lds + kLds0 + slot_off + offl)));
     };
-    const int q0 = qpos;
-    auto stream_src = [&](uint32_t idx) -> const char* {
-        const int p = q0 + (int)(idx / SPP) * gxw, j = (int)(idx % SPP);
-        return slab_src(p, j);
-    };
-    const uint32_t nslabs = (uint32_t)((nq - q0 + gxw - 1) / gxw) * SPP;
+    constexpr int LA = (SPP - 1 + kDist) / SPP;
+    int qn[LA + 1];
+    qn[0] = qpos;
+#pragma unroll
+    for (int k = 1; k <= LA; ++k) qn[k] = walk.next(qn[k - 1]);
+    auto stream_src = [&](int idx) -> const char* { return slab_src(qn[idx / SPP], idx % SPP); };
+    const uint32_t nslabs = (uint32_t)npos_ * SPP;
 
     if (DF == 0) {
 #pragma unroll
@@ -354,7 +393,7 @@
         for (int f = 0; f < 4; ++f) asm volatile("" : "+v"(HA[f]));
     }
     if (DF != 0) {
-        df_wait_one(A.df_wait + qpos, A.df_need, A.df_err);
+        df_wait_one(A.df_wait + q0, A.df_need, A.df_err);
 #pragma unroll
         for (int d = 0; d < kDist; ++d) {
             if ((uint32_t)d < nslabs) {
@@ -444,7 +483,13 @@
 #ifdef AF_F16S_TIMING
     unsigned long long tacc[8] = {0, 0, 0, 0, 0, 0, 0, 0};
 #endif
-    for (; qpos < nq; qpos += gxw) {
+    auto advance = [&]() {
+#pragma unroll
+        for (int k = 0; k < LA; ++k) qn[k] = qn[k + 1];
+        qn[LA] = walk.next(qn[LA]);
+        qpos = qn[0];
+    };
+    for (; qpos < nq; advance()) {
         const int pos = (HV == 1 || HSEL >= 0) ? qpos : qpos / HV;
         AF_T(tp0);
         if (!XPOS) { AF_FIRST_ITEM(cur) }
@@ -473,7 +518,7 @@
             const int NI = proj ? ITP : ITM;
             const int ibase = proj ? pslab * ITP : NSP * ITP + ms * ITM;
             const int seq = proj ? NSM * ITM + pslab * ITP : ms * ITM;
-            const int npos = qpos + ((j + kDist) / SPP) * gxw;
+            const int npos = qn[(j + kDist) / SPP];
             const bool more = npos < nq && !(A.abl & 1);
             const char* nsrc = slab_src((A.abl & 4) ? q0 : (more ? npos : qpos), (j + kDist) % SPP);
             const uint32_t nx1 = cur + kSlotL == kRing * kSlotL ? 0u : cur + kSlotL;
@@ -966,7 +1011,16 @@
 template <class G, bool SC1 = false>
 __device__ __forceinline__ void f16s_stem_body(const float* __restrict__ planes, const uint4* __restrict__ w ,
                                                const float* __restrict__ bias, float inv_scale, char* __restrict__ out, int batch,
-                                               const int bx, const int gx, uint4* ent, _Float16* img) {
+                                               const int bx, const int gx, uint4* ent, _Float16* img, const int32_t* __restrict__ live = nullptr) {
+    if (bx >= batch) return;
+    LiveWalk walk;
+    walk.rem = 0; walk.q0 = bx; walk.gxw = gx; walk.nq = batch;
+    walk.masked = !SC1 && live != nullptr && f16s_live_walkable(bx, gx, batch);
+    if (walk.masked) walk.rem = f16s_live_mask(live, bx, gx, batch);
+    int npos_;
+    int pos = walk.begin(&npos_);
+    if (npos_ == 0) return;
+    int nxp = walk.next(pos);
     constexpr int S = G::S, NPIX = G::NPIX, SR = S + 4, IW = S + 5;
     constexpr int NPL = 3 * NPIX, NLD = (NPL + 255) / 256;
     constexpr int NTL = (NPIX + 31) / 32, NRND = (NTL + 3) / 4;
@@ -991,15 +1045,15 @@
         const int i = (int)threadIdx.x + 256 * q;
         at[q] = img_at(i < NPL ? i : 0);
         nx[q] = 0.0f;
-        if (i < NPL && bx < batch) nx[q] = planes[(size_t)bx * NPL + i];
-    }
-    for (int pos = bx; pos < batch; pos += gx) {
+        if (i < NPL) nx[q] = planes[(size_t)pos * NPL + i];
+    }
+    for (; pos < batch; pos = nxp, nxp = walk.next(nxp)) {
         __syncthreads();
 #pragma unroll
         for (int q = 0; q < NLD; ++q)
             if ((int)threadIdx.x + 256 * q < NPL) img[at[q]] = (_Float16)nx[q];
-        if (pos + gx < batch) {
-            const float* pl = planes + (size_t)(pos + gx) * NPL;
+        if (nxp < batch) {
+            const float* pl = planes + (size_t)nxp * NPL;
 #pragma unroll
             for (int q = 0; q < NLD; ++q)
                 if ((int)threadIdx.x + 256 * q < NPL) nx[q] = pl[threadIdx.x + 256 * q];
@@ -1055,10 +1109,10 @@
 
 template <class G>
 __global__ __launch_bounds__(256) void af_stem_mfma_f16s(const float* __restrict__ planes, const uint4* __restrict__ w, const float* __restrict__ bias,
-                                                         float inv_scale, char* __restrict__ out, int batch) {
+                                                         float inv_scale, char* __restrict__ out, int batch, const int32_t* __restrict__ live) {
     __shared__ __attribute__((aligned(16))) uint4 ent[StemLds<G>::kEnt];
     __shared__ _Float16 img[StemLds<G>::kImg];
-    f16s_stem_body<G>(planes, w, bias, inv_scale, out, batch, (int)blockIdx.x, (int)gridDim.x, ent, img);
+    f16s_stem_body<G>(planes, w, bias, inv_scale, out, batch, (int)blockIdx.x, (int)gridDim.x, ent, img, live);
 }
 
 template <class G>
@@ -1855,7 +1909,7 @@
 
 constexpr int kSmallBatch = 8;
 
-F16sPlan f16s_plan(const f16s_net* n, int batch, int bits, bool heads) {
+F16sPlan f16s_plan(const f16s_net* n, int batch, int bits, bool heads, const int32_t* live) {
     const bool s11 = n->S == 11, small = batch <= kSmallBatch;
     F16sPlan p = {};
     p.batch = batch; p.bits = bits; p.heads = heads;
@@ -1870,6 +1924,7 @@
         p.form = kF16sPaired;
     else
         p.form = kF16sBranches;
+    p.live = s11 && p.form != kF16sRoles ? live : nullptr;
     return p;
 }
 
@@ -1879,7 +1934,7 @@
     a.w = n->w[li]; a.bias = n->bias[li]; a.inv_scale = n->inv_scale[li];
     a.pw = n->pw[li]; a.pbuf = n->pbuf[li / 2]; a.inv_scale_p = n->inv_scale_p[li];
     a.inv_scale2 = a.inv_scale_h = 1.0f;
-    a.batch = p.batch; a.stash = n->stash;
+    a.batch = p.batch; a.stash = n->stash; a.live = p.live;
     a.abl = (p.bits & 0xf0ff) | (li << 8);
     static const int mask = [] { const char* e = getenv("AF_F16S_ABL_LAYERS"); return e ? (int)strtol(e, nullptr, 0) : 0x3ff; }();
     if (!((mask >> li) & 1)) a.abl &= ~kF16sProfilingBits;
@@ -1941,7 +1996,7 @@
     int rc = with_geo(n, [&](auto g) {
         using G = decltype(g);
         if (p.valu_stem) hipLaunchKernelGGL(af_stem_f16s<G>, dim3(std::min(batch, 2048)), dim3(256), 0, st, planes, n->stem_w, n->stem_b, n->f0, batch);
-        else hipLaunchKernelGGL(af_stem_mfma_f16s<G>, dim3(std::min(batch, 1024)), dim3(256), 0, st, planes, n->stem_wm, n->stem_b, n->stem_inv_scale, n->f0, batch);
+        else hipLaunchKernelGGL(af_stem_mfma_f16s<G>, dim3(std::min(batch, 1024)), dim3(256), 0, st, planes, n->stem_wm, n->stem_b, n->stem_inv_scale, n->f0, batch, p.live);
         FS_HIP_OK(hipGetLastError());
         return 0;
     });
@@ -2099,6 +2154,24 @@
     return C;
 }
 
+int f16s_live_walk(int bx, int gxw, int nq, int swizzle, const int32_t* live_host, int32_t* out, int cap) {
+    if (bx < 0 || gxw < 1 || bx >= gxw || nq < 0 || (cap > 0 && !out)) return -1;
+    const int q0 = f16s_first_pos(bx, gxw, 1, swizzle != 0);
+    if (q0 >= nq) return 0;
+    LiveWalk walk;
+    walk.rem = 0; walk.q0 = q0; walk.gxw = gxw; walk.nq = nq;
+    walk.masked = live_host != nullptr && f16s_live_walkable(q0, gxw, nq);
+    if (walk.masked)
+        for (int lane = 0; lane < 64; ++lane) {
+            const long long q = (long long)q0 + (long long)lane * gxw;
+            if (q < nq && live_host[q] != 0) walk.rem |= 1ull << lane;
+        }
+    int count = 0, k = 0;
+    for (int q = walk.begin(&count); q < nq; q = walk.next(q), ++k)
+        if (k < cap) out[k] = q;
+    return k == count ? count : -1;
+}
+
 #ifdef AF_DF_TIMING
 extern "C" int af_df_debug_wall(unsigned long long* host) {
     FS_HIP_OK(hipDeviceSynchronize());
diff --git a/alphafive_amd/csrc/af_engine.hip b/alphafive_amd/csrc/af_engine.hip
--- a/alphafive_amd/csrc/af_engine.hip
+++ b/alphafive_amd/csrc/af_engine.hip
@@ -1564,6 +1564,8 @@
 
 int64_t af_engine_memo_epoch(af_engine* e) { return (e && e->memo) ? (int64_t)e->P.memo_epoch : 0; }
 
+const int32_t* af_engine_live_rows(af_engine* e) { return e ? e->P.pending : nullptr; }
+
 int af_engine_memo_stats(af_engine* e, void* stream, uint64_t* out) {
     if (!e || !e->memo || !out) return AF_ERR_ARG;
     hipStream_t st = (hipStream_t)stream;
diff --git a/alphafive_amd/csrc/af_net.hip b/alphafive_amd/csrc/af_net.hip
--- a/alphafive_amd/csrc/af_net.hip
+++ b/alphafive_amd/csrc/af_net.hip
@@ -829,9 +829,9 @@
     return join_value(n, st, vs);
 }
 
-static int forward_f16s(af_net* n, hipStream_t st, const float* planes, int batch, float* policy, float* value) {
+static int forward_f16s(af_net* n, hipStream_t st, const float* planes, int batch, float* policy, float* value, const int32_t* live) {
     const bool fhead = g_tune.fhead;
-    const F16sPlan plan = f16s_plan(n->f16s, batch, g_tune.f16s_bits, fhead);
+    const F16sPlan plan = f16s_plan(n->f16s, batch, g_tune.f16s_bits, fhead, live);
     if (plan.form != kF16sBranches) return f16s_forward(n->f16s, plan, st, planes, value, policy) ? AF_NET_ERR_HIP : AF_NET_OK;
     float *o3 = n->act[kO + 4], *o5 = n->act[kO + 8];
     if (f16s_trunk(n->f16s, plan, st, planes)) return AF_NET_ERR_HIP;
@@ -848,9 +848,18 @@
 extern "C" {
 
 int af_net_forward(af_net* n, void* stream, const float* planes, int32_t batch, float* policy, float* value) {
+    return af_net_forward_live(n, stream, planes, batch, policy, value, nullptr);
+}
+
+int af_net_debug_live_walk(int32_t bx, int32_t gxw, int32_t nq, int32_t swizzle, const int32_t* live_host, int32_t* out, int32_t cap) {
+    const int c = f16s_live_walk(bx, gxw, nq, swizzle, live_host, out, cap);
+    return c < 0 ? AF_NET_ERR_ARG : c;
+}
+
+int af_net_forward_live(af_net* n, void* stream, const float* planes, int32_t batch, float* policy, float* value, const int32_t* live_dev) {
     if (!n || !planes || !policy || !value || batch < 1 || batch > n->max_batch) return AF_NET_ERR_ARG;
     if (!n->ready) return AF_NET_ERR_STATE;
-    if (g_tune.conv == 5 && n->f16s) return forward_f16s(n, (hipStream_t)stream, planes, batch, policy, value);
+    if (g_tune.conv == 5 && n->f16s) return forward_f16s(n, (hipStream_t)stream, planes, batch, policy, value, live_dev);
     return forward_wino(n, (hipStream_t)stream, planes, batch, policy, value);
 }
 
diff --git a/alphafive_amd/engine.py b/alphafive_amd/engine.py
--- a/alphafive_amd/engine.py
+++ b/alphafive_amd/engine.py
@@ -82,6 +82,8 @@
         L.af_engine_memo_stats.argtypes = [vp, vp, u64p]
         L.af_engine_memo_epoch.argtypes = [vp]
         L.af_engine_memo_epoch.restype = C.c_int64
+        L.af_engine_live_rows.argtypes = [vp]
+        L.af_engine_live_rows.restype = vp
         L.af_match_create.argtypes = [vp, vp, C.POINTER(vp)]
         L.af_match_destroy.argtypes = [vp]
         L.af_match_destroy.restype = None
@@ -148,6 +150,7 @@
         self._status = np.zeros(num_games, np.int32)
         self._params = {"training": int(bool(training)), "sims": int(self.cfg.simulation_per_step),
                         "upper": int(self.cfg.upper_simulation_per_step), "tick_budget": None}
+        self.outside_writes = 0
 
     def close(self):
         if getattr(self, "_h", None):
@@ -159,6 +162,12 @@
     def tick(self, policy_ptr, value_ptr, planes_ptr, stream=None):
         _check(lib().af_engine_tick(self._h, stream, policy_ptr, value_ptr, planes_ptr), "af_engine_tick")
 
+    def live_rows(self):
+        ptr = lib().af_engine_live_rows(self._h)
+        if not ptr:
+            raise EngineError("af_engine_live_rows returned NULL")
+        return int(ptr)
+
     def status(self, stream=None):
         rc = lib().af_engine_status(self._h, stream, _p(self._status, C.c_int32))
         _check(rc, "engine status")
@@ -178,6 +187,7 @@
 
     def set_root(self, game, key, last_cell=-1, random_a=False, reset_tree=False):
         key = np.ascontiguousarray(key, np.uint64)
+        self.outside_writes += 1
         _check(lib().af_engine_set_root(self._h, game, _p(key, C.c_uint64), last_cell, int(random_a), int(reset_tree)),
                "af_engine_set_root")
 
@@ -191,6 +201,7 @@
 
     def set_roots(self, games, keys, last_cells, random_a=False, reset_tree=False, stream=None):
         n = len(games)
+        self.outside_writes += 1
         g = np.ascontiguousarray(games, np.int32)
         k = np.ascontiguousarray(keys, np.uint64).reshape(n, self.KW2)
         lc = np.ascontiguousarray(last_cells, np.int32)
@@ -279,6 +290,7 @@
 
     def load_tree(self, game, dump):
         cnt = len(dump["sum_n"])
+        self.outside_writes += 1
         arr = {k: np.ascontiguousarray(dump[k], t) for k, t in (("keys", np.uint64), ("sum_n", np.int32), ("n", np.int32),
                                                                  ("w", np.float32), ("p", np.float32), ("f32", np.uint8))}
         _check(lib().af_engine_load_tree(self._h, game, cnt, _p(arr["keys"], C.c_uint64), _p(arr["sum_n"], C.c_int32),
@@ -354,7 +366,7 @@
 class SelfPlayEngine:
 
     def __init__(self, cfg, num_games, pv_device, device=0, seed=0, first_game_id=0, training=True, node_cap=0,
-                 value_f64=False, weights_version=None, eval_memo=None):
+                 value_f64=False, weights_version=None, eval_memo=None, live_rows=True):
         import torch
         if not torch.cuda.is_available():
             raise EngineError("SelfPlayEngine needs a HIP device (torch.cuda.is_available() is False)")
@@ -380,6 +392,12 @@
                                   "pass SelfPlayEngine(..., weights_version=lambda: net.version)")
             self.engine.memo_enable(**({} if eval_memo is True else dict(eval_memo)))
             self._memo_version = self._weights_version()
+        self._live_ptr = None
+        if live_rows and getattr(pv_device, "accepts_live", False) and self._weights_version is not None:
+            self._live_ptr = self.engine.live_rows()
+        self._live_seen = None
+        self.all_rows_ticks, self.live_ticks = 0, 0
+        self._graph_live = self._graph_stamped_live = False
         self.ticks = 0
         self._boxes = {}
         self._graph = None
@@ -398,10 +416,22 @@
             if ver != self._memo_version:
                 self.engine.memo_clear(stream)
                 self._memo_version = ver
+        live = None
+        if self._live_ptr is not None:
+            seen = (self._weights_version(), self.engine.outside_writes)
+            mine = (self.planes.data_ptr(), self.G, self.policy.data_ptr(), self.value.data_ptr())
+            if seen == self._live_seen and self.pv_device.last_forward() == mine:
+                live = self._live_ptr
+            self._live_seen = seen
         self.engine.tick(self.policy.data_ptr(), self.value.data_ptr(), self.planes.data_ptr(), stream)
         if stamp_base is not None:
             self.engine.stamp(stamp_base + 1, stream)
-        p, v = self.pv_device(self.planes)
+        if live is not None:
+            p, v = self.pv_device(self.planes, live=live)
+            self.live_ticks += 1
+        else:
+            p, v = self.pv_device(self.planes)
+            self.all_rows_ticks += 1
         if p.data_ptr() != self.policy.data_ptr():
             self.policy.copy_(p.reshape(self.G, self.C))
         if v.data_ptr() != self.value.data_ptr():
@@ -426,7 +456,7 @@
 
     def _graph_key(self, n):
         ver = self._weights_version
-        return (int(n), self.engine.params_key(), ver() if ver is not None else None)
+        return (int(n), self.engine.params_key(), ver() if ver is not None else None, self.engine.outside_writes)
 
     def run_ticks_graph(self, n=16, timed=False, stamped=False):
         torch = self.torch
@@ -434,6 +464,10 @@
             raise EngineError("run_ticks_graph: pv_device takes bind_outputs but exposes no weights_version (a replayed graph "
                               "would keep evaluating with stale weights); pass SelfPlayEngine(..., weights_version=lambda: net.version)")
         key = self._graph_key(n)
+        if self._live_ptr is not None and self._graph is not None:
+            mine = (self.planes.data_ptr(), self.G, self.policy.data_ptr(), self.value.data_ptr())
+            if self.pv_device.last_forward() != mine:
+                self._graph = self._graph_stamped = None
         if stamped:
             if 3 * n > STAMP_SLOTS:
                 raise EngineError("run_ticks_graph(stamped=True): at most %d ticks per replay" % (STAMP_SLOTS // 3))
@@ -446,6 +480,7 @@
                     self._stamp_event = torch.cuda.Event()
                 torch.cuda.synchronize(self.dev)
                 g = torch.cuda.CUDAGraph()
+                counts = (self.live_ticks, self.all_rows_ticks)
                 with torch.cuda.graph(g, capture_error_mode="thread_local"):
                     for i in range(n):
                         self.tick(stamp_base=3 * i)
@@ -453,10 +488,13 @@
                     self.engine.stamps_async(self._stamp_host.data_ptr(), st)
                     self.engine.progress_async(self._prog_host.data_ptr(), st)
                 self.ticks -= n
+                self._graph_stamped_live = self.live_ticks - counts[0] == n
+                self.live_ticks, self.all_rows_ticks = counts
                 self._graph_stamped = (self._graph_key(n), g, n)
             if self._stamp_pending:
                 self._collect_stamps()
             self._graph_stamped[1].replay()
+            self._count_replayed(n, self._graph_stamped_live)
             self._stamp_event.record(torch.cuda.current_stream(self.dev))
             self._stamp_pending = True
             self.ticks += n
@@ -472,17 +510,21 @@
             self.tick()
             torch.cuda.synchronize(self.dev)
             g = torch.cuda.CUDAGraph()
+            counts = (self.live_ticks, self.all_rows_ticks)
             with torch.cuda.graph(g, capture_error_mode="thread_local"):
                 for _ in range(n):
                     self.tick()
                 st = torch.cuda.current_stream(self.dev).cuda_stream
                 self.engine.progress_async(self._prog_host.data_ptr(), st)
             self.ticks -= n
+            self._graph_live = self.live_ticks - counts[0] == n
+            self.live_ticks, self.all_rows_ticks = counts
             self._graph = (self._graph_key(n), g)
         if timed:
             e0, e1 = torch.cuda.Event(enable_timing=True), torch.cuda.Event(enable_timing=True)
             e0.record(torch.cuda.current_stream(self.dev))
         self._graph[1].replay()
+        self._count_replayed(n, self._graph_live)
         if timed:
             e1.record(torch.cuda.current_stream(self.dev))
             self.replay_events.append((n, e0, e1))
@@ -490,6 +532,12 @@
         self._prog_turn ^= 1
         self._prog_events[self._prog_turn].record(torch.cuda.current_stream(self.dev))
         self._prog_replays += 1
+
+    def _count_replayed(self, n, live):
+        if live:
+            self.live_ticks += n
+        else:
+            self.all_rows_ticks += n
 
     def _collect_stamps(self):
         self._stamp_event.synchronize()
diff --git a/alphafive_amd/net_hip.py b/alphafive_amd/net_hip.py
--- a/alphafive_amd/net_hip.py
+++ b/alphafive_amd/net_hip.py
@@ -27,6 +27,8 @@
         L.af_net_set_variable.argtypes = [vp, C.c_char_p, C.POINTER(C.c_float), C.c_int64]
         L.af_net_finalize.argtypes = [vp]
         L.af_net_forward.argtypes = [vp, vp, vp, C.c_int32, vp, vp]
+        L.af_net_forward_live.argtypes = [vp, vp, vp, C.c_int32, vp, vp, vp]
+        L.af_net_debug_live_walk.argtypes = [C.c_int32, C.c_int32, C.c_int32, C.c_int32, C.POINTER(C.c_int32), C.POINTER(C.c_int32), C.c_int32]
         L.af_net_update_device.argtypes = [vp, vp, C.POINTER(C.c_char_p), C.POINTER(vp), C.POINTER(C.c_int64), C.c_int32]
         L.af_net_debug_weights.argtypes = [vp, C.c_int32, vp, C.c_int64]
         L.af_net_debug_weights.restype = C.c_int64
@@ -133,12 +135,12 @@
         assert policy.shape[0] >= self.max_batch or policy.shape[0] == value.shape[0]
         self.policy, self.value = policy, value
 
-    def __call__(self, planes):
+    def __call__(self, planes, live=None):
         B = planes.shape[0]
         assert B <= self.max_batch and planes.is_contiguous() and planes.dtype == torch.float32
         stream = torch.cuda.current_stream(self.device).cuda_stream
-        _check(lib().af_net_forward(self._h, stream, planes.data_ptr(), B, self.policy.data_ptr(), self.value.data_ptr()),
-               "af_net_forward")
+        _check(lib().af_net_forward_live(self._h, stream, planes.data_ptr(), B, self.policy.data_ptr(), self.value.data_ptr(), live),
+               "af_net_forward_live")
         return self.policy[:B], self.value[:B]
 
     def small_forward_error(self):
@@ -159,10 +161,11 @@
     if resnet.device.type != "cuda" or not (3 <= resnet.board_size <= 15):
         return None
     lib()
-    state = {"net": None, "out": None, "version": None}
-
-    def pv(planes):
+    state = {"net": None, "out": None, "version": None, "last": None}
+
+    def pv(planes, live=None):
         B = planes.shape[0]
+        reloaded = state["net"] is None or state["net"].max_batch < B or state["version"] != getattr(resnet, "version", None)
         if state["net"] is None or state["net"].max_batch < B:
             if state["net"] is not None:
                 state["net"].close()
@@ -183,7 +186,12 @@
             else:
                 state["net"].load(resnet.variables)
             state["version"] = version
-        return state["net"](planes)
+        net = state["net"]
+        if reloaded:
+            live = None
+        out = net(planes, live)
+        state["last"] = (planes.data_ptr(), B, net.policy.data_ptr(), net.value.data_ptr())
+        return out
 
     def bind_outputs(policy, value):
         state["out"] = (policy, value)
@@ -194,8 +202,11 @@
         if state["net"] is not None:
             state["net"].close()
             state["net"] = None
+            state["last"] = None
 
     pv.bind_outputs = bind_outputs
+    pv.accepts_live = True
+    pv.last_forward = lambda: state["last"]
     pv.close = close
     pv.weights_version = lambda: getattr(resnet, "version", None)
     return pv
diff --git a/include/af_engine.h b/include/af_engine.h
--- a/include/af_engine.h
+++ b/include/af_engine.h
@@ -97,6 +97,8 @@
 int af_engine_stamp(af_engine* e, void* stream, int32_t slot);
 int af_engine_stamps_async(af_engine* e, void* stream, uint64_t* out_pinned);
 
+const int32_t* af_engine_live_rows(af_engine* e);
+
 #define AF_MATCH_UNFINISHED (-1)
 #define AF_MATCH_WIN0 0
 #define AF_MATCH_WIN1 1
diff --git a/include/af_net.h b/include/af_net.h
--- a/include/af_net.h
+++ b/include/af_net.h
@@ -26,6 +26,10 @@
 
 int af_net_forward(af_net* n, void* stream, const float* planes_dev, int32_t batch, float* policy_dev, float* value_dev);
 
+int af_net_forward_live(af_net* n, void* stream, const float* planes_dev, int32_t batch, float* policy_dev, float* value_dev,
+                        const int32_t* live_dev);
+int af_net_debug_live_walk(int32_t bx, int32_t gxw, int32_t nq, int32_t swizzle, const int32_t* live_host, int32_t* out, int32_t cap);
+
 int af_net_tune(int32_t key, int32_t value);
 
 int af_net_debug_activation(af_net* n, int32_t which, int32_t batch, float* host_out);
```

Result: no change. 6098 (-0.0%).
